# UVA-Computer-Vision-Lab/FrameINO

Measured on AMD Instinct MI355X. Metric: denoise-steps/sec (Wan2.2-5B FrameINO, 49f 704x1280, cond+uncond DiT forward + CFG + Euler), higher is better.
Workload: dtype bf16; 1 GPU; wan2.2-5b-49f-704x1280; layers=30, id_frames=1, hip_graph=False, parallelism=single, dead_rows_last_block=1760

## Files before the change

frameino_amd/_lib.py:

```python
import ctypes
import os
import re

_HERE = os.path.dirname(os.path.abspath(__file__))
LIB_PATH = os.environ.get("FINO_LIB_PATH") or os.path.join(_HERE, "lib", "libframeino_hip.so")
HEADER_PATH = os.path.join(os.path.dirname(_HERE), "include", "frameino_hip.h")

c_void_p, c_int, c_i64, c_float = ctypes.c_void_p, ctypes.c_int, ctypes.c_int64, ctypes.c_float

SIGNATURES = {
    "fino_version": [],
    "fino_last_error": [],
    "fino_tune_set": [c_int, c_int],
    "fino_tune_get": [c_int],
    "fino_adaln_modulate": [c_void_p, c_void_p, c_i64, c_int, c_i64, c_i64, c_void_p, c_void_p, c_i64, c_void_p,
                            c_float, c_int, c_void_p],
    "fino_layernorm": [c_void_p, c_void_p, c_i64, c_int, c_i64, c_i64, c_void_p, c_void_p, c_float, c_int, c_void_p],
    "fino_gated_residual": [c_void_p, c_void_p, c_void_p, c_i64, c_int, c_i64, c_i64, c_i64, c_void_p, c_i64,
                            c_void_p, c_int, c_void_p],
    "fino_gated_residual_staged": [c_void_p, c_void_p, c_void_p, c_i64, c_int, c_i64, c_i64, c_i64, c_void_p, c_i64,
                                   c_void_p, c_int, c_void_p],
    "fino_layernorm_zero": [c_void_p, c_void_p, c_i64, c_int, c_i64, c_i64, c_void_p, c_void_p, c_void_p, c_void_p,
                            c_i64, c_void_p, c_float, c_int, c_void_p],
    "fino_rmsnorm_rope": [c_void_p, c_i64, c_int, c_i64, c_void_p, c_float, c_void_p, c_void_p, c_int, c_int,
                          c_void_p],
    "fino_rmsnorm_rope_scaled": [c_void_p, c_i64, c_int, c_i64, c_void_p, c_float, c_void_p, c_void_p, c_int, c_float,
                                 c_int, c_void_p],
    "fino_qkv_rmsnorm_rope": [c_void_p, c_i64, c_int, c_i64, c_void_p, c_float, c_void_p, c_float, c_void_p, c_void_p, c_int,
                              c_float, c_void_p, c_void_p, c_void_p, c_int, c_void_p],
    "fino_rmsnorm_rope_scatter": [c_void_p, c_i64, c_int, c_i64, c_void_p, c_float, c_void_p, c_void_p, c_int, c_float,
                                  c_void_p, c_void_p, c_void_p, c_int, c_void_p],
    "fino_diag_mfma_peak": [c_int, c_int, c_int, c_void_p, ctypes.POINTER(ctypes.c_double), c_void_p],
    "fino_headnorm_rope": [c_void_p, c_int, c_i64, c_int, c_int, c_i64, c_i64, c_void_p, c_void_p, c_float,
                           c_void_p, c_void_p, c_i64, c_int, c_void_p],
    "fino_headnorm_rope_scaled": [c_void_p, c_int, c_i64, c_int, c_int, c_i64, c_i64, c_void_p, c_void_p, c_float,
                                  c_void_p, c_void_p, c_i64, c_float, c_int, c_void_p],
    "fino_attn_fwd": [c_void_p] * 4 + [c_int, c_int, c_i64, c_i64, c_int] + [c_i64] * 12 + [c_float, c_int, c_void_p],
    "fino_attn_fwd_ws": [c_void_p] * 4 + [c_int, c_int, c_i64, c_i64, c_int] + [c_i64] * 12 +
                        [c_float, c_int, c_void_p, c_i64, c_void_p],
    "fino_attn_workspace_bytes": [c_int, c_int, c_i64, c_i64, c_int],
    "fino_attn_tail_supported": [c_int, c_int, c_i64, c_i64, c_int],
    "fino_attn_fwd_tail": [c_void_p] * 4 + [c_int, c_int, c_i64, c_i64, c_int] + [c_i64] * 12 + [c_float, c_int, c_void_p, c_void_p,
                                                                                            c_void_p],
    "fino_attn_probs_supported": [c_int, c_int, c_i64, c_i64, c_int],
    "fino_attn_probs": [c_void_p] * 3 + [c_int, c_int, c_i64, c_i64, c_int] + [c_i64] * 6 + [c_int, c_i64, c_i64, c_float, c_int,
                                                                                         c_void_p, c_void_p, c_void_p, c_i64,
                                                                                         c_void_p, c_void_p],
    "fino_row_rrms": [c_void_p, c_i64, c_int, c_i64, c_float, c_void_p, c_int, c_void_p],
    "fino_attn_fp8_kv_bytes": [c_int, c_int, c_i64, c_int],
    "fino_attn_fwd_fp8": [c_void_p] * 4 + [c_int, c_int, c_i64, c_i64, c_int] + [c_i64] * 8 + [c_float, c_int, c_int, c_void_p,
                                                                                           c_i64, c_void_p],
    "fino_attn_partial_bytes": [c_int, c_int, c_i64, c_int],
    "fino_attn_partial": [c_void_p] * 3 + [c_int, c_int, c_i64, c_i64, c_int] + [c_i64] * 9 + [c_float, c_int, c_void_p,
                                                                                               c_i64, c_void_p],
    "fino_attn_merge": [c_void_p, c_int, c_int, c_i64, c_int, c_i64, c_i64, c_i64, c_void_p, c_void_p, c_void_p, c_int,
                        c_void_p],
    "fino_mxfp8_scale_bytes": [c_i64, c_i64],
    "fino_quantize_mxfp8": [c_void_p, c_void_p, c_void_p, c_i64, c_i64, c_i64, c_int, c_void_p],
    "fino_gemm_mxfp8": [c_void_p] * 6 + [c_i64] * 4 + [c_int, c_void_p, c_i64, c_void_p, c_i64, c_void_p, c_int, c_void_p],
    "fino_gemm_mxfp8_q": [c_void_p] * 7 + [c_i64] * 3 + [c_int, c_int, c_void_p],
    "fino_mxfp6_bytes": [c_i64, c_i64],
    "fino_mxfp6_scale_bytes": [c_i64, c_i64],
    "fino_quantize_mxfp6": [c_void_p, c_void_p, c_void_p, c_i64, c_i64, c_i64, c_int, c_void_p],
    "fino_gemm_mxfp6": [c_void_p] * 6 + [c_i64] * 4 + [c_int, c_void_p, c_i64, c_void_p, c_i64, c_void_p, c_int, c_void_p],
    "fino_traj_paint": [c_void_p, c_void_p, c_void_p, c_int, c_int, c_int, c_int, c_void_p],
    "fino_traj_blur_quantize": [c_void_p, c_void_p, c_void_p, c_void_p, c_int, c_int, c_int, c_int, c_void_p],
    "fino_groupnorm_workspace_bytes": [c_int],
    "fino_groupnorm_cl": [c_void_p, c_void_p] + [c_int] * 6 + [c_void_p, c_void_p, c_float, c_void_p, c_void_p] +
                         [c_int] * 4 + [c_void_p, c_i64, c_int, c_void_p],
    "fino_avg_pool_time2": [c_void_p, c_void_p] + [c_int] * 5 + [c_void_p],
    "fino_resize_area_pad_u8": [c_void_p, c_void_p] + [c_int] * 9 + [c_void_p],
    "fino_u8_hwc_to_chw_unit": [c_void_p, c_void_p, c_int, c_int, c_void_p],
    "fino_gemm": [c_void_p] * 4 + [c_i64] * 6 + [c_int, c_void_p, c_i64, c_void_p, c_i64, c_void_p, c_int, c_void_p],
    "fino_gemm_split_n": [c_void_p] * 4 + [c_i64] * 6 + [c_int, c_void_p, c_i64, c_void_p, c_i64, c_void_p, c_int, c_void_p,
                          c_i64, c_i64, c_int, c_void_p],
    "fino_ln_mxfp8": [c_int, c_void_p, c_void_p, c_void_p, c_i64, c_int, c_i64, c_void_p, c_void_p, c_void_p, c_void_p, c_i64,
                      c_void_p, c_float, c_int, c_void_p],
    "fino_gemm_blocked_a": [c_void_p, c_void_p, c_void_p, c_void_p, c_i64, c_i64, c_i64, c_i64, c_i64, c_int, c_i64, c_i64, c_i64,
                            c_i64, c_void_p, c_i64, c_void_p, c_i64, c_void_p, c_int, c_int, c_void_p],
    "fino_gemm_plan": [c_i64, c_i64, ctypes.POINTER(c_i64), ctypes.POINTER(c_int)],
    "fino_skinny_linear": [c_void_p, c_void_p, c_void_p, c_void_p, c_int, c_i64, c_i64, c_int, c_int, c_void_p],
    "fino_patchify": [c_void_p, c_void_p] + [c_int] * 7 + [c_i64, c_int, c_void_p],
    "fino_unpatchify": [c_void_p, c_void_p] + [c_int] * 7 + [c_i64, c_int, c_void_p],
    "fino_wan_model_input": [c_void_p] * 5 + [c_int] * 6 + [c_void_p],
    "fino_cfg_euler_step": [c_void_p, c_void_p, c_void_p] + [c_int] * 5 + [c_float, c_void_p, c_int, c_int, c_void_p],
    "fino_cfg_unipc_step": [c_void_p] * 6 + [c_int] * 5 + [c_void_p, c_int, c_void_p],
    "fino_cfg_vpred_step": [c_void_p, c_void_p, c_i64, c_i64, c_void_p, c_int, c_int, c_void_p],
    "fino_cfg_dpm_step": [c_void_p, c_void_p, c_void_p, c_void_p, c_i64, c_i64, c_void_p, c_int, c_int, c_void_p],
    "fino_conv3d": [c_void_p] * 4 + [c_int] * 19 + [c_void_p, c_void_p, c_int, c_void_p],
    "fino_rmsnorm_silu_cl": [c_void_p, c_void_p, c_i64, c_int, c_int, c_void_p, c_int, c_int, c_void_p],
    "fino_split_bf16": [c_void_p, c_void_p, c_i64, c_int, c_i64, c_i64, c_int, ctypes.c_uint, c_void_p],
    "fino_rmsnorm_silu_cl_f32": [c_void_p, c_void_p, c_i64, c_int, c_int, c_void_p, c_int, c_int, ctypes.c_uint, c_void_p],
    "fino_conv3d_split": [c_void_p] * 4 + [c_int] * 20 + [c_void_p, c_void_p, c_void_p],
    "fino_vae_blend_tiles": [c_void_p, c_void_p] + [c_int] * 9 + [c_void_p],
    "fino_softmax_rows": [c_void_p, c_i64, c_int, c_i64, c_float, c_int, c_void_p],
    "fino_dup_up3d_add": [c_void_p] * 3 + [c_int] * 10 + [c_void_p],
    "fino_avg_down3d_add": [c_void_p] * 3 + [c_int] * 10 + [c_void_p],
    "fino_vae_unpatchify_clamp": [c_void_p, c_void_p] + [c_int] * 7 + [c_void_p],
    "fino_vae_patchify": [c_void_p, c_void_p] + [c_int] * 7 + [c_void_p],
    "fino_lora_merge": [c_void_p, c_i64, c_void_p, c_i64, c_i64, c_i64, c_int, ctypes.POINTER(c_void_p),
                        ctypes.POINTER(c_i64), ctypes.POINTER(c_void_p), ctypes.POINTER(c_i64), ctypes.POINTER(c_int),
                        ctypes.POINTER(c_float), c_int, c_void_p],
    "fino_step_cache_probe": [c_void_p, c_int, c_i64, c_void_p, c_void_p, c_int, c_void_p],
    "fino_step_cache_residual": [c_void_p, c_i64, c_void_p, c_i64, c_void_p, c_i64, c_i64, c_i64, c_int, c_int, c_void_p],
}


class StepCacheSegment(ctypes.Structure):
    _fields_ = [("h0", c_void_p), ("h1", c_void_p), ("p", c_void_p), ("r", c_void_p), ("h1_copy", c_void_p),
                ("rows", c_i64), ("ld_h0", c_i64), ("ld_h1", c_i64), ("ld_p", c_i64), ("ld_r", c_i64), ("ld_h1_copy", c_i64)]
_RESTYPES = {"fino_last_error": ctypes.c_char_p, "fino_attn_workspace_bytes": c_i64, "fino_mxfp8_scale_bytes": c_i64,
             "fino_groupnorm_workspace_bytes": c_i64,
             "fino_attn_partial_bytes": c_i64, "fino_attn_fp8_kv_bytes": c_i64, "fino_mxfp6_bytes": c_i64,
             "fino_mxfp6_scale_bytes": c_i64}


ABI_VERSION = 103


def declared_symbols(header_path=HEADER_PATH):
    text = open(header_path).read()
    text = re.sub(r"/\*.*?\*/", "", text, flags=re.S)
    return sorted(set(re.findall(r"\b(fino_[a-z0-9_]+)\s*\(", text)))


def load(path=LIB_PATH):
    if not os.path.exists(path):
        raise RuntimeError(
            f"frameino_amd: HIP library not found at {path}. Build it with `python -c 'import __graft_entry__ as g; "
            f"g.build()'` (or `make -C frameino_amd/csrc`). There is no CPU fallback for the product path.")
    lib = ctypes.CDLL(path)
    lib.fino_version.restype = c_int
    if lib.fino_version() < 0 and os.environ.get("FINO_ALLOW_EXPERIMENT") != "1":
        raise RuntimeError(
            f"frameino_amd: {path} is a timing-EXPERIMENT build (compiled with -DFINO_EXPERIMENT: its kernels may skip "
            f"work and return wrong results; fino_version() = {lib.fino_version()}).  It is refused as the product library; "
            f"set FINO_ALLOW_EXPERIMENT=1 for the tools/ scripts that time it.")
    if abs(lib.fino_version()) != ABI_VERSION:
        raise RuntimeError(
            f"frameino_amd: {path} reports fino_version() = {lib.fino_version()}, this package binds ABI version "
            f"{ABI_VERSION} (include/frameino_hip.h: FINO_VERSION).  Rebuild it (`make -C frameino_amd/csrc`).")
    for name, argtypes in SIGNATURES.items():
        fn = getattr(lib, name)
        fn.argtypes = argtypes
        fn.restype = _RESTYPES.get(name, c_int)
    return lib


_lib = None


def lib():
    global _lib
    if _lib is None:
        _lib = load()
    return _lib


def check(rc, what=""):
    if rc != 0:
        raise RuntimeError(f"{what} failed ({rc}): {lib().fino_last_error().decode()}")
```

frameino_amd/csrc/fino_attention_probs.hip:

```cpp
#include <stdlib.h>

#include "fino_attention_common.h"
using namespace fino_attn_ns;

namespace {

struct ProbsParams {
    const uint16_t* q;
    const uint16_t* k;
    uint16_t* p;
    int batch, heads, lq, lk;
    int64_t q_bs, q_rs, q_hs, k_bs, k_rs, k_hs, p_bs, p_rs;
    int kp;
    const float* q_rrms;
    const uint16_t* q_weight;
    int64_t q_rrms_bs;
    float scale_log2;
    int lk_b[4];
    float log2_mult[4];
};

template <typename T, int NKB>
__global__ __launch_bounds__(256) void attn_probs_kernel(const ProbsParams p) {
    typedef typename T::vec8 vec8;
    __shared__ __attribute__((aligned(16))) char smem[4 * 8192];
    const int tid = threadIdx.x;
    const int lane = tid & 63;
    const int wave = tid >> 6;
    const int r = lane & 31;
    const int h = lane >> 5;
    const int hb = blockIdx.y;
    const int bi = hb / p.heads;
    const int head = hb - bi * p.heads;

    const int lkc = p.lk_b[bi < 4 ? bi : 3];
    const float lm = p.log2_mult[bi < 4 ? bi : 3];
    const int nkb = (lkc + 31) >> 5;
    const uint16_t* kp_ = p.k + bi * p.k_bs + head * p.k_hs;
    for (int i = 0; i < nkb * 2; ++i) {
        const int c = tid + 256 * i;
        const int row = c >> 4, ch = c & 15;
        uint4 u = make_uint4(0, 0, 0, 0);
        if (row < p.lk) u = *reinterpret_cast<const uint4*>(kp_ + (int64_t)row * p.k_rs + ch * 8);
        *reinterpret_cast<uint4*>(smem + row * 256 + ((ch ^ (row & 15)) << 4)) = u;
    }
    const int qrow = blockIdx.x * 128 + wave * 32 + r;
    const int qrc = qrow < p.lq ? qrow : p.lq - 1;
    const uint16_t* qp = p.q + bi * p.q_bs + head * p.q_hs + (int64_t)qrc * p.q_rs + 8 * h;
    vec8 qf[8];
    if (p.q_rrms) {
        const float rs = p.q_rrms[bi * p.q_rrms_bs + qrc];
        const uint16_t* wp = p.q_weight + head * 128 + 8 * h;
#pragma unroll
        for (int ks = 0; ks < 8; ++ks) {
            float f[8], ww[8];
            unpack8<T>(*reinterpret_cast<const uint4*>(qp + 16 * ks), f);
            unpack8<T>(*reinterpret_cast<const uint4*>(wp + 16 * ks), ww);
#pragma unroll
            for (int j = 0; j < 8; ++j) f[j] = round_to<T>(round_to<T>(f[j] * rs) * ww[j]);
            qf[ks] = __builtin_bit_cast(vec8, pack8<T>(f));
        }
    } else {
#pragma unroll
        for (int ks = 0; ks < 8; ++ks) qf[ks] = __builtin_bit_cast(vec8, *reinterpret_cast<const uint4*>(qp + 16 * ks));
    }
    __syncthreads();

    f32x16_t acc[NKB];
#pragma unroll
    for (int kb = 0; kb < NKB; ++kb)
#pragma unroll
        for (int j = 0; j < 16; ++j) acc[kb][j] = 0.f;
#pragma unroll
    for (int kb = 0; kb < NKB; ++kb) {
        if (kb < nkb) {
#pragma unroll
            for (int ks = 0; ks < 8; ++ks) {
                const int row = kb * 32 + r;
                const uint4 a = *reinterpret_cast<const uint4*>(smem + row * 256 + (((2 * ks + h) ^ (row & 15)) << 4));
                acc[kb] = T::mfma32(__builtin_bit_cast(vec8, a), qf[ks], acc[kb]);
            }
        }
    }

    const float c2 = p.scale_log2;
    float m = -INFINITY;
#pragma unroll
    for (int kb = 0; kb < NKB; ++kb) {
#pragma unroll
        for (int j = 0; j < 16; ++j) {
            const int key = kb * 32 + (j & 3) + 8 * (j >> 2) + 4 * h;
            float x = acc[kb][j] * c2;
            x = key == lkc - 1 ? x + lm : x;
            x = key >= lkc ? -INFINITY : x;
            acc[kb][j] = x;
            m = fmaxf(m, x);
        }
    }
    {
        const auto sw = __builtin_amdgcn_permlane32_swap(__float_as_uint(m), __float_as_uint(m), false, false);
        m = fmaxf(__uint_as_float(sw[0]), __uint_as_float(sw[1]));
    }
    float l = 0.f;
#pragma unroll
    for (int kb = 0; kb < NKB; ++kb) {
#pragma unroll
        for (int j = 0; j < 16; ++j) {
            const float e = __builtin_amdgcn_exp2f(acc[kb][j] - m);
            acc[kb][j] = e;
            l += e;
        }
    }
    {
        const auto sw = __builtin_amdgcn_permlane32_swap(__float_as_uint(l), __float_as_uint(l), false, false);
        l = __uint_as_float(sw[0]) + __uint_as_float(sw[1]);
    }
    const float inv = 1.0f / l;
    __syncthreads();
    char* stage = smem + wave * 8192;
#pragma unroll
    for (int kb = 0; kb < NKB; ++kb) {
#pragma unroll
        for (int g4 = 0; g4 < 4; ++g4) {
            const int key0 = kb * 32 + 8 * g4 + 4 * h;
            if (key0 < p.kp) {
                const uint32_t w0 = (uint32_t)T::from_f32(acc[kb][4 * g4 + 0] * inv) | ((uint32_t)T::from_f32(acc[kb][4 * g4 + 1] * inv) << 16);
                const uint32_t w1 = (uint32_t)T::from_f32(acc[kb][4 * g4 + 2] * inv) | ((uint32_t)T::from_f32(acc[kb][4 * g4 + 3] * inv) << 16);
                *reinterpret_cast<uint2*>(stage + r * 256 + ((((key0 >> 3)) ^ (r & 15)) << 4) + ((key0 & 4) << 1)) = make_uint2(w0, w1);
            }
        }
    }
    __syncthreads();
    const int pieces = p.kp >> 3;
    const int total = 32 * pieces;
    const int row_base = blockIdx.x * 128 + wave * 32;
    uint16_t* pbase = p.p + bi * p.p_bs + head * p.kp;
    for (int i = lane; i < total; i += 64) {
        const int rr = i / pieces, pc = i - rr * pieces;
        const uint4 u = *reinterpret_cast<const uint4*>(stage + rr * 256 + ((pc ^ (rr & 15)) << 4));
        if (row_base + rr < p.lq) *reinterpret_cast<uint4*>(pbase + (int64_t)(row_base + rr) * p.p_rs + pc * 8) = u;
    }
}

}

extern "C" int fino_attn_probs_supported(int batch, int heads, int64_t lq, int64_t lk, int head_dim) {
    return head_dim == 128 && batch >= 1 && batch <= 4 && heads > 0 && lq > 0 && lk >= 1 && lk <= 128 &&
           (int64_t)batch * heads <= 65535;
}

extern "C" int fino_attn_probs(const void* q, const void* k, void* p, int batch, int heads, int64_t lq, int64_t lk,
                               int head_dim, int64_t q_bs, int64_t q_rs, int64_t q_hs, int64_t k_bs, int64_t k_rs, int64_t k_hs,
                               int kp, int64_t p_bs, int64_t p_rs, float scale, int dtype, const int* lk_b,
                               const float* tail_mult, const float* q_rrms, int64_t q_rrms_bs, const void* q_weight,
                               void* stream) {
    FINO_CHECK((q_rrms == nullptr) == (q_weight == nullptr) && fino_aligned16(q_weight), FINO_ERR_ARG,
               "fino_attn_probs: q_rrms and q_weight come together (q_weight 16-byte aligned)");
    FINO_CHECK(dtype == FINO_BF16 || dtype == FINO_F16, FINO_ERR_ARG, "fino_attn_probs: dtype %d", dtype);
    FINO_CHECK(q && k && p && lk_b && tail_mult, FINO_ERR_ARG, "fino_attn_probs: null pointer");
    FINO_CHECK(fino_attn_probs_supported(batch, heads, lq, lk, head_dim), FINO_ERR_UNSUPPORTED,
               "fino_attn_probs: needs head_dim 128, batch <= 4, lk <= 128 (got head_dim %d, batch %d, lk %lld)", head_dim, batch,
               (long long)lk);
    FINO_CHECK(fino_aligned16(q) && fino_aligned16(k) && fino_aligned16(p) && q_rs % 8 == 0 && k_rs % 8 == 0 && q_hs % 8 == 0 &&
                   k_hs % 8 == 0 && q_bs % 8 == 0 && k_bs % 8 == 0 && p_bs % 8 == 0 && p_rs % 8 == 0,
               FINO_ERR_ARG, "fino_attn_probs: pointers and strides must be 16-byte aligned");
    FINO_CHECK(kp > 0 && kp % 8 == 0 && kp <= 128 && p_rs >= (int64_t)heads * kp, FINO_ERR_ARG,
               "fino_attn_probs: kp %d (a multiple of 8, <= 128), row stride %lld", kp, (long long)p_rs);
    FINO_CHECK(scale > 0.f || scale == FINO_ATTN_SCALE_FOLDED, FINO_ERR_ARG, "fino_attn_probs: scale");
    if (lq == 0) return FINO_OK;
    ProbsParams pp;
    pp.q = (const uint16_t*)q; pp.k = (const uint16_t*)k; pp.p = (uint16_t*)p;
    pp.batch = batch; pp.heads = heads; pp.lq = (int)lq; pp.lk = (int)lk;
    pp.q_bs = q_bs; pp.q_rs = q_rs; pp.q_hs = q_hs; pp.k_bs = k_bs; pp.k_rs = k_rs; pp.k_hs = k_hs; pp.p_bs = p_bs; pp.p_rs = p_rs;
    pp.kp = kp;
    pp.q_rrms = q_rrms; pp.q_weight = (const uint16_t*)q_weight; pp.q_rrms_bs = q_rrms_bs;
    pp.scale_log2 = scale == FINO_ATTN_SCALE_FOLDED ? 1.0f : scale * 1.4426950408889634f;
    for (int b = 0; b < 4; ++b) {
        const int bb = b < batch ? b : batch - 1;
        FINO_CHECK(lk_b[bb] >= 1 && lk_b[bb] <= lk && lk_b[bb] <= kp && tail_mult[bb] >= 1.0f, FINO_ERR_ARG,
                   "fino_attn_probs: lk_b[%d] = %d (of %lld, kp %d), tail_mult %g", bb, lk_b[bb], (long long)lk, kp,
                   (double)tail_mult[bb]);
        pp.lk_b[b] = lk_b[bb];
        pp.log2_mult[b] = log2f(tail_mult[bb]);
    }
    hipStream_t st = (hipStream_t)stream;
    const dim3 grid((unsigned)((lq + 127) / 128), (unsigned)(batch * heads));
    int max_lk = 0;
    for (int b = 0; b < batch; ++b) max_lk = lk_b[b] > max_lk ? lk_b[b] : max_lk;
    const int need = max_lk > kp ? max_lk : kp;
    const int nkb = need <= 64 ? 2 : (need <= 96 ? 3 : 4);
#define PROBS_LAUNCH(T_)                                                                                      \
    {                                                                                                         \
        if (nkb == 2) attn_probs_kernel<T_, 2><<<grid, 256, 0, st>>>(pp);                                     \
        else if (nkb == 3) attn_probs_kernel<T_, 3><<<grid, 256, 0, st>>>(pp);                                \
        else attn_probs_kernel<T_, 4><<<grid, 256, 0, st>>>(pp);                                              \
    }
    if (dtype == FINO_BF16) PROBS_LAUNCH(BF16) else PROBS_LAUNCH(F16)
#undef PROBS_LAUNCH
    FINO_LAUNCH_CHECK();
    return FINO_OK;
}
```

frameino_amd/csrc/fino_gemm.hip:

```cpp
#include <stdlib.h>

#include <atomic>
#include <type_traits>

#include "fino_gemm_common.h"

using namespace fino_gemm_ns;

#ifdef FINO_GEMM_STAMP
extern "C" int fino_gemm_debug_read(unsigned long long* out) {
    return (int)hipMemcpyFromSymbol(out, HIP_SYMBOL(fino_gemm_dbg), sizeof(unsigned long long) * 64);
}
#endif

namespace {

template <typename T, int EPI, bool GENERIC, bool CONV>
__global__ __launch_bounds__(kThreads, 2) void gemm_kernel(const GemmParams p) {
    extern __shared__ __attribute__((aligned(16))) char smem[];
    typedef typename T::vec8 vec8;
    const int tid = threadIdx.x;
    const int lane = tid & 63;
    const int wave = tid >> 6;
    const int wm = wave >> 2;
// ... 210 lines not shown
            acc0 += t1 - t0; acc1 += t2 - t1; acc2 += t3 - t2; acc3 += t4 - t3;
#endif
        }
#ifdef FINO_GEMM_STAMP
        if (blockIdx.x == 17 && lane == 0) {
            fino_gemm_dbg[wave * 8 + 0] = acc0; fino_gemm_dbg[wave * 8 + 1] = acc1;
            fino_gemm_dbg[wave * 8 + 2] = acc2; fino_gemm_dbg[wave * 8 + 3] = acc3;
            fino_gemm_dbg[wave * 8 + 4] = (unsigned long long)nk;
        }
#endif
        __syncthreads();
    }
#undef LD_W
#undef LD_A
#undef K_STEP
#undef LOAD_FRAGS
#undef MFMA_BLOCK

    gemm_epilogue<T, EPI>(acc, p, smem, m0, n0, tid, lane, wm, wn);
}

__device__ __forceinline__ int ablk_koff(const GemmParams& p, int kt) {
    const int b = (kt * p.a_inv) >> 16;
    const int j = (b * p.a_ginv) >> 16;
    return (b - j * p.a_groups) * (int)(p.a_grp_elems * 2) + j * (int)(p.a_blk_elems * 2) + (kt - b * p.a_tpb) * (BK * 2);
}

template <typename T, bool CONV, int MI, bool ABLK = false>
__device__ __forceinline__ void pp_mainloop(const GemmParams& p, char* smem, const int64_t m0, const int64_t n0,
                                            const int kb, const int nk, f32x4_t (&acc)[MI][4], const int tid,
                                            const int lane, const int wave, const int wm, const int wn) {
    typedef typename T::vec8 vec8;
    static_assert(MI >= 2 && MI <= 8, "tile height 64 .. 256");
    static_assert(!CONV || MI == 8, "the implicit-GEMM gather is built for 256-row tiles");
    enum : int { NA0 = (MI + 1) / 2, NA1 = MI - (MI + 1) / 2 };

    const int r8 = lane >> 3;
    const int sk = ((lane & 7) ^ ((4 * (wn & 1) + (lane >> 4)) & 7)) * 8;
    const __amdgpu_buffer_rsrc_t w_rsrc = __builtin_amdgcn_make_buffer_rsrc(
        (void*)p.w, 0, (int)(((p.n - 1) * p.ldw + p.k) * 2), 0x00020000);
    const int aq0 = wm == 0 ? 0 : NA0;
    uint32_t a_off[4], w_off[8];
    uint32_t pos[CONV ? 4 : 1];
    int ck = 0, tap_t = 0, tap_h = 0, tap_w = 0, t_first = 0, t_in_first = 0;
    int cseg = 0, seg = 0, a_koff = 0;
    const uint16_t* a_base_ptr = p.a;
    int64_t a_bytes = ((p.m - 1) * p.lda + p.k) * 2;
    if constexpr (ABLK)
        a_bytes = ((p.a_groups - 1) * p.a_grp_elems + (p.k / (BK * p.a_tpb) / p.a_groups - 1) * p.a_blk_elems +
                   (p.m - 1) * p.lda + BK * p.a_tpb) * 2;
    if constexpr (CONV) {
        const int hw = p.ho * p.wo;
        t_first = (int)(m0 / hw);
        t_in_first = t_first * p.st - p.pt;
        t_in_first = t_in_first < 0 ? 0 : t_in_first;
        const int64_t frame = (int64_t)p.hi * p.wi * p.lda;
        a_base_ptr = p.a + (int64_t)t_in_first * frame;
        a_bytes = (int64_t)(p.ti - t_in_first) * frame * 2;
        a_bytes = a_bytes > 0x7fffffffll ? 0x7fffffffll : a_bytes;
#pragma unroll
        for (int q = 0; q < NA0; ++q) {
            int64_t gm = m0 + (aq0 + q) * 32 + wn * 8 + r8;
            gm = gm < p.m ? gm : p.m - 1;
            const int t = (int)(gm / hw);
            const int rem = (int)(gm - (int64_t)t * hw);
            const int h = rem / p.wo;
            pos[q] = ((uint32_t)(t - t_first) << 24) | ((uint32_t)h << 12) | (uint32_t)(rem - h * p.wo);
        }
    }
    const __amdgpu_buffer_rsrc_t a_rsrc = __builtin_amdgcn_make_buffer_rsrc((void*)a_base_ptr, 0, (int)a_bytes, 0x00020000);
    auto conv_offsets = [&]() {
        const int hlim = p.up ? 2 * p.hi : p.hi, wlim = p.up ? 2 * p.wi : p.wi;
#pragma unroll
        for (int q = 0; q < NA0; ++q) {
            const int ti = (t_first + (int)(pos[CONV ? q : 0] >> 24)) * p.st + tap_t - p.pt;
            int hi = (int)((pos[CONV ? q : 0] >> 12) & 0xfffu) * p.sh + tap_h - p.ph;
            int wi = (int)(pos[CONV ? q : 0] & 0xfffu) * p.sw + tap_w - p.pw;
            const bool ok = (unsigned)ti < (unsigned)p.ti && (unsigned)hi < (unsigned)hlim && (unsigned)wi < (unsigned)wlim;
            if (p.up) { hi >>= 1; wi >>= 1; }
            const uint32_t off = (uint32_t)(((((ti - t_in_first) * p.hi + hi) * p.wi + wi) * (int)p.lda + sk) * 2);
            a_off[q] = ok ? off : 0x80000000u;
        }
    };
    auto conv_next = [&]() {
        if (p.a_cc > 0 && ++cseg == p.a_cc) { cseg = 0; ++seg; }
        if (++ck == p.cin_chunks) {
            ck = 0; cseg = 0; seg = 0;
            if (++tap_w == p.kw) {
                tap_w = 0;
                if (++tap_h == p.kh) { tap_h = 0; ++tap_t; }
            }
            conv_offsets();
        }
        if (p.a_cc > 0) {
            const int plane = p.a_nplanes == 3 ? (seg >= 3) + (seg >= 5) : (seg >= 2);
            a_koff = (plane * p.a_cc + cseg) * (BK * 2);
        } else {
            a_koff = ck * (BK * 2);
        }
    };
    if constexpr (CONV) {
        conv_offsets();
    } else {
#pragma unroll
        for (int q = 0; q < NA0; ++q) {
            int64_t gm = m0 + (aq0 + q) * 32 + wn * 8 + r8;
            gm = gm < p.m ? gm : p.m - 1;
            a_off[q] = (uint32_t)((gm * p.lda + sk) * 2);
        }
    }
    const int w_piece_bytes = (int)(32 * p.ldw * 2);
    const int w_pieces = CONV ? (int)((p.n - n0 + 31) / 32) : 8;
#pragma unroll
    for (int q = 0; q < 8; ++q) {
        int64_t gn = n0 + q * 32 + wn * 8 + r8;
        gn = gn < p.n ? gn : p.n - 1;
        w_off[q] = (uint32_t)((gn * p.ldw + sk) * 2);
    }
#ifndef GP_DMA_AUX
#define GP_DMA_AUX 0
#endif
#define PP_DMA_A(STAGE_, KT_, QI_)                                                                                \
    if ((QI_) < NA1 || wm == 0)                                                                                   \
        __builtin_amdgcn_raw_ptr_buffer_load_lds(                                                                 \
            a_rsrc, (FINO_LDS void*)(smem + (STAGE_) * kStageBytes + ((aq0 + (QI_)) * 32 + wn * 8) * 128), 16,    \
            a_off[QI_], CONV ? a_koff : (ABLK ? ablk_koff(p, kb + (KT_)) : (kb + (KT_)) * (BK * 2)), 0, GP_DMA_AUX);
#define PP_DMA_W(STAGE_, KT_, Q_)                                                                                 \
    if (!CONV || (Q_) < w_pieces)                                                                                 \
        __builtin_amdgcn_raw_ptr_buffer_load_lds(                                                                 \
            w_rsrc, (FINO_LDS void*)(smem + (STAGE_) * kStageBytes + kTileBytes + ((Q_) * 32 + wn * 8) * 128), 16, \
            w_off[CONV ? 0 : (Q_)], (kb + (KT_)) * (BK * 2) + (CONV ? (Q_) * w_piece_bytes : 0), 0, GP_DMA_AUX);

    const int frow = lane & 15;
    const int pch0 = (lane >> 4) ^ (frow >> 1);
    const int a_base = (wm * (16 * MI) + frow) * 128;
    const int w_base = kTileBytes + (wn * 64 + frow) * 128;

#pragma unroll
    for (int i = 0; i < MI; ++i)
#pragma unroll
        for (int j = 0; j < 4; ++j) acc[i][j] = f32x4_t{0.f, 0.f, 0.f, 0.f};

#pragma unroll
    for (int q = 0; q < 4; ++q) {
        if (q < NA0) { PP_DMA_A(0, 0, q) }
        if (wm == 0) { PP_DMA_W(0, 0, q) } else { PP_DMA_W(0, 0, 4 + q) }
    }
    if constexpr (CONV) conv_next();
    if (nk > 1) {
#pragma unroll
        for (int q = 0; q < 4; ++q) {
            if (q < NA0) { PP_DMA_A(1, 1, q) }
            if (wm == 0) { PP_DMA_W(1, 1, q) } else { PP_DMA_W(1, 1, 4 + q) }
        }
        if constexpr (CONV) conv_next();
    }
    asm volatile("s_waitcnt vmcnt(0)" ::: "memory");
    __builtin_amdgcn_s_barrier();
    if (wm == 1) __builtin_amdgcn_s_barrier();

    u32x4_t af[2][MI], wf[2][4];
#ifdef FINO_GEMM_STAMP
    unsigned long long t0, t1, t2, t3, t4, acc0 = 0, acc1 = 0, acc2 = 0, acc3 = 0;
#define PSTAMP(V_) { __builtin_amdgcn_sched_barrier(0); STAMP(V_) __builtin_amdgcn_sched_barrier(0); }
#else
#define PSTAMP(V_)
#endif
    for (int t = 0; t < nk; ++t) {
        const int cur = t & 1;
        const char* sb = smem + cur * kStageBytes;
        PSTAMP(t0)
#pragma unroll
        for (int kk = 0; kk < 2; ++kk) {
            const int pch = (pch0 ^ (kk << 2)) << 4;
#pragma unroll
            for (int j = 0; j < 4; ++j) wf[kk][j] = *reinterpret_cast<const u32x4_t*>(sb + w_base + j * 2048 + pch);
#pragma unroll
            for (int i = 0; i < MI; ++i) af[kk][i] = *reinterpret_cast<const u32x4_t*>(sb + a_base + i * 2048 + pch);
        }
        if (t >= 1 && t + 1 < nk) {
#pragma unroll
            for (int q = 0; q < NA0; ++q) PP_DMA_A(cur ^ 1, t + 1, q)
            if (wm == 0) {
#pragma unroll
                for (int q = 0; q < 8; ++q) { PP_DMA_W(cur ^ 1, t + 1, q) }
            }
            if constexpr (CONV) conv_next();
        }
        __builtin_amdgcn_sched_barrier(0);
        asm volatile("s_waitcnt lgkmcnt(0)" ::: "memory");
        PSTAMP(t1)
        __builtin_amdgcn_s_barrier();
        __builtin_amdgcn_sched_barrier(0);
        PSTAMP(t2)
#ifndef GP_ORDER
#define GP_ORDER 3
#endif
#pragma unroll
        for (int kk = 0; kk < 2; ++kk) {
#if GP_ORDER == 0
#pragma unroll
            for (int i = 0; i < MI; ++i) {
#pragma unroll
                for (int j = 0; j < 4; ++j)
                    acc[i][j] = T::mfma16(__builtin_bit_cast(vec8, wf[kk][j]), __builtin_bit_cast(vec8, af[kk][i]),
                                          acc[i][j]);
            }
#elif GP_ORDER == 1
#pragma unroll
            for (int j = 0; j < 4; ++j) {
#pragma unroll
                for (int i = 0; i < MI; ++i)
                    acc[i][j] = T::mfma16(__builtin_bit_cast(vec8, wf[kk][j]), __builtin_bit_cast(vec8, af[kk][i]),
                                          acc[i][j]);
            }
#elif GP_ORDER == 2
#pragma unroll
            for (int j = 0; j < 4; ++j) {
#pragma unroll
                for (int ii = 0; ii < MI; ++ii) {
                    const int i = ((j + 4 * kk) & 1) ? MI - 1 - ii : ii;
                    acc[i][j] = T::mfma16(__builtin_bit_cast(vec8, wf[kk][j]), __builtin_bit_cast(vec8, af[kk][i]),
                                          acc[i][j]);
                }
            }
#else
#pragma unroll
            for (int i = 0; i < MI; ++i) {
#pragma unroll
                for (int jj = 0; jj < 4; ++jj) {
                    const int j = ((i + MI * kk) & 1) ? 3 - jj : jj;
                    acc[i][j] = T::mfma16(__builtin_bit_cast(vec8, wf[kk][j]), __builtin_bit_cast(vec8, af[kk][i]),
                                          acc[i][j]);
                }
            }
#endif
        }
        __builtin_amdgcn_sched_barrier(0);
        asm volatile("s_waitcnt vmcnt(0)" ::: "memory");
        PSTAMP(t3)
        __builtin_amdgcn_s_barrier();
        __builtin_amdgcn_sched_barrier(0);
#ifdef FINO_GEMM_STAMP
        STAMP(t4)
        acc0 += t1 - t0; acc1 += t2 - t1; acc2 += t3 - t2; acc3 += t4 - t3;
#endif
    }
#ifdef FINO_GEMM_STAMP
    if (blockIdx.x == 17 && lane == 0) {
        fino_gemm_dbg[wave * 8 + 0] = acc0; fino_gemm_dbg[wave * 8 + 1] = acc1;
        fino_gemm_dbg[wave * 8 + 2] = acc2; fino_gemm_dbg[wave * 8 + 3] = acc3;
        fino_gemm_dbg[wave * 8 + 4] = (unsigned long long)nk;
    }
#endif
    if (wm == 0) __builtin_amdgcn_s_barrier();
    asm volatile("s_waitcnt vmcnt(0)" ::: "memory");
#undef PP_DMA_A
#undef PP_DMA_W
}

template <typename T, int EPI, bool CONV = false, int MI = 8, bool ABLK = false>
__global__ __launch_bounds__(kThreads, 2) void gemm_pp_kernel(const GemmParams p) {
    extern __shared__ __attribute__((aligned(16))) char smem[];
    const int tid = threadIdx.x;
    const int lane = tid & 63;
    const int wave = __builtin_amdgcn_readfirstlane(tid >> 6);
    const int wm = wave >> 2;
    const int wn = wave & 3;
    int tm, tn;
    tile_coords(p, tm, tn);
    const int64_t m0 = (int64_t)tm * (32 * MI), n0 = (int64_t)tn * BN;
    int nk = (int)(p.k / BK);
#ifndef GP_RAGGED
#define GP_RAGGED 1
#endif
    if constexpr (GP_RAGGED && MI == 8 && !CONV && EPI != FINO_EPI_F32 && EPI != FINO_EPI_F32_RESIDUAL) {
        const int64_t rows = p.m - m0;
        if (rows <= 64) {
            f32x4_t acc2[2][4];
            pp_mainloop<T, false, 2, ABLK>(p, smem, m0, n0, 0, nk, acc2, tid, lane, wave, wm, wn);
            gemm_epilogue<T, EPI, false, 2>(acc2, p, smem, m0, n0, tid, lane, wm, wn);
            return;
        }
        if (rows <= 128) {
            f32x4_t acc4[4][4];
            pp_mainloop<T, false, 4, ABLK>(p, smem, m0, n0, 0, nk, acc4, tid, lane, wave, wm, wn);
            gemm_epilogue<T, EPI, false, 4>(acc4, p, smem, m0, n0, tid, lane, wm, wn);
            return;
        }
    }
    f32x4_t acc[MI][4];
#ifdef FINO_GEMM_STAMP
    unsigned long long ts0, ts1;
    STAMP(ts0)
#endif
    pp_mainloop<T, CONV, MI, ABLK>(p, smem, m0, n0, 0, nk, acc, tid, lane, wave, wm, wn);
#ifdef FINO_GEMM_STAMP
    STAMP(ts1)
    if (blockIdx.x == 17 && lane == 0) fino_gemm_dbg[wave * 8 + 5] = ts1 - ts0;
#endif
    gemm_epilogue<T, EPI, false, MI>(acc, p, smem, m0, n0, tid, lane, wm, wn);
}

template <typename T, int EPI, bool GENERIC, bool CONV = false>
int launch_gemm_t(const GemmParams& p, hipStream_t st) {
    static FinoPerDeviceOnce once;
    if (int rc = fino_max_smem_once(once, reinterpret_cast<const void*>(&gemm_kernel<T, EPI, GENERIC, CONV>), kSmemBytes, "fino_gemm")) return rc;
    gemm_kernel<T, EPI, GENERIC, CONV><<<dim3((unsigned)(p.tiles_m * p.tiles_n)), kThreads, kSmemBytes, st>>>(p);
    FINO_LAUNCH_CHECK();
    return FINO_OK;
}

template <typename T, int EPI, bool CONV = false, int MI = 8, bool ABLK = false>
int launch_gemm_pp(const GemmParams& p, hipStream_t st) {
    static FinoPerDeviceOnce once;
    if (int rc = fino_max_smem_once(once, reinterpret_cast<const void*>(&gemm_pp_kernel<T, EPI, CONV, MI, ABLK>), kSmemBytes, "fino_gemm")) return rc;
    gemm_pp_kernel<T, EPI, CONV, MI, ABLK><<<dim3((unsigned)(p.tiles_m * p.tiles_n)), kThreads, kSmemBytes, st>>>(p);
    FINO_LAUNCH_CHECK();
    return FINO_OK;
}

inline int gemm_device_cus() {
    static std::atomic<int> cus[kFinoMaxDevices];
    const int dev = fino_current_device();
    int c = cus[dev].load(std::memory_order_relaxed);
    if (c == 0) {
        int n = 0;
        c = (hipDeviceGetAttribute(&n, hipDeviceAttributeMultiprocessorCount, dev) == hipSuccess && n > 0) ? n : 256;
        cus[dev].store(c, std::memory_order_relaxed);
    }
    return c;
}

struct TilePlan { int64_t rows1; int mi2; };
inline double plan_launch_cost(int64_t rows, int mi, int tiles_n, int cus) {
    if (rows <= 0) return 0.0;
    const double bm = 32.0 * mi;
    const int64_t tiles = ((rows + 32 * mi - 1) / (32 * mi)) * tiles_n;
    const double mfma_raw = 0.85 * bm / 256.0, mfma = mfma_raw > 0.80 ? mfma_raw : 0.80, deliver = (bm + 256.0) / 512.0;
    const int64_t full = tiles / cus, rem = tiles % cus;
    double c = (double)full * (mfma > deliver ? mfma : deliver);
    if (rem) {
        const double d = deliver * (double)rem / cus;
        c += mfma > d ? mfma : d;
    }
    return c + 0.07;
}
inline TilePlan plan_tiles_search(int64_t m, int tiles_n, int cus);
inline TilePlan plan_tiles(int64_t m, int tiles_n, int cus, int tile_m = 0) {
    const int forced = tile_m ? tile_m : fino_tune_get(FINO_TUNE_GEMM_TILE_M);
    if (forced >= 2 && forced <= 7) return TilePlan{0, forced};
    if (forced == 8 || m <= 0) return TilePlan{m, 8};
    static std::atomic<uint64_t> memo[64];
    const bool memoable = m < (1ll << 24) && tiles_n > 0 && tiles_n < 512 && cus > 0 && cus < 512;
    const uint64_t key = ((uint64_t)m << 18) | ((uint64_t)tiles_n << 9) | (uint64_t)cus;
    std::atomic<uint64_t>& slot = memo[(key * 0x9E3779B97F4A7C15ull) >> 58];
    if (memoable) {
        const uint64_t e = slot.load(std::memory_order_relaxed);
        if ((e & 1) && (e >> 22) == key) {
            const uint64_t r = (e >> 6) & 0xffff;
            return TilePlan{r == 0xffff ? m : (int64_t)r * 256, (int)((e >> 3) & 7) + 1};
        }
    }
    const TilePlan tp = plan_tiles_search(m, tiles_n, cus);
    if (memoable && (tp.rows1 == m || (tp.rows1 % 256 == 0 && tp.rows1 / 256 < 0xffff)) && tp.mi2 >= 2 && tp.mi2 <= 8)
        slot.store((key << 22) | ((tp.rows1 == m ? 0xffffull : (uint64_t)(tp.rows1 / 256)) << 6) |
                       ((uint64_t)(tp.mi2 - 1) << 3) | 1ull, std::memory_order_relaxed);
    return tp;
}
inline TilePlan plan_tiles_search(int64_t m, int tiles_n, int cus) {
    TilePlan best{m, 8};
    double best_c = plan_launch_cost(m, 8, tiles_n, cus);
    const double base_c = best_c;
    const int64_t rows256 = (m + 255) / 256;
    for (int64_t r1 = 0; r1 < rows256; ++r1) {
        const int64_t rows1 = r1 * 256;
        const double c1 = plan_launch_cost(rows1, 8, tiles_n, cus);
        for (int mi = 2; mi <= 8; ++mi) {
            if (rows1 > 0 && mi == 8) continue;
            const double c = c1 + plan_launch_cost(m - rows1, mi, tiles_n, cus);
            if (c < best_c - 1e-9) { best_c = c; best = TilePlan{rows1, mi}; }
        }
    }
    if (best_c > (best.rows1 > 0 ? 0.97 : 0.985) * base_c) return TilePlan{m, 8};
    return best;
}

inline bool use_pingpong() {
    static int v = -1;
    if (v < 0) {
        const char* e = getenv("FINO_GEMM_PP");
        v = (e && e[0] == '0') ? 0 : 1;
    }
    return v == 1;
}

template <typename T, int EPI>
int launch_gemm_pp_mi(const GemmParams& p, int mi, hipStream_t st) {
    if (p.a_tpb > 0) {
        if constexpr (EPI == FINO_EPI_GATED_RESIDUAL) {
            switch (mi) {
                case 2: return launch_gemm_pp<T, EPI, false, 2, true>(p, st);
                case 3: return launch_gemm_pp<T, EPI, false, 3, true>(p, st);
                case 4: return launch_gemm_pp<T, EPI, false, 4, true>(p, st);
                case 5: return launch_gemm_pp<T, EPI, false, 5, true>(p, st);
                case 6: return launch_gemm_pp<T, EPI, false, 6, true>(p, st);
                case 7: return launch_gemm_pp<T, EPI, false, 7, true>(p, st);
                default: return launch_gemm_pp<T, EPI, false, 8, true>(p, st);
            }
        } else {
            fino_set_error("fino_gemm_blocked_a: epilogue must be FINO_EPI_GATED_RESIDUAL");
            return FINO_ERR_UNSUPPORTED;
        }
    }
    switch (mi) {
        case 2: return launch_gemm_pp<T, EPI, false, 2>(p, st);
        case 3: return launch_gemm_pp<T, EPI, false, 3>(p, st);
        case 4: return launch_gemm_pp<T, EPI, false, 4>(p, st);
        case 5: return launch_gemm_pp<T, EPI, false, 5>(p, st);
        case 6: return launch_gemm_pp<T, EPI, false, 6>(p, st);
        case 7: return launch_gemm_pp<T, EPI, false, 7>(p, st);
        default: return launch_gemm_pp<T, EPI, false, 8>(p, st);
    }
}

template <typename T>
int launch_gemm_rows(GemmParams p, int64_t r0, int64_t rows, int mi, int epi, hipStream_t st) {
    p.a += r0 * p.lda;
    p.c += r0 * p.ldc;
    if (p.c2) p.c2 += r0 * p.ldc2;
    if (p.r) p.r += r0 * p.ldr;
    if (p.sel) p.sel += r0;
    p.m = rows;
    p.tiles_m = (int)((rows + 32 * mi - 1) / (32 * mi));
    switch (epi) {
        case FINO_EPI_NONE: return launch_gemm_pp_mi<T, FINO_EPI_NONE>(p, mi, st);
        case FINO_EPI_GELU_TANH: return launch_gemm_pp_mi<T, FINO_EPI_GELU_TANH>(p, mi, st);
        case FINO_EPI_RESIDUAL: return launch_gemm_pp_mi<T, FINO_EPI_RESIDUAL>(p, mi, st);
        case FINO_EPI_GATED_RESIDUAL_STAGED: return launch_gemm_pp_mi<T, FINO_EPI_GATED_RESIDUAL_STAGED>(p, mi, st);
        default: return launch_gemm_pp_mi<T, FINO_EPI_GATED_RESIDUAL>(p, mi, st);
    }
}

template <typename T, bool GENERIC>
int launch_gemm_e(const GemmParams& p, int epi, int tile_m, hipStream_t st) {
    const bool fits32 = ((p.m - 1) * p.lda + p.k) * 2 < (1ll << 31) && ((p.n - 1) * p.ldw + p.k) * 2 < (1ll << 31);
    if (epi == FINO_EPI_F32 || epi == FINO_EPI_F32_RESIDUAL) {
        if (GENERIC || !fits32) {
            fino_set_error("fino_gemm: the fp32-output epilogues need K %% 64 == 0, 16-byte aligned operands and operands < 2 GiB");
            return FINO_ERR_UNSUPPORTED;
        }
        return epi == FINO_EPI_F32 ? launch_gemm_pp<T, FINO_EPI_F32, false, 8>(p, st)
                                   : launch_gemm_pp<T, FINO_EPI_F32_RESIDUAL, false, 8>(p, st);
    }
    if (!GENERIC && use_pingpong() && fits32) {
        const TilePlan tp = plan_tiles(p.m, p.tiles_n, gemm_device_cus(), tile_m);
        if (tp.rows1 > 0)
            if (int rc = launch_gemm_rows<T>(p, 0, tp.rows1, 8, epi, st)) return rc;
        if (tp.rows1 < p.m) return launch_gemm_rows<T>(p, tp.rows1, p.m - tp.rows1, tp.mi2, epi, st);
        return FINO_OK;
    }
    switch (epi) {
        case FINO_EPI_NONE: return launch_gemm_t<T, FINO_EPI_NONE, GENERIC>(p, st);
        case FINO_EPI_GELU_TANH: return launch_gemm_t<T, FINO_EPI_GELU_TANH, GENERIC>(p, st);
        case FINO_EPI_RESIDUAL: return launch_gemm_t<T, FINO_EPI_RESIDUAL, GENERIC>(p, st);
        case FINO_EPI_GATED_RESIDUAL_STAGED: return launch_gemm_t<T, FINO_EPI_GATED_RESIDUAL_STAGED, GENERIC>(p, st);
        default: return launch_gemm_t<T, FINO_EPI_GATED_RESIDUAL, GENERIC>(p, st);
    }
}

template <int WT>
__global__ __launch_bounds__(256) void skinny_linear_kernel(const float* __restrict__ x, const void* __restrict__ w,
                                                            const void* __restrict__ b, float* __restrict__ y, int m,
                                                            int64_t n, int64_t k, int silu_input) {
    const int lane = threadIdx.x & 63;
    const int64_t col = (int64_t)blockIdx.x * 4 + (threadIdx.x >> 6);
    if (col >= n) return;
    float acc[16];
#pragma unroll
    for (int i = 0; i < 16; ++i) acc[i] = 0.f;
    for (int64_t kk = lane; kk < k; kk += 64) {
        float wv;
        if (WT == -1) wv = ((const float*)w)[col * k + kk];
        else if (WT == FINO_BF16) wv = BF16::to_f32(((const uint16_t*)w)[col * k + kk]);
        else wv = F16::to_f32(((const uint16_t*)w)[col * k + kk]);
#pragma unroll
        for (int i = 0; i < 16; ++i) {
            if (i < m) {
                float xv = x[(int64_t)i * k + kk];
                if (silu_input) xv = xv / (1.0f + __expf(-xv));
                acc[i] += xv * wv;
            }
        }
    }
    float bias = 0.f;
    if (b) {
        if (WT == -1) bias = ((const float*)b)[col];
        else if (WT == FINO_BF16) bias = BF16::to_f32(((const uint16_t*)b)[col]);
        else bias = F16::to_f32(((const uint16_t*)b)[col]);
    }
#pragma unroll
    for (int i = 0; i < 16; ++i) {
        if (i < m) {
            const float s = wave_sum(acc[i]);
            if (lane == 0) y[(int64_t)i * n + col] = s + bias;
        }
    }
}

}

extern "C" int fino_gemm_plan(int64_t m, int64_t n, int64_t* rows_256, int* tile_rows_rest) {
    if (m <= 0 || n <= 0) return FINO_ERR_ARG;
    const TilePlan tp = plan_tiles(m, (int)((n + BN - 1) / BN), gemm_device_cus());
    if (rows_256) *rows_256 = tp.rows1;
    if (tile_rows_rest) *tile_rows_rest = tp.rows1 < m ? 32 * tp.mi2 : 0;
    return FINO_OK;
}

extern "C" int fino_gemm(const void* a, const void* w, const void* bias, void* c, int64_t m, int64_t n, int64_t k,
                         int64_t lda, int64_t ldw, int64_t ldc, int epilogue, const void* r, int64_t ldr,
                         const float* gate, int64_t mod_stride, const int32_t* sel, int dtype, void* stream) {
    return fino_gemm_split_n(a, w, bias, c, m, n, k, lda, ldw, ldc, epilogue, r, ldr, gate, mod_stride, sel, dtype, nullptr,
                             0, 0, 0, stream);
}

extern "C" int fino_gemm_split_n(const void* a, const void* w, const void* bias, void* c, int64_t m, int64_t n, int64_t k,
                                 int64_t lda, int64_t ldw, int64_t ldc, int epilogue, const void* r, int64_t ldr,
                                 const float* gate, int64_t mod_stride, const int32_t* sel, int dtype, void* c2,
                                 int64_t ldc2, int64_t n_split, int tile_m, void* stream) {
    FINO_CHECK(dtype == FINO_BF16 || dtype == FINO_F16, FINO_ERR_ARG, "fino_gemm: dtype %d", dtype);
    FINO_CHECK(tile_m == 0 || (tile_m >= 2 && tile_m <= 8), FINO_ERR_ARG, "fino_gemm: tile_m=%d (0 = planned, 2 .. 8)", tile_m);
    if (c2 || n_split) {
        FINO_CHECK(c2 && n_split > 0 && n_split < n && n_split % BN == 0 && ldc2 % 8 == 0 && ldc2 >= n - n_split &&
                       fino_aligned16(c2) && k % BK == 0 && epilogue <= FINO_EPI_GELU_TANH,
                   FINO_ERR_ARG,
                   "fino_gemm_split_n: needs c2, 0 < n_split < N a multiple of %d, ldc2 >= N - n_split, K %% %d == 0, no "
                   "residual epilogue", BN, BK);
        FINO_CHECK(ldc >= n_split, FINO_ERR_ARG, "fino_gemm_split_n: ldc must cover the first n_split columns");
    }
    FINO_CHECK(a && w && c, FINO_ERR_ARG, "fino_gemm: null pointer");
    FINO_CHECK(m >= 0 && n > 0 && k > 0, FINO_ERR_ARG, "fino_gemm: bad shape M=%lld N=%lld K=%lld", (long long)m,
               (long long)n, (long long)k);
    FINO_CHECK(n % 8 == 0 && k % 8 == 0, FINO_ERR_ARG, "fino_gemm: N=%lld and K=%lld must be multiples of 8",
               (long long)n, (long long)k);
    FINO_CHECK(lda % 8 == 0 && ldw % 8 == 0 && ldc % 8 == 0 && lda >= k && ldw >= k && ldc >= (n_split > 0 ? n_split : n),
               FINO_ERR_ARG, "fino_gemm: leading dimensions must be multiples of 8 and cover the row");
    FINO_CHECK(fino_aligned16(a) && fino_aligned16(w) && fino_aligned16(c), FINO_ERR_ARG,
               "fino_gemm: A/W/C must be 16-byte aligned");
    FINO_CHECK(epilogue >= FINO_EPI_NONE && epilogue <= FINO_EPI_F32_RESIDUAL, FINO_ERR_ARG,
               "fino_gemm: epilogue %d", epilogue);
    if (epilogue == FINO_EPI_F32 || epilogue == FINO_EPI_F32_RESIDUAL)
        FINO_CHECK(!c2 && tile_m == 0 && fino_aligned16(bias), FINO_ERR_ARG,
                   "fino_gemm: the fp32-output epilogues take one output, the planned tiling and a 16-byte aligned fp32 bias");
    if (epilogue >= FINO_EPI_RESIDUAL && epilogue != FINO_EPI_F32)
        FINO_CHECK(r && ldr % 8 == 0 && ldr >= n && fino_aligned16(r), FINO_ERR_ARG, "fino_gemm: residual operand");
    if (epilogue == FINO_EPI_GATED_RESIDUAL || epilogue == FINO_EPI_GATED_RESIDUAL_STAGED)
        FINO_CHECK(gate && fino_aligned16(gate) && mod_stride % 4 == 0, FINO_ERR_ARG, "fino_gemm: gate operand");
    if (m == 0) return FINO_OK;
    GemmParams p = {};
    p.c2 = (uint16_t*)c2; p.ldc2 = ldc2; p.n_split = n_split;
    p.a = (const uint16_t*)a; p.w = (const uint16_t*)w; p.bias = (const uint16_t*)bias; p.c = (uint16_t*)c;
    p.r = (const uint16_t*)r; p.gate = gate; p.sel = sel;
    p.m = m; p.n = n; p.k = k; p.lda = lda; p.ldw = ldw; p.ldc = ldc; p.ldr = ldr; p.mod_stride = mod_stride;
    p.tiles_m = (int)((m + BM - 1) / BM);
    p.tiles_n = (int)((n + BN - 1) / BN);
    p.group_m = fino_tune_get(FINO_TUNE_GEMM_GROUP_M);
    hipStream_t st = (hipStream_t)stream;
    const bool generic = (k % BK) != 0;
    if (p.group_m <= 0) p.group_m = gemm_default_group_m(p.tiles_n, k);
    {
        const int rk = fino_tune_get(FINO_TUNE_GEMM_RASTER);
        if (rk == 1 || (rk == 3 && (k >= 8192 || n >= 8192)) || (rk != 2 && rk != 3 && k >= 8192)) p.group_m |= 0x100;
    }
    if (dtype == FINO_BF16)
        return generic ? launch_gemm_e<BF16, true>(p, epilogue, tile_m, st) : launch_gemm_e<BF16, false>(p, epilogue, tile_m, st);
    return generic ? launch_gemm_e<F16, true>(p, epilogue, tile_m, st) : launch_gemm_e<F16, false>(p, epilogue, tile_m, st);
}

extern "C" int fino_gemm_blocked_a(const void* a, const void* w, const void* bias, void* c, int64_t m, int64_t n, int64_t k,
                                   int64_t a_block_k, int64_t a_block_stride, int a_groups, int64_t a_group_stride,
                                   int64_t lda, int64_t ldw, int64_t ldc,
                                   const void* r, int64_t ldr, const float* gate, int64_t mod_stride, const int32_t* sel,
                                   int dtype, int tile_m, void* stream) {
    FINO_CHECK(dtype == FINO_BF16 || dtype == FINO_F16, FINO_ERR_ARG, "fino_gemm_blocked_a: dtype %d", dtype);
    FINO_CHECK(tile_m == 0 || (tile_m >= 2 && tile_m <= 8), FINO_ERR_ARG, "fino_gemm_blocked_a: tile_m=%d (0 = planned, 2 .. 8)",
               tile_m);
    FINO_CHECK(a && w && c && r && gate, FINO_ERR_ARG, "fino_gemm_blocked_a: null pointer");
    FINO_CHECK(m >= 0 && n > 0 && k > 0 && n % 8 == 0, FINO_ERR_ARG, "fino_gemm_blocked_a: bad shape");
    FINO_CHECK(a_block_k > 0 && a_block_k % BK == 0 && k % a_block_k == 0 && a_block_k / BK <= 256 && k / BK <= 4096,
               FINO_ERR_ARG, "fino_gemm_blocked_a: a_block_k=%lld must be a multiple of %d dividing K=%lld",
               (long long)a_block_k, BK, (long long)k);
    FINO_CHECK(lda % 8 == 0 && lda >= a_block_k && a_block_stride % 8 == 0 && ldw % 8 == 0 && ldw >= k && ldc % 8 == 0 &&
                   ldc >= n && ldr % 8 == 0 && ldr >= n && mod_stride % 4 == 0,
               FINO_ERR_ARG, "fino_gemm_blocked_a: leading dimensions");
    FINO_CHECK(fino_aligned16(a) && fino_aligned16(w) && fino_aligned16(c) && fino_aligned16(r) && fino_aligned16(gate),
               FINO_ERR_ARG, "fino_gemm_blocked_a: 16-byte alignment required");
    const int64_t nblk = k / a_block_k;
    FINO_CHECK(a_groups >= 1 && a_groups <= 16 && nblk % a_groups == 0 && a_group_stride % 8 == 0, FINO_ERR_ARG,
               "fino_gemm_blocked_a: a_groups=%d must divide the %lld K blocks", a_groups, (long long)nblk);
    const int64_t span = ((a_groups - 1) * a_group_stride + (nblk / a_groups - 1) * a_block_stride +
                          (m > 0 ? m - 1 : 0) * lda + a_block_k) * 2;
    FINO_CHECK(span < (1ll << 31) && ((n - 1) * ldw + k) * 2 < (1ll << 31), FINO_ERR_ARG,
               "fino_gemm_blocked_a: operands must span < 2 GiB");
    if (m == 0) return FINO_OK;
    GemmParams p = {};
    p.a = (const uint16_t*)a; p.w = (const uint16_t*)w; p.bias = (const uint16_t*)bias; p.c = (uint16_t*)c;
    p.r = (const uint16_t*)r; p.gate = gate; p.sel = sel;
    p.m = m; p.n = n; p.k = k; p.lda = lda; p.ldw = ldw; p.ldc = ldc; p.ldr = ldr; p.mod_stride = mod_stride;
    p.a_tpb = (int)(a_block_k / BK); p.a_inv = (65536 + p.a_tpb - 1) / p.a_tpb; p.a_blk_elems = a_block_stride;
    p.a_groups = a_groups; p.a_ginv = (65536 + a_groups - 1) / a_groups; p.a_grp_elems = a_group_stride;
    FINO_CHECK((k / BK - 1) * ((int64_t)p.a_inv * p.a_tpb - 65536) < 65536 &&
                   (nblk - 1) * ((int64_t)p.a_ginv * a_groups - 65536) < 65536,
               FINO_ERR_UNSUPPORTED,
               "fino_gemm_blocked_a: a_block_k=%lld / a_groups=%d with K=%lld is beyond the exact range of the kernel's "
               "reciprocal index arithmetic", (long long)a_block_k, a_groups, (long long)k);
    p.tiles_m = (int)((m + BM - 1) / BM);
    p.tiles_n = (int)((n + BN - 1) / BN);
    p.group_m = fino_tune_get(FINO_TUNE_GEMM_GROUP_M);
    if (p.group_m <= 0) p.group_m = gemm_default_group_m(p.tiles_n, k);
    hipStream_t st = (hipStream_t)stream;
    const TilePlan tp = plan_tiles(p.m, p.tiles_n, gemm_device_cus(), tile_m);
    auto rows = [&](int64_t r0, int64_t nr, int mi) {
        return dtype == FINO_BF16 ? launch_gemm_rows<BF16>(p, r0, nr, mi, FINO_EPI_GATED_RESIDUAL, st)
                                  : launch_gemm_rows<F16>(p, r0, nr, mi, FINO_EPI_GATED_RESIDUAL, st);
    };
    if (tp.rows1 > 0)
        if (int rc = rows(0, tp.rows1, 8)) return rc;
    if (tp.rows1 < p.m) return rows(tp.rows1, p.m - tp.rows1, tp.mi2);
    return FINO_OK;
}

static int conv3d_impl(const void* x, const void* w, const void* bias, void* y, int t_in, int h_in, int w_in,
                       int c_in_pad, int t_out, int h_out, int w_out, int c_out_pad, int kt, int kh, int kw, int st,
                       int sh, int sw, int pt, int ph, int pw, int upsample2x, int epilogue, const void* r,
                       const void* zero_page, int dtype, int planes, void* stream);

extern "C" int fino_conv3d(const void* x, const void* w, const void* bias, void* y, int t_in, int h_in, int w_in,
                           int c_in_pad, int t_out, int h_out, int w_out, int c_out_pad, int kt, int kh, int kw, int st,
                           int sh, int sw, int pt, int ph, int pw, int upsample2x, int epilogue, const void* r,
                           const void* zero_page, int dtype, void* stream) {
    return conv3d_impl(x, w, bias, y, t_in, h_in, w_in, c_in_pad, t_out, h_out, w_out, c_out_pad, kt, kh, kw, st, sh, sw, pt, ph,
                       pw, upsample2x, epilogue, r, zero_page, dtype, 0, stream);
}

extern "C" int fino_conv3d_split(const void* x_planes, const void* w_products, const float* bias, float* y, int t_in, int h_in,
                                 int w_in, int c_in_pad, int planes, int t_out, int h_out, int w_out, int c_out_pad, int kt,
                                 int kh, int kw, int st, int sh, int sw, int pt, int ph, int pw, int upsample2x, int epilogue,
                                 const float* r, const void* zero_page, void* stream) {
    FINO_CHECK(planes == 2 || planes == 3, FINO_ERR_ARG, "fino_conv3d_split: planes = %d (2: hi | lo, 3: hi | mid | lo)", planes);
    return conv3d_impl(x_planes, w_products, bias, y, t_in, h_in, w_in, c_in_pad, t_out, h_out, w_out, c_out_pad, kt, kh, kw, st,
                       sh, sw, pt, ph, pw, upsample2x, epilogue, r, zero_page, FINO_BF16, planes, stream);
}

static int conv3d_impl(const void* x, const void* w, const void* bias, void* y, int t_in, int h_in, int w_in,
                       int c_in_pad, int t_out, int h_out, int w_out, int c_out_pad, int kt, int kh, int kw, int st,
                       int sh, int sw, int pt, int ph, int pw, int upsample2x, int epilogue, const void* r,
                       const void* zero_page, int dtype, int planes, void* stream) {
    FINO_CHECK(dtype == FINO_BF16 || dtype == FINO_F16, FINO_ERR_ARG, "fino_conv3d: dtype %d", dtype);
    FINO_CHECK(x && w && y && zero_page, FINO_ERR_ARG, "fino_conv3d: null pointer");
    FINO_CHECK(c_in_pad > 0 && c_in_pad % BK == 0, FINO_ERR_ARG,
               "fino_conv3d: c_in_pad=%d must be a multiple of %d (pad channels with zeros)", c_in_pad, BK);
    FINO_CHECK(c_out_pad > 0 && c_out_pad % 8 == 0, FINO_ERR_ARG, "fino_conv3d: c_out_pad=%d %% 8 != 0", c_out_pad);
    FINO_CHECK(t_in > 0 && h_in > 0 && w_in > 0 && t_out > 0 && h_out > 0 && w_out > 0 && kt > 0 && kh > 0 && kw > 0 &&
                   st > 0 && sh > 0 && sw > 0 && pt >= 0 && ph >= 0 && pw >= 0,
               FINO_ERR_ARG, "fino_conv3d: bad geometry");
    FINO_CHECK(epilogue == FINO_EPI_NONE || (epilogue == FINO_EPI_RESIDUAL && r), FINO_ERR_ARG,
               "fino_conv3d: epilogue %d (NONE or RESIDUAL with r)", epilogue);
    FINO_CHECK(fino_aligned16(x) && fino_aligned16(w) && fino_aligned16(y) && fino_aligned16(r) &&
                   fino_aligned16(zero_page),
               FINO_ERR_ARG, "fino_conv3d: 16-byte alignment required");
    FINO_CHECK(planes == 0 || fino_aligned16(bias), FINO_ERR_ARG, "fino_conv3d_split: bias must be 16-byte aligned");
    const int products = planes == 0 ? 1 : (planes == 2 ? 3 : 6);
    const int64_t a_width = (int64_t)(planes == 0 ? 1 : planes) * c_in_pad;
    GemmParams p = {};
    p.a = (const uint16_t*)x; p.w = (const uint16_t*)w; p.bias = (const uint16_t*)bias; p.c = (uint16_t*)y;
    p.r = (const uint16_t*)r; p.gate = nullptr; p.sel = nullptr;
    p.m = (int64_t)t_out * h_out * w_out; p.n = c_out_pad; p.k = (int64_t)kt * kh * kw * c_in_pad * products;
    p.lda = a_width; p.ldw = p.k; p.ldc = c_out_pad; p.ldr = c_out_pad; p.mod_stride = 0;
    p.a_cc = planes == 0 ? 0 : c_in_pad / BK; p.a_nplanes = planes;
    p.tiles_m = (int)((p.m + BM - 1) / BM); p.tiles_n = (int)((p.n + BN - 1) / BN);
    p.group_m = fino_tune_get(FINO_TUNE_GEMM_GROUP_M);
    p.to = t_out; p.ho = h_out; p.wo = w_out; p.ti = t_in; p.hi = h_in; p.wi = w_in;
    p.kt = kt; p.kh = kh; p.kw = kw; p.st = st; p.sh = sh; p.sw = sw; p.pt = pt; p.ph = ph; p.pw = pw;
    p.up = upsample2x; p.cin_chunks = c_in_pad / BK * products; p.zero_page = (const uint16_t*)zero_page;
    hipStream_t s = (hipStream_t)stream;
    const int64_t hw_out = (int64_t)h_out * w_out;
    const int64_t t_span = (BM - 1 + hw_out - 1) / hw_out + 1;
    const int64_t in_span_bytes = (t_span * st + kt) * (int64_t)h_in * w_in * a_width * 2;
    const bool pp = use_pingpong() && fino_tune_get(FINO_TUNE_CONV_LOOP) != 1 && in_span_bytes < (1ll << 31) &&
                    h_out < 4096 && w_out < 4096 && t_span < 256 && c_out_pad % 32 == 0 && ((p.n - 1) * p.ldw + p.k) * 2 < (1ll << 31);
    if (planes > 0) {
        if (!pp) {
            fino_set_error("fino_conv3d_split: a 256-row tile's input span (%lld bytes) exceeds the 2 GiB the gather offsets cover, "
                           "or c_out_pad %% 32 != 0 -- run the layer in chunks of fewer frames", (long long)in_span_bytes);
            return FINO_ERR_UNSUPPORTED;
        }
        return epilogue == FINO_EPI_NONE ? launch_gemm_pp<BF16, FINO_EPI_F32, true>(p, s)
                                         : launch_gemm_pp<BF16, FINO_EPI_F32_RESIDUAL, true>(p, s);
    }
    if (pp) {
        if (dtype == FINO_BF16)
            return epilogue == FINO_EPI_NONE ? launch_gemm_pp<BF16, FINO_EPI_NONE, true>(p, s)
                                             : launch_gemm_pp<BF16, FINO_EPI_RESIDUAL, true>(p, s);
        return epilogue == FINO_EPI_NONE ? launch_gemm_pp<F16, FINO_EPI_NONE, true>(p, s)
                                         : launch_gemm_pp<F16, FINO_EPI_RESIDUAL, true>(p, s);
    }
    if (dtype == FINO_BF16)
        return epilogue == FINO_EPI_NONE ? launch_gemm_t<BF16, FINO_EPI_NONE, false, true>(p, s)
                                         : launch_gemm_t<BF16, FINO_EPI_RESIDUAL, false, true>(p, s);
    return epilogue == FINO_EPI_NONE ? launch_gemm_t<F16, FINO_EPI_NONE, false, true>(p, s)
                                     : launch_gemm_t<F16, FINO_EPI_RESIDUAL, false, true>(p, s);
}

extern "C" int fino_skinny_linear(const float* x, const void* w, const void* b, float* y, int m, int64_t n,
                                  int64_t k, int w_dtype, int silu_input, void* stream) {
    FINO_CHECK(x && w && y, FINO_ERR_ARG, "fino_skinny_linear: null pointer");
    FINO_CHECK(m >= 1 && m <= 16 && n > 0 && k > 0, FINO_ERR_ARG, "fino_skinny_linear: need 1 <= M <= 16 (M=%d)", m);
    FINO_CHECK(w_dtype == -1 || w_dtype == FINO_BF16 || w_dtype == FINO_F16, FINO_ERR_ARG,
               "fino_skinny_linear: w_dtype %d", w_dtype);
    const dim3 grid((unsigned)((n + 3) / 4));
    hipStream_t st = (hipStream_t)stream;
    if (w_dtype == -1) skinny_linear_kernel<-1><<<grid, 256, 0, st>>>(x, w, b, y, m, n, k, silu_input);
    else if (w_dtype == FINO_BF16) skinny_linear_kernel<FINO_BF16><<<grid, 256, 0, st>>>(x, w, b, y, m, n, k, silu_input);
    else skinny_linear_kernel<FINO_F16><<<grid, 256, 0, st>>>(x, w, b, y, m, n, k, silu_input);
    FINO_LAUNCH_CHECK();
    return FINO_OK;
}
```

frameino_amd/ops.py:

```python
import os

import torch

from . import _lib

BF16, F16 = 0, 1
EPI_NONE, EPI_GELU_TANH, EPI_RESIDUAL, EPI_GATED_RESIDUAL, EPI_GATED_RESIDUAL_STAGED = 0, 1, 2, 3, 4
EPI_F32, EPI_F32_RESIDUAL = 5, 6


class KernelTimer:

    active = None

    def __init__(self, names):
        self.names = set(names)
        self.events = {n: [] for n in self.names}
        self.flops = {}
        self.bytes = {}

    def __enter__(self):
        KernelTimer.active = self
        return self

    def __exit__(self, *exc):
        KernelTimer.active = None

    def summary(self):
        torch.cuda.synchronize()
        out = {}
        for n, evs in self.events.items():
            ms = [s.elapsed_time(e) for s, e in evs]
            if ms:
                out[n] = {"launches": len(ms), "avg_us": 1e3 * sum(ms) / len(ms), "total_ms": sum(ms)}
        return out


def _timed(name):
    kt = KernelTimer.active
    if kt is None or name not in kt.names:
        return None
    s, e = torch.cuda.Event(enable_timing=True), torch.cuda.Event(enable_timing=True)
    kt.events[name].append((s, e))
    s.record()
    return e


def _timed_gemm(epilogue, flops, nbytes=0.0):
    kt = KernelTimer.active
    if kt is None:
        return None
    name = "gemm" if epilogue is None else f"gemm_epi{int(epilogue)}"
    if name not in kt.names:
        name = "gemm"
        if name not in kt.names:
            return None
    ev = _timed(name)

    def done():
        ev.record()
        kt.flops[name] = kt.flops.get(name, 0.0) + flops
        kt.bytes[name] = kt.bytes.get(name, 0.0) + nbytes
    return done


def _dt(t):
    if t.dtype == torch.bfloat16:
        return BF16
    if t.dtype == torch.float16:
        return F16
    raise TypeError(f"frameino_amd: activations must be bf16 or fp16, got {t.dtype}")


F32 = 2


def _dt3(t):
    return F32 if t.dtype == torch.float32 else _dt(t)


def _stream():
    return torch.cuda.current_stream().cuda_stream


def _p(t):
    return 0 if t is None else t.data_ptr()


def _rows2d(t):
    if not t.is_cuda:
        raise RuntimeError("frameino_amd ops need CUDA(HIP) tensors; there is no CPU path")
    if t.stride(-1) != 1:
        raise ValueError("last dimension must be contiguous")
    t2 = t if t.dim() == 2 else t.reshape(-1, t.shape[-1]) if t.is_contiguous() else None
    if t2 is None:
        if t.dim() == 3 and t.shape[0] == 1:
            t2 = t[0]
        else:
            raise ValueError("need a 2-D row-strided view")
    return t2, t2.shape[0], t2.shape[1], t2.stride(0)


def _epi_operands(residual, gate):
    r2, ldr = (None, 0)
    if residual is not None:
        r2, _, _, ldr = _rows2d(residual)
    return r2, ldr, gate.stride(0) if (gate is not None and gate.dim() == 2) else 0


def _mx_pair(shape, scale_bytes, device, out):
    if out is not None:
        return out
    return (torch.empty(shape, dtype=torch.uint8, device=device), torch.zeros(scale_bytes, dtype=torch.uint8, device=device))


def adaln_modulate(x, shift, scale, sel=None, eps=1e-6, out=None):
    x2, rows, dim, ldx = _rows2d(x)
    out = torch.empty_like(x2) if out is None else out
    o2, _, _, ldy = _rows2d(out)
    assert shift.dtype == torch.float32 and scale.dtype == torch.float32
    ms = shift.stride(0) if shift.dim() == 2 else 0
    if scale.dim() == 2:
        assert scale.stride(0) == ms
    _lib.check(_lib.lib().fino_adaln_modulate(_p(x2), _p(o2), rows, dim, ldx, ldy, _p(shift), _p(scale), ms, _p(sel),
                                             eps, _dt(x), _stream()), "fino_adaln_modulate")
    return out.view(x.shape) if out.shape != x.shape and out.numel() == x.numel() else out


def layernorm(x, weight=None, bias=None, eps=1e-5, out=None):
    x2, rows, dim, ldx = _rows2d(x)
    out = torch.empty_like(x2) if out is None else out
    o2, _, _, ldy = _rows2d(out)
    for t in (weight, bias):
        assert t is None or t.dtype == torch.float32
    _lib.check(_lib.lib().fino_layernorm(_p(x2), _p(o2), rows, dim, ldx, ldy, _p(weight), _p(bias), eps, _dt(x),
                                        _stream()), "fino_layernorm")
    return out.view(x.shape) if out.shape != x.shape and out.numel() == x.numel() else out


def layernorm_zero(x, weight, bias, shift, scale, sel=None, eps=1e-5, out=None):
    x2, rows, dim, ldx = _rows2d(x)
    out = torch.empty_like(x2) if out is None else out
    o2, _, _, ldy = _rows2d(out)
    for t in (weight, bias, shift, scale):
        assert t is None or t.dtype == torch.float32
    ms = shift.stride(0) if shift.dim() == 2 else 0
    _lib.check(_lib.lib().fino_layernorm_zero(_p(x2), _p(o2), rows, dim, ldx, ldy, _p(weight), _p(bias), _p(shift),
                                             _p(scale), ms, _p(sel), eps, _dt(x), _stream()), "fino_layernorm_zero")
    return out.view(x.shape) if out.shape != x.shape and out.numel() == x.numel() else out


def gated_residual(x, y, gate=None, sel=None, out=None, staged=False):
    x2, rows, dim, ldx = _rows2d(x)
    y2, _, _, ldy = _rows2d(y)
    out = torch.empty_like(x2) if out is None else out
    o2, _, _, ldo = _rows2d(out)
    ms = gate.stride(0) if (gate is not None and gate.dim() == 2) else 0
    fn = _lib.lib().fino_gated_residual_staged if staged else _lib.lib().fino_gated_residual
    _lib.check(fn(_p(x2), _p(y2), _p(o2), rows, dim, ldx, ldy, ldo, _p(gate), ms, _p(sel), _dt(x), _stream()),
               "fino_gated_residual")
    return out.view(x.shape) if out.shape != x.shape and out.numel() == x.numel() else out


SCALE_FOLDED = -1.0
LOG2E = 1.4426950408889634


def rmsnorm_rope_(x, weight, eps, cos=None, sin=None, head_dim=0, out_scale=1.0):
    x2, rows, dim, ldx = _rows2d(x)
    if cos is not None:
        assert cos.dtype == torch.float32 and cos.is_contiguous() and cos.shape == (rows, head_dim // 2)
        assert sin.dtype == torch.float32 and sin.is_contiguous() and sin.shape == cos.shape
    _lib.check(_lib.lib().fino_rmsnorm_rope_scaled(_p(x2), rows, dim, ldx, _p(weight), eps, _p(cos), _p(sin), head_dim,
                                                  float(out_scale), _dt(x), _stream()), "fino_rmsnorm_rope")
    return x


def qkv_rmsnorm_rope_(qkv, dim, q_weight, q_eps, k_weight, k_eps, cos, sin, head_dim, q_out_scale=1.0, out=None,
                      head_off=None, head_ld=None):
    x2, rows, width, ldx = _rows2d(qkv)
    assert width == 3 * dim
    assert cos.dtype == torch.float32 and cos.is_contiguous() and cos.shape == (rows, head_dim // 2) and sin.shape == cos.shape
    if out is not None:
        assert head_off.dtype == torch.int64 and head_off.numel() == 3 * (dim // head_dim) and head_off.is_contiguous()
        assert head_ld.dtype == torch.int64 and head_ld.numel() == dim // head_dim and out.is_contiguous()
    _lib.check(_lib.lib().fino_qkv_rmsnorm_rope(_p(x2), rows, dim, ldx, _p(q_weight), q_eps, _p(k_weight), k_eps, _p(cos),
                                                _p(sin), head_dim, float(q_out_scale), _p(out), _p(head_off), _p(head_ld),
                                                _dt(qkv), _stream()), "fino_qkv_rmsnorm_rope")
    return qkv if out is None else out


def rmsnorm_rope_scatter(x, weight, eps, cos, sin, head_dim, out, head_off, head_ld, out_scale=1.0):
    x2, rows, dim, ldx = _rows2d(x)
    assert head_off.dtype == torch.int64 and head_ld.dtype == torch.int64 and head_off.is_cuda and head_ld.is_cuda
    assert head_off.numel() == dim // head_dim == head_ld.numel() and out.is_contiguous() and out.dtype == x.dtype
    if cos is not None:
        assert cos.dtype == torch.float32 and cos.is_contiguous() and cos.shape == (rows, head_dim // 2)
        assert sin.dtype == torch.float32 and sin.is_contiguous() and sin.shape == cos.shape
    _lib.check(_lib.lib().fino_rmsnorm_rope_scatter(_p(x2), rows, dim, ldx, _p(weight), eps, _p(cos), _p(sin), head_dim,
                                                    float(out_scale), _p(out), _p(head_off), _p(head_ld), _dt(x),
                                                    _stream()), "fino_rmsnorm_rope_scatter")
    return out


def headnorm_rope_(x, heads, head_dim, weight, bias, eps, cos=None, sin=None, rope_row0=0, out_scale=1.0):
    assert x.dim() == 3 and x.stride(2) == 1
    b, rows, _ = x.shape
    _lib.check(_lib.lib().fino_headnorm_rope_scaled(_p(x), b, rows, heads, head_dim, x.stride(1), x.stride(0), _p(weight),
                                                   _p(bias), eps, _p(cos), _p(sin), rope_row0, float(out_scale), _dt(x),
                                                   _stream()), "fino_headnorm_rope")
    return x


SPLIT_ATTENTION_TAIL = os.environ.get("FINO_ATTN_SPLIT", "1") != "0"
_attn_ws = {}


def _attention_workspace(b, heads, lq, lk, dh, device):
    need = _lib.lib().fino_attn_workspace_bytes(b, heads, lq, lk, dh)
    if need <= 0:
        return None, 0
    key = (device.index, torch.cuda.current_stream().cuda_stream)
    ws = _attn_ws.get(key)
    if ws is None or ws.numel() * 4 < need:
        ws = _attn_ws[key] = torch.empty(need // 4, dtype=torch.float32, device=device)
    return ws, need


def attention(q, k, v, heads, out=None, scale=None):
    assert q.dim() == 3 and k.dim() == 3 and v.dim() == 3
    b, lq, hd = q.shape
    lk = k.shape[1]
    dh = hd // heads
    for t in (q, k, v):
        assert t.stride(2) == 1 and t.is_cuda
    if out is None:
        out = torch.empty((b, lq, hd), dtype=q.dtype, device=q.device)
    scale = dh ** -0.5 if scale is None else scale
    ev = _timed("attn_self" if lk > 1024 else "attn_cross")
    ws, ws_bytes = _attention_workspace(b, heads, lq, lk, dh, q.device) if SPLIT_ATTENTION_TAIL else (None, 0)
    _lib.check(_lib.lib().fino_attn_fwd_ws(_p(q), _p(k), _p(v), _p(out), b, heads, lq, lk, dh,
                                          q.stride(0), q.stride(1), dh, k.stride(0), k.stride(1), dh,
                                          v.stride(0), v.stride(1), dh, out.stride(0), out.stride(1), dh,
                                          float(scale), _dt(q), _p(ws), ws_bytes, _stream()), "fino_attn_fwd_ws")
    if ev is not None:
        ev.record()
        kt_ = KernelTimer.active
        nm = "attn_self" if lk > 1024 else "attn_cross"
        kt_.flops[nm] = kt_.flops.get(nm, 0.0) + 4.0 * b * lq * lk * hd
        kt_.bytes[nm] = kt_.bytes.get(nm, 0.0) + 2.0 * b * hd * (2 * lq + 2 * lk)
    return out


def attention_tail_supported(b, heads, lq, lk, dh):
    return bool(_lib.lib().fino_attn_tail_supported(int(b), int(heads), int(lq), int(lk), int(dh)))


def attention_tail(q, k, v, heads, lk_b, tail_mult, out=None, scale=None):
    import ctypes
    assert q.dim() == 3 and k.dim() == 3 and v.dim() == 3
    b, lq, hd = q.shape
    lk = k.shape[1]
    dh = hd // heads
    for t in (q, k, v):
        assert t.stride(2) == 1 and t.is_cuda
    assert len(lk_b) == b and len(tail_mult) == b
    if out is None:
        out = torch.empty((b, lq, hd), dtype=q.dtype, device=q.device)
    scale = dh ** -0.5 if scale is None else scale
    lk_arr = (ctypes.c_int * b)(*[int(x) for x in lk_b])
    mult_arr = (ctypes.c_float * b)(*[float(x) for x in tail_mult])
    ev = _timed("attn_cross")
    _lib.check(_lib.lib().fino_attn_fwd_tail(_p(q), _p(k), _p(v), _p(out), b, heads, lq, lk, dh,
                                            q.stride(0), q.stride(1), dh, k.stride(0), k.stride(1), dh,
                                            v.stride(0), v.stride(1), dh, out.stride(0), out.stride(1), dh,
                                            float(scale), _dt(q), ctypes.cast(lk_arr, ctypes.c_void_p),
                                            ctypes.cast(mult_arr, ctypes.c_void_p), _stream()), "fino_attn_fwd_tail")
    if ev is not None:
        ev.record()
        kt_ = KernelTimer.active
        kt_.flops["attn_cross"] = kt_.flops.get("attn_cross", 0.0) + 4.0 * lq * hd * sum(int(x) for x in lk_b)
    return out


def attention_probs_supported(b, heads, lq, lk, dh):
    return bool(_lib.lib().fino_attn_probs_supported(int(b), int(heads), int(lq), int(lk), int(dh)))


def row_rrms(x, eps, out=None):
    x2, rows, dim, ldx = _rows2d(x)
    if out is None:
        out = torch.empty(rows, dtype=torch.float32, device=x.device)
    assert out.dtype == torch.float32 and out.is_contiguous() and out.numel() >= rows
    _lib.check(_lib.lib().fino_row_rrms(_p(x2), rows, dim, ldx, float(eps), _p(out), _dt(x), _stream()), "fino_row_rrms")
    return out


def attention_probs(q, k, heads, lk_b, tail_mult, kp, out=None, scale=None, q_rrms=None, q_weight=None):
    import ctypes
    assert q.dim() == 3 and k.dim() == 3
    b, lq, hd = q.shape
    lk = k.shape[1]
    dh = hd // heads
    for t in (q, k):
        assert t.stride(2) == 1 and t.is_cuda
    if out is None:
        out = torch.empty((b, lq, heads * kp), dtype=q.dtype, device=q.device)
    assert out.shape == (b, lq, heads * kp) and out.stride(2) == 1
    scale = dh ** -0.5 if scale is None else scale
    lk_arr = (ctypes.c_int * b)(*[int(x) for x in lk_b])
    mult_arr = (ctypes.c_float * b)(*[float(x) for x in tail_mult])
    ev = _timed("attn_cross")
    _lib.check(_lib.lib().fino_attn_probs(_p(q), _p(k), _p(out), b, heads, lq, lk, dh, q.stride(0), q.stride(1), dh,
                                         k.stride(0), k.stride(1), dh, int(kp), out.stride(0), out.stride(1), float(scale),
                                         _dt(q), ctypes.cast(lk_arr, ctypes.c_void_p), ctypes.cast(mult_arr, ctypes.c_void_p),
                                         _p(q_rrms), q_rrms.stride(0) if q_rrms is not None else 0, _p(q_weight), _stream()),
               "fino_attn_probs")
    if ev is not None:
        ev.record()
        kt_ = KernelTimer.active
        kt_.flops["attn_cross"] = kt_.flops.get("attn_cross", 0.0) + 2.0 * lq * hd * sum(int(x) for x in lk_b)
    return out


_attn_fp8_ws = {}


FP8_P_EXP2, FP8_P_RAMP = 0, 1
FP8_P_MODES = {"exp2": FP8_P_EXP2, "ramp": FP8_P_RAMP}
_p_env = os.environ.get("FINO_FP8_P_MODE", "ramp")
if _p_env not in FP8_P_MODES:
    raise ValueError(f"FINO_FP8_P_MODE={_p_env!r}: expected one of {' | '.join(FP8_P_MODES)} (how the opt-in fp8 attention turns a "
                     f"softmax weight into its e4m3 byte; 'ramp' -- a piecewise-linear exp2, the default since round 4 -- adds "
                     f"~0.3e-2 to the 5.5e-2 rel-RMS of the fp8 operands, 'exp2' is the exact form)")
FP8_P_DEFAULT = FP8_P_MODES[_p_env]


def attention_fp8(q, k, v, heads, out=None, scale=None, p_mode=None):
    p_mode = FP8_P_DEFAULT if p_mode is None else FP8_P_MODES.get(p_mode, p_mode)
    assert q.dim() == 3 and k.dim() == 3 and v.dim() == 3
    b, lq, hd = q.shape
    lk = k.shape[1]
    dh = hd // heads
    for t in (q, k, v):
        assert t.stride(2) == 1 and t.is_cuda
    if out is None:
        out = torch.empty((b, lq, hd), dtype=q.dtype, device=q.device)
    scale = dh ** -0.5 if scale is None else scale
    need = _lib.lib().fino_attn_fp8_kv_bytes(b, heads, lk, dh)
    if need <= 0:
        raise RuntimeError(f"attention_fp8: head_dim {dh} is not supported (64 or 128)")
    key = (q.device.index, torch.cuda.current_stream().cuda_stream)
    ws = _attn_fp8_ws.get(key)
    if ws is None or ws.numel() < need:
        ws = _attn_fp8_ws[key] = torch.empty(need, dtype=torch.uint8, device=q.device)
    ev = _timed("attn_self" if lk > 1024 else "attn_cross")
    _lib.check(_lib.lib().fino_attn_fwd_fp8(_p(q), _p(k), _p(v), _p(out), b, heads, lq, lk, dh, q.stride(0), q.stride(1),
                                           k.stride(0), k.stride(1), v.stride(0), v.stride(1), out.stride(0), out.stride(1),
                                           float(scale), _dt(q), int(p_mode), _p(ws), need, _stream()), "fino_attn_fwd_fp8")
    if ev is not None:
        ev.record()
        kt_ = KernelTimer.active
        nm = "attn_self" if lk > 1024 else "attn_cross"
        kt_.flops[nm] = kt_.flops.get(nm, 0.0) + 4.0 * b * lq * lk * hd
    return out


def attention_partial_floats(batch, heads, lq, head_dim):
    return _lib.lib().fino_attn_partial_bytes(batch, heads, lq, head_dim) // 4


def attention_partial(q, k, v, heads, out=None, scale=None):
    assert q.dim() == 3 and k.dim() == 3 and v.dim() == 3
    b, lq, hd = q.shape
    lk = k.shape[1]
    dh = hd // heads
    for t in (q, k, v):
        assert t.stride(2) == 1 and t.is_cuda
    need = _lib.lib().fino_attn_partial_bytes(b, heads, lq, dh)
    if out is None or out.numel() * 4 < need:
        out = torch.empty(need // 4, dtype=torch.float32, device=q.device)
    scale = dh ** -0.5 if scale is None else scale
    _lib.check(_lib.lib().fino_attn_partial(_p(q), _p(k), _p(v), b, heads, lq, lk, dh, q.stride(0), q.stride(1), dh,
                                           k.stride(0), k.stride(1), dh, v.stride(0), v.stride(1), dh, float(scale),
                                           _dt(q), _p(out), need, _stream()), "fino_attn_partial")
    return out


def attention_merge(parts, batch, lq, heads, head_dim, dtype, out=None):
    assert 1 <= len(parts) <= 3
    if out is None:
        out = torch.empty((batch, lq, heads * head_dim), dtype=dtype, device=parts[0].device)
    ps = list(parts) + [None] * (3 - len(parts))
    _lib.check(_lib.lib().fino_attn_merge(_p(out), batch, heads, lq, head_dim, out.stride(0), out.stride(1), head_dim,
                                         _p(ps[0]), _p(ps[1]), _p(ps[2]), _dt(out), _stream()), "fino_attn_merge")
    return out


def gemm_plan(m, n):
    import ctypes
    r, t = ctypes.c_int64(), ctypes.c_int()
    _lib.check(_lib.lib().fino_gemm_plan(m, n, ctypes.byref(r), ctypes.byref(t)), "fino_gemm_plan")
    return r.value, t.value


def gemm(a, w, bias=None, epilogue=EPI_NONE, residual=None, gate=None, sel=None, out=None, out2=None, split=0, tile_m=0):
    a2, m, k, lda = _rows2d(a)
    assert w.dim() == 2 and w.stride(1) == 1 and w.shape[1] == k and w.dtype == a.dtype
    n = w.shape[0]
    if out is None:
        out = torch.empty((m, split or n), dtype=a.dtype, device=a.device)
    o2, _, _, ldc = _rows2d(out)
    if out2 is not None:
        assert 0 < split < n and residual is None
        c2, _, _, ldc2 = _rows2d(out2)
        done = _timed_gemm(None, 2.0 * m * n * k)
        _lib.check(_lib.lib().fino_gemm_split_n(_p(a2), _p(w), _p(bias), _p(o2), m, n, k, lda, w.stride(0), ldc, epilogue,
                                               0, 0, 0, 0, 0, _dt(a), _p(c2), ldc2, split, tile_m, _stream()),
                   "fino_gemm_split_n")
        if done is not None:
            done()
        return out, out2
    r2, ldr, ms = _epi_operands(residual, gate)
    if bias is not None:
        assert bias.dtype == a.dtype and bias.is_contiguous()
    done = _timed_gemm(epilogue, 2.0 * m * n * k, 2.0 * (m * k + n * k + m * n * (2 if residual is not None else 1)))
    if tile_m:
        _lib.check(_lib.lib().fino_gemm_split_n(_p(a2), _p(w), _p(bias), _p(o2), m, n, k, lda, w.stride(0), ldc, epilogue,
                                               _p(r2), ldr, _p(gate), ms, _p(sel), _dt(a), None, 0, 0, tile_m, _stream()),
                   "fino_gemm_split_n")
    else:
        _lib.check(_lib.lib().fino_gemm(_p(a2), _p(w), _p(bias), _p(o2), m, n, k, lda, w.stride(0), ldc, epilogue, _p(r2),
                                       ldr, _p(gate), ms, _p(sel), _dt(a), _stream()), "fino_gemm")
    if done is not None:
        done()
    return out


def gemm_blocked_a(a_blocks, rows, w, bias, residual, gate, sel, out, tile_m=0):
    if a_blocks.dim() == 3:
        a_blocks = a_blocks[None]
    assert a_blocks.dim() == 4 and a_blocks.stride(3) == 1 and w.dtype == a_blocks.dtype and w.stride(1) == 1
    groups, peers, _, bk = a_blocks.shape
    n, k = w.shape
    assert k == groups * peers * bk and residual.shape == (rows, n) and out.shape == (rows, n)
    r2, _, _, ldr = _rows2d(residual)
    o2, _, _, ldc = _rows2d(out)
    ms = gate.stride(0) if gate.dim() == 2 else 0
    done = _timed_gemm(None, 2.0 * rows * n * k)
    _lib.check(_lib.lib().fino_gemm_blocked_a(_p(a_blocks), _p(w), _p(bias), _p(o2), rows, n, k, bk, a_blocks.stride(1),
                                              groups, a_blocks.stride(0), a_blocks.stride(2), w.stride(0), ldc, _p(r2),
                                              ldr, _p(gate), ms, _p(sel), _dt(a_blocks), tile_m, _stream()),
               "fino_gemm_blocked_a")
    if done is not None:
        done()
    return out


def quantize_mxfp8(x, out=None):
    x2, rows, cols, ldx = _rows2d(x)
    nbytes = _lib.lib().fino_mxfp8_scale_bytes(rows, cols)
    if nbytes <= 0:
        raise ValueError(f"quantize_mxfp8: cols={cols} must be a positive multiple of 128")
    q, s = _mx_pair((rows, cols), nbytes, x.device, out)
    _lib.check(_lib.lib().fino_quantize_mxfp8(_p(x2), _p(q), _p(s), rows, cols, ldx, _dt(x), _stream()),
               "fino_quantize_mxfp8")
    return q, s


def ln_mxfp8(mode, x, weight=None, bias=None, shift=None, scale=None, sel=None, eps=1e-6, out=None):
    x2, rows, dim, ldx = _rows2d(x)
    nbytes = _lib.lib().fino_mxfp8_scale_bytes(rows, dim)
    if nbytes <= 0:
        raise ValueError(f"ln_mxfp8: dim={dim} must be a positive multiple of 128")
    q, s = _mx_pair((rows, dim), nbytes, x.device, out)
    for t in (weight, bias, shift, scale):
        assert t is None or t.dtype == torch.float32
    ms = shift.stride(0) if (shift is not None and shift.dim() == 2) else 0
    _lib.check(_lib.lib().fino_ln_mxfp8(mode, _p(x2), _p(q), _p(s), rows, dim, ldx, _p(weight), _p(bias), _p(shift),
                                       _p(scale), ms, _p(sel), eps, _dt(x), _stream()), "fino_ln_mxfp8")
    return q, s


def _mx_gemm(entry, aq, a_scales, wq, w_scales, bias, epilogue, residual, gate, sel, out, out_dtype, m, n, k):
    if out is None:
        out = torch.empty((m, n), dtype=out_dtype, device=aq.device)
    o2, _, _, ldc = _rows2d(out)
    r2, ldr, ms = _epi_operands(residual, gate)
    done = _timed_gemm(None, 2.0 * m * n * k)
    _lib.check(getattr(_lib.lib(), entry)(_p(aq), _p(a_scales), _p(wq), _p(w_scales), _p(bias), _p(o2), m, n, k, ldc,
                                          epilogue, _p(r2), ldr, _p(gate), ms, _p(sel), _dt(out), _stream()), entry)
    if done is not None:
        done()
    return out


def gemm_mxfp8(aq, a_scales, wq, w_scales, bias=None, epilogue=EPI_NONE, residual=None, gate=None, sel=None, out=None,
               out_dtype=torch.bfloat16):
    m, k = aq.shape
    n = wq.shape[0]
    assert wq.shape[1] == k and aq.dtype == torch.uint8 and wq.dtype == torch.uint8 and aq.is_contiguous() \
        and wq.is_contiguous()
    return _mx_gemm("fino_gemm_mxfp8", aq, a_scales, wq, w_scales, bias, epilogue, residual, gate, sel, out, out_dtype, m, n, k)


def gemm_mxfp8_q(aq, a_scales, wq, w_scales, bias, epilogue=EPI_NONE, out=None):
    m, k = aq.shape
    n = wq.shape[0]
    assert bias is not None and wq.shape[1] == k
    q, s = _mx_pair((m, n), _lib.lib().fino_mxfp8_scale_bytes(m, n), aq.device, out)
    done = _timed_gemm(None, 2.0 * m * n * k)
    _lib.check(_lib.lib().fino_gemm_mxfp8_q(_p(aq), _p(a_scales), _p(wq), _p(w_scales), _p(bias), _p(q), _p(s), m, n, k,
                                           epilogue, _dt(bias), _stream()), "fino_gemm_mxfp8_q")
    if done is not None:
        done()
    return q, s


def quantize_mxfp6(x, out=None):
    x2, rows, cols, ldx = _rows2d(x)
    nbytes = _lib.lib().fino_mxfp6_scale_bytes(rows, cols)
    if nbytes <= 0:
        raise ValueError(f"quantize_mxfp6: cols={cols} must be a positive multiple of 128")
    q, s = _mx_pair(_lib.lib().fino_mxfp6_bytes(rows, cols), nbytes, x.device, out)
    _lib.check(_lib.lib().fino_quantize_mxfp6(_p(x2), _p(q), _p(s), rows, cols, ldx, _dt(x), _stream()),
               "fino_quantize_mxfp6")
    q.mx_shape = (rows, cols)
    return q, s


def gemm_mxfp6(aq, a_scales, wq, w_scales, bias=None, epilogue=EPI_NONE, residual=None, gate=None, sel=None, out=None,
               out_dtype=torch.bfloat16, m=None, n=None, k=None):
    assert aq.dtype == torch.uint8 and wq.dtype == torch.uint8 and aq.is_contiguous() and wq.is_contiguous()
    sa_, sw_ = getattr(aq, "mx_shape", None), getattr(wq, "mx_shape", None)
    m = m if m is not None else (sa_[0] if sa_ else None)
    n = n if n is not None else (sw_[0] if sw_ else None)
    k = k if k is not None else (sa_[1] if sa_ else (sw_[1] if sw_ else None))
    if m is None or n is None or k is None:
        raise ValueError("gemm_mxfp6: operands without mx_shape need m / n / k")
    if sw_ and sw_[1] != k:
        raise ValueError(f"gemm_mxfp6: K of A ({k}) and of W ({sw_[1]}) differ")
    lib = _lib.lib()
    if aq.numel() != lib.fino_mxfp6_bytes(m, k) or wq.numel() != lib.fino_mxfp6_bytes(n, k):
        raise ValueError(f"gemm_mxfp6: operand sizes {aq.numel()} / {wq.numel()} do not match M={m} N={n} K={k}")
    return _mx_gemm("fino_gemm_mxfp6", aq, a_scales, wq, w_scales, bias, epilogue, residual, gate, sel, out, out_dtype, m, n, k)


def skinny_linear(x, w, b=None, silu_input=False):
    assert x.dtype == torch.float32 and x.dim() == 2 and x.is_contiguous() and w.is_contiguous()
    m, k = x.shape
    n = w.shape[0]
    wd = -1 if w.dtype == torch.float32 else _dt(w)
    if b is not None:
        assert b.dtype == w.dtype
    y = torch.empty((m, n), dtype=torch.float32, device=x.device)
    _lib.check(_lib.lib().fino_skinny_linear(_p(x), _p(w), _p(b), _p(y), m, n, k, wd, int(silu_input), _stream()),
               "fino_skinny_linear")
    return y


def patchify(x, patch, out=None):
    assert x.dim() == 4 and x.is_contiguous()
    c, f, h, w = x.shape
    pt, ph, pw = patch
    L = (f // pt) * (h // ph) * (w // pw)
    if out is None:
        out = torch.empty((L, c * pt * ph * pw), dtype=x.dtype, device=x.device)
    _lib.check(_lib.lib().fino_patchify(_p(x), _p(out), c, f, h, w, pt, ph, pw, out.stride(0), _dt(x), _stream()),
               "fino_patchify")
    return out


def unpatchify(y, cout, frames, height, width, patch, out=None):
    pt, ph, pw = patch
    if out is None:
        out = torch.empty((cout, frames, height, width), dtype=y.dtype, device=y.device)
    _lib.check(_lib.lib().fino_unpatchify(_p(y), _p(out), cout, frames, height, width, pt, ph, pw, y.stride(0), _dt(y),
                                         _stream()), "fino_unpatchify")
    return out


def wan_model_input(lat, cond, id_lat, traj, dtype, out=None):
    c, fg, h, w = lat.shape
    nid = 0 if id_lat is None else id_lat.shape[1]
    for t in (lat, cond, id_lat, traj):
        assert t is None or (t.dtype == torch.float32 and t.is_contiguous())
    assert traj.shape == (c, fg + nid, h, w) and cond.shape == (c, 1, h, w)
    if out is None:
        out = torch.empty((2 * c, fg + nid, h, w), dtype=dtype, device=lat.device)
    _lib.check(_lib.lib().fino_wan_model_input(_p(lat), _p(cond), _p(id_lat), _p(traj), _p(out), c, fg, nid, h, w,
                                              _dt(out), _stream()), "fino_wan_model_input")
    return out


def cfg_euler_step_(lat, cond_pred, uncond_pred, guidance, dt_dev, round_out=True):
    c, fg, h, w = lat.shape
    ft = cond_pred.shape[1]
    assert lat.dtype == torch.float32 and lat.is_contiguous() and cond_pred.is_contiguous()
    assert dt_dev.dtype == torch.float32 and dt_dev.is_cuda
    _lib.check(_lib.lib().fino_cfg_euler_step(_p(cond_pred), _p(uncond_pred), _p(lat), c, fg, ft, h, w, float(guidance),
                                             _p(dt_dev), int(round_out), _dt(cond_pred), _stream()),
               "fino_cfg_euler_step")
    return lat


def cfg_unipc_step_(x, last, m0, m1, cond_pred, uncond_pred, coef_dev):
    c, fg, h, w = x.shape
    ft = cond_pred.shape[1]
    for t in (x, last, m0, m1):
        assert t.dtype == torch.float32 and t.is_contiguous() and t.shape == x.shape
    assert coef_dev.dtype == torch.float32 and coef_dev.numel() >= 10 and cond_pred.is_contiguous()
    _lib.check(_lib.lib().fino_cfg_unipc_step(_p(cond_pred), _p(uncond_pred), _p(x), _p(last), _p(m0), _p(m1), c, fg,
                                             ft, h, w, _p(coef_dev), _dt(cond_pred), _stream()), "fino_cfg_unipc_step")
    return x


def cfg_vpred_step_(lat, pred, coef_dev, has_uncond=True):
    assert lat.is_contiguous() and pred.is_contiguous() and coef_dev.dtype == torch.float32 and lat.dtype == pred.dtype
    _lib.check(_lib.lib().fino_cfg_vpred_step(_p(pred), _p(lat), lat.numel(), pred[0].numel(), _p(coef_dev),
                                             int(has_uncond), _dt(lat), _stream()), "fino_cfg_vpred_step")
    return lat


def cfg_dpm_step_(lat, pred, x0_old, noise, coef_dev, has_uncond=True):
    assert lat.is_contiguous() and pred.is_contiguous() and noise.is_contiguous() and x0_old.is_contiguous()
    assert coef_dev.dtype == torch.float32 and coef_dev.numel() >= 9 and lat.dtype == pred.dtype == noise.dtype
    assert x0_old.dtype == torch.float32 and x0_old.numel() == lat.numel() == noise.numel()
    _lib.check(_lib.lib().fino_cfg_dpm_step(_p(pred), _p(lat), _p(x0_old), _p(noise), lat.numel(), pred[0].numel(),
                                           _p(coef_dev), int(has_uncond), _dt(lat), _stream()), "fino_cfg_dpm_step")
    return lat


_ZERO_PAGE = {}


def zero_page(device):
    z = _ZERO_PAGE.get(str(device))
    if z is None:
        z = _ZERO_PAGE[str(device)] = torch.zeros(256, dtype=torch.uint8, device=device)
    return z


def conv3d_cl(x, w2, bias, kernel, stride=(1, 1, 1), pad=(0, 0, 0), out_thw=None, upsample2x=False, residual=None,
              out=None):
    assert x.dim() == 4 and x.is_contiguous() and w2.is_contiguous()
    t, h, w, cin = x.shape
    kt, kh, kw = kernel
    cout = w2.shape[0]
    assert w2.shape[1] == kt * kh * kw * cin, (w2.shape, kernel, cin)
    if out_thw is None:
        up = 2 if upsample2x else 1
        out_thw = ((t + pad[0] - kt) // stride[0] + 1, (h * up + 2 * pad[1] - kh) // stride[1] + 1,
                   (w * up + 2 * pad[2] - kw) // stride[2] + 1)
    to, ho, wo = out_thw
    if out is None:
        out = torch.empty((to, ho, wo, cout), dtype=x.dtype, device=x.device)
    ev = _timed("conv3d")
    _lib.check(_lib.lib().fino_conv3d(_p(x), _p(w2), _p(bias), _p(out), t, h, w, cin, to, ho, wo, cout, kt, kh, kw,
                                     stride[0], stride[1], stride[2], pad[0], pad[1], pad[2], int(upsample2x),
                                     EPI_RESIDUAL if residual is not None else EPI_NONE, _p(residual),
                                     _p(zero_page(x.device)), _dt(x), _stream()), "fino_conv3d")
    if ev is not None:
        ev.record()
        kt_ = KernelTimer.active
        kt_.flops["conv3d"] = kt_.flops.get("conv3d", 0.0) + 2.0 * to * ho * wo * cout * w2.shape[1]
    return out


def rmsnorm_silu_cl(x, gamma, c_valid, silu=True, out=None):
    assert x.is_contiguous() and gamma.dtype == torch.float32
    cpad = x.shape[-1]
    rows = x.numel() // cpad
    out = torch.empty_like(x) if out is None else out
    _lib.check(_lib.lib().fino_rmsnorm_silu_cl(_p(x), _p(out), rows, c_valid, cpad, _p(gamma), int(silu), _dt(x),
                                              _stream()), "fino_rmsnorm_silu_cl")
    return out


def softmax_rows_(s, n, scale):
    assert s.dim() == 2 and s.stride(1) == 1
    _lib.check(_lib.lib().fino_softmax_rows(_p(s), s.shape[0], n, s.stride(0), float(scale), _dt3(s), _stream()),
               "fino_softmax_rows")
    return s


def dup_up3d_add(main, x, c_in, c_out, factor_t, factor_s):
    t, h, w, cin_pad = x.shape
    out = torch.empty_like(main)
    assert main.shape == (1 + (t - 1) * factor_t, h * factor_s, w * factor_s, main.shape[3])
    _lib.check(_lib.lib().fino_dup_up3d_add(_p(main), _p(x), _p(out), t, h, w, c_in, cin_pad, c_out, main.shape[3],
                                           factor_t, factor_s, _dt3(x), _stream()), "fino_dup_up3d_add")
    return out


def avg_down3d_add(main, x, c_in, c_out, factor_t, factor_s):
    t, h, w, cin_pad = x.shape
    out = torch.empty_like(main)
    _lib.check(_lib.lib().fino_avg_down3d_add(_p(main), _p(x), _p(out), t, h, w, c_in, cin_pad, c_out, main.shape[3],
                                             factor_t, factor_s, _dt3(x), _stream()), "fino_avg_down3d_add")
    return out


def vae_unpatchify_clamp(y, channels, patch):
    t, h, w, cpad = y.shape
    out = torch.empty((channels, t, h * patch, w * patch), dtype=torch.float32, device=y.device)
    _lib.check(_lib.lib().fino_vae_unpatchify_clamp(_p(y), _p(out), t, h, w, cpad, channels, patch, _dt3(y), _stream()),
               "fino_vae_unpatchify_clamp")
    return out


def vae_patchify(x, c_pad, patch, dtype):
    c, t, hp, wp = x.shape
    assert x.dtype == torch.float32 and x.is_contiguous()
    y = torch.empty((t, hp // patch, wp // patch, c_pad), dtype=dtype, device=x.device)
    _lib.check(_lib.lib().fino_vae_patchify(_p(x), _p(y), t, hp // patch, wp // patch, c_pad, c, patch, _dt3(y),
                                           _stream()), "fino_vae_patchify")
    return y


SPLIT_PRODUCTS = {2: ((0, 0), (0, 1), (1, 0)),
                  3: ((0, 0), (0, 1), (0, 2), (1, 0), (1, 1), (2, 0))}


def _pack_planes(planes):
    v = 0
    for i, q in enumerate(planes):
        v |= int(q) << (2 * i)
    return v


def split_bf16(x, layout, nplanes=3, out=None):
    assert x.dtype == torch.float32 and x.stride(-1) == 1
    x2 = x if x.dim() == 2 else x.reshape(-1, x.shape[-1])
    rows, cols = x2.shape
    prod = SPLIT_PRODUCTS[nplanes]
    planes = tuple(range(nplanes)) if layout == "planes" else tuple(p[0 if layout == "A" else 1] for p in prod)
    nseg = len(planes)
    if out is None:
        out = torch.empty(tuple(x.shape[:-1]) + (nseg * cols,), dtype=torch.bfloat16, device=x.device)
# ... 196 lines not shown
```

frameino_amd/transformer_wan.py:

```python
import contextlib
import math
import os
from types import SimpleNamespace

import torch
from torch import nn

from . import ops
from .attention_processor import Attention, MI355WanAttnProcessor
from .loading import FromPretrainedMixin
from .lora import LoraModelMixin
from .mx_linears import MXLinearsMixin
from .step_cache import FirstBlockCacheMixin


class _Config(dict):
    __getattr__ = dict.__getitem__


class _FP32LayerNormParams(nn.Module):

    def __init__(self, dim, eps, elementwise_affine):
        super().__init__()
        self.eps = eps
        if elementwise_affine:
            self.weight = nn.Parameter(torch.ones(dim))
            self.bias = nn.Parameter(torch.zeros(dim))
        else:
            self.register_parameter("weight", None)
            self.register_parameter("bias", None)


class _GELUProj(nn.Module):
    def __init__(self, dim_in, dim_out):
        super().__init__()
        self.proj = nn.Linear(dim_in, dim_out)


class FeedForward(nn.Module):

    def __init__(self, dim, inner_dim):
        super().__init__()
        self.net = nn.ModuleList([_GELUProj(dim, inner_dim), nn.Dropout(0.0), nn.Linear(inner_dim, dim)])


class _MLP2(nn.Module):
    def __init__(self, d_in, d_hidden, d_out=None):
        super().__init__()
        self.linear_1 = nn.Linear(d_in, d_hidden)
        self.linear_2 = nn.Linear(d_hidden, d_out or d_hidden)


class WanTimeTextImageEmbedding(nn.Module):

    def __init__(self, dim, time_freq_dim, time_proj_dim, text_embed_dim):
        super().__init__()
        self.time_embedder = _MLP2(time_freq_dim, dim)
        self.time_proj = nn.Linear(dim, time_proj_dim)
        self.text_embedder = _MLP2(text_embed_dim, dim)


def wan_rope_tables(head_dim, max_seq_len, ppf, pph, ppw, theta=10000.0):
    h_dim = w_dim = 2 * (head_dim // 6)
    t_dim = head_dim - h_dim - w_dim

    def axis(dim):
        freqs = 1.0 / (theta ** (torch.arange(0, dim, 2, dtype=torch.float64)[: dim // 2] / dim))
        ang = torch.outer(torch.arange(max_seq_len, dtype=torch.float64), freqs)
        return ang.cos().float(), ang.sin().float()

    (ct, st), (ch, sh), (cw, sw) = axis(t_dim), axis(h_dim), axis(w_dim)

    def build(t, h, w):
        a = t[:ppf].view(ppf, 1, 1, -1).expand(ppf, pph, ppw, -1)
        b = h[:pph].view(1, pph, 1, -1).expand(ppf, pph, ppw, -1)
        c = w[:ppw].view(1, 1, ppw, -1).expand(ppf, pph, ppw, -1)
        return torch.cat([a, b, c], dim=-1).reshape(ppf * pph * ppw, -1).contiguous()

    return build(ct, ch, cw), build(st, sh, sw)


class WanTransformerBlock(nn.Module):
    def __init__(self, dim, ffn_dim, num_heads, qk_norm="rms_norm_across_heads", cross_attn_norm=False, eps=1e-6):
        super().__init__()
        self.attn1 = Attention(dim, heads=num_heads, dim_head=dim // num_heads, qk_norm=qk_norm, eps=eps, bias=True,
                               out_bias=True, processor=MI355WanAttnProcessor())
        self.attn2 = Attention(dim, heads=num_heads, dim_head=dim // num_heads, qk_norm=qk_norm, eps=eps, bias=True,
                               out_bias=True, processor=MI355WanAttnProcessor())
        self.norm2 = _FP32LayerNormParams(dim, eps, True) if cross_attn_norm else None
        self.ffn = FeedForward(dim, ffn_dim)
        self.scale_shift_table = nn.Parameter(torch.randn(1, 6, dim) / dim ** 0.5)


class WanTransformer3DModel(nn.Module, FromPretrainedMixin, LoraModelMixin, FirstBlockCacheMixin, MXLinearsMixin):
    _loader_name = "load_wan_transformer"
    _keep_in_fp32_modules = ["time_embedder", "scale_shift_table", "norm1", "norm2", "norm3"]
    _lora_wan_layout = True

    def __init__(self, patch_size=(1, 2, 2), num_attention_heads=40, attention_head_dim=128, in_channels=16,
                 out_channels=16, text_dim=4096, freq_dim=256, ffn_dim=13824, num_layers=40, cross_attn_norm=True,
                 qk_norm="rms_norm_across_heads", eps=1e-6, image_dim=None, added_kv_proj_dim=None,
                 rope_max_seq_len=1024, pos_embed_seq_len=None):
        super().__init__()
        if image_dim is not None or added_kv_proj_dim is not None:
            raise NotImplementedError("Wan2.1 image-embedding branch is outside FrameINO's TI2V-5B path")
        self.config = _Config(patch_size=tuple(patch_size), num_attention_heads=num_attention_heads,
                              attention_head_dim=attention_head_dim, in_channels=in_channels,
                              out_channels=out_channels or in_channels, text_dim=text_dim, freq_dim=freq_dim,
                              ffn_dim=ffn_dim, num_layers=num_layers, cross_attn_norm=cross_attn_norm, qk_norm=qk_norm,
                              eps=eps, image_dim=image_dim, added_kv_proj_dim=added_kv_proj_dim,
                              rope_max_seq_len=rope_max_seq_len, pos_embed_seq_len=pos_embed_seq_len)
        inner = num_attention_heads * attention_head_dim
        self.inner_dim = inner
        self.patch_embedding = nn.Conv3d(in_channels, inner, kernel_size=patch_size, stride=patch_size)
        self.condition_embedder = WanTimeTextImageEmbedding(inner, freq_dim, inner * 6, text_dim)
        self.blocks = nn.ModuleList([WanTransformerBlock(inner, ffn_dim, num_attention_heads, qk_norm, cross_attn_norm,
                                                         eps) for _ in range(num_layers)])
        self.proj_out = nn.Linear(inner, self.config.out_channels * math.prod(patch_size))
        self.scale_shift_table = nn.Parameter(torch.randn(1, 2, inner) / inner ** 0.5)
        self._packed = None
        self._rope_cache = {}
        self._text_cache = {}
        self._ws = {}
        self._ctx_name = None
        self.ops = ops
        self.parallel = None
        self.dedup_shared_prefix = True
        self.fold_softmax_scale = False
        self.fp8_attention = False
        self.dedup_text_padding = os.environ.get("FINO_TEXT_FOLD", "1") != "0"
        self.reassociate_text_out = os.environ.get("FINO_TEXT_REASSOC", "1") != "0"
        self.skip_dead_rows = os.environ.get("FINO_SKIP_DEAD_ROWS", "1") != "0"

    @property
    def dtype(self):
        return self.proj_out.weight.dtype

    @property
    def device(self):
        return self.proj_out.weight.device

    @contextlib.contextmanager
    def cache_context(self, name):
        prev, self._ctx_name = self._ctx_name, name
        try:
            yield
        finally:
            self._ctx_name = prev

    @property
    def attn_processors(self):
        out = {}
        for i, blk in enumerate(self.blocks):
            out[f"blocks.{i}.attn1.processor"] = blk.attn1.processor
            out[f"blocks.{i}.attn2.processor"] = blk.attn2.processor
        return out

    def load_reference_state_dict(self, sd, dtype=None):
        own = self.state_dict()
        missing = [k for k in own if k not in sd]
        extra = [k for k in sd if k not in own]
        if missing or extra:
            raise KeyError(f"state-dict mismatch: missing {missing[:5]} unexpected {extra[:5]}")
        with torch.no_grad():
            for k, p in self.named_parameters():
                keep32 = any(s in k for s in self._keep_in_fp32_modules)
                t = sd[k].to(torch.float32 if keep32 else (dtype or sd[k].dtype))
                p.data = t.to(p.device).contiguous()
        self.reset_caches()
        return self

    def reset_caches(self):
        had_fp8 = self._mx_invalidate()
        self._reset_stateful_cache()
        self._packed = None
        self._text_cache.clear()
        self._rope_cache.clear()
        self._ws.clear()
        return had_fp8

    def _apply(self, fn, *args, **kwargs):
        out = super()._apply(fn, *args, **kwargs)
        if hasattr(self, "_text_cache"):
            self.reset_caches()
        return out

    def load_state_dict(self, *args, **kwargs):
        out = super().load_state_dict(*args, **kwargs)
        self.reset_caches()
        return out

    def _default_processors(self):
        return all(type(b.attn1.processor) is MI355WanAttnProcessor and type(b.attn2.processor) is MI355WanAttnProcessor
                   for b in self.blocks)

    def _pack(self):
        d = self.inner_dim
        pk = SimpleNamespace(layers=[])
        for blk in self.blocks:
            a1, a2 = blk.attn1, blk.attn2
            e = SimpleNamespace()
            e.wqkv = torch.cat([a1.to_q.weight, a1.to_k.weight, a1.to_v.weight]).detach().contiguous()
            e.bqkv = torch.cat([a1.to_q.bias, a1.to_k.bias, a1.to_v.bias]).detach().contiguous()
            e.wkv2 = torch.cat([a2.to_k.weight, a2.to_v.weight]).detach().contiguous()
            e.bkv2 = torch.cat([a2.to_k.bias, a2.to_v.bias]).detach().contiguous()
            pk.layers.append(e)
        pk.sst = torch.stack([b.scale_shift_table.detach().float()[0] for b in self.blocks])
        pk.w_patch = self.patch_embedding.weight.detach().reshape(d, -1).contiguous()
        self._packed = pk
        return pk

    def _mx_linear_weights(self, pk):
        for li, (blk, e) in enumerate(zip(self.blocks, pk.layers)):
            for key, w in (("qkv", e.wqkv), ("out", blk.attn1.to_out[0].weight), ("q2", blk.attn2.to_q.weight),
                           ("out2", blk.attn2.to_out[0].weight), ("ff1", blk.ffn.net[0].proj.weight),
                           ("ff2", blk.ffn.net[2].weight)):
                yield li, key, w

    def enable_fp8_attention(self, enabled=True, p_mode=None):
        self.fp8_attention = bool(enabled)
        self.fp8_p_mode = p_mode
        return self

    def _workspace(self, L, dtype, device):
        key = (L, dtype, str(device), self._ctx_name)
        ws = self._ws.get(key)
        if ws is None:
            d, f = self.inner_dim, self.config.ffn_dim
            mk = lambda *s: torch.empty(*s, dtype=dtype, device=device)
            ws = SimpleNamespace(x=mk(L, d), n=mk(L, d), qkv=mk(L, 3 * d), att=mk(L, d), q2=mk(L, d), ff=mk(L, f),
                                 a=mk(L, self.config.in_channels * math.prod(self.config.patch_size)),
                                 po=mk(L, self.config.out_channels * math.prod(self.config.patch_size)))
            self._ws = {k: v for k, v in self._ws.items() if k[:3] == key[:3]}
            self._ws[key] = ws
        return ws

    def _rope(self, ppf, pph, ppw, device):
        key = (ppf, pph, ppw, str(device))
        if key not in self._rope_cache:
            cos, sin = wan_rope_tables(self.config.attention_head_dim, self.config.rope_max_seq_len, ppf, pph, ppw)
            self._rope_cache[key] = (cos.to(device), sin.to(device))
        return self._rope_cache[key]

    def _time_rows(self, t_rows, act_dtype):
        ce = self.condition_embedder
        half = self.config.freq_dim // 2
        expo = torch.exp(-math.log(10000.0) * torch.arange(half, dtype=torch.float32, device=t_rows.device) / half)
        ang = t_rows.float()[:, None] * expo[None, :]
        sinus = torch.cat([torch.cos(ang), torch.sin(ang)], dim=-1)
        te = ce.time_embedder
        wd = te.linear_1.weight.dtype
        silu = torch.nn.functional.silu
        outs = []
        for i in range(0, sinus.shape[0], 16):
            s = sinus[i:i + 16].to(wd).float().contiguous()
            h = self.ops.skinny_linear(s, te.linear_1.weight, te.linear_1.bias).to(wd)
            h = silu(h).float().contiguous()
            e = self.ops.skinny_linear(h, te.linear_2.weight, te.linear_2.bias).to(wd)
            temb = e.to(act_dtype)
            a = silu(temb).float().contiguous()
            tp = self.ops.skinny_linear(a, ce.time_proj.weight, ce.time_proj.bias).to(ce.time_proj.weight.dtype)
            outs.append((temb, tp))
        temb = torch.cat([o[0] for o in outs])
        tproj = torch.cat([o[1] for o in outs]).unflatten(1, (6, -1))
        return temb, tproj

    def _qk_norm_rope(self, blk, qkv, d, cos, sin, dh, qfold):
        o, a = self.ops, blk.attn1
        if hasattr(o, "qkv_rmsnorm_rope_"):
            o.qkv_rmsnorm_rope_(qkv, d, a.norm_q.weight, a.norm_q.eps, a.norm_k.weight, a.norm_k.eps, cos, sin, dh,
                                q_out_scale=qfold.get("out_scale", 1.0))
        else:
            o.rmsnorm_rope_(qkv[:, :d], a.norm_q.weight, a.norm_q.eps, cos, sin, dh, **qfold)
            o.rmsnorm_rope_(qkv[:, d:2 * d], a.norm_k.weight, a.norm_k.eps, cos, sin, dh)

    def _text_tail(self, ehs, lq):
        o = self.ops
        b, lt, _ = ehs.shape
        if not (self.dedup_text_padding and hasattr(o, "attention_tail")):
            return None
        live = (ehs != 0).any(dim=-1)
        last = torch.where(live.any(dim=1), lt - 1 - live.flip(1).int().argmax(dim=1), torch.full((b,), -1, device=ehs.device))
        n_real = [int(x) + 1 for x in last.tolist()]
        if max(n_real) >= lt:
            return None
        keep = max(128, -(-(max(n_real) + 1) // 64) * 64)
        heads = self.config.num_attention_heads
        if keep > lt - 64 or not o.attention_tail_supported(b, heads, lq, keep, self.inner_dim // heads):
            return None
        return keep, [n + 1 for n in n_real], [float(lt - n) for n in n_real]

    def _text_out_weights(self, val, b, lq, pk):
        o, d = self.ops, self.inner_dim
        heads = self.config.num_attention_heads
        dh = d // heads
        lk_b = val.tail[0]
        kps = [-(-lk // 8) * 8 for lk in lk_b]
        dev, dt = val.txt.device, val.txt.dtype
        hidx = torch.arange(heads, device=dev)
        val.kp = kps
        val.pbuf = [torch.empty((lq, heads * kp), dtype=dt, device=dev) for kp in kps]
        val.rrms = torch.empty(b * lq, dtype=torch.float32, device=dev)
        val.w2 = []
        for li, blk in enumerate(self.blocks):
            kv = val.kv[li].view(b, val.lt, 2 * d)
            per_sample = []
            for i, kp in enumerate(kps):
                vblk = torch.zeros((heads, kp, heads, dh), dtype=dt, device=dev)
                vblk[hidx, :, hidx, :] = kv[i, :kp, d:].reshape(kp, heads, dh).permute(1, 0, 2)
                per_sample.append(o.gemm(blk.attn2.to_out[0].weight, vblk.view(heads * kp, d)))
            val.w2.append(per_sample)
        if dt == torch.float16:
            finite = torch.stack([torch.isfinite(w).all() for layer in val.w2 for w in layer]).all()
            if not bool(finite):
                val.w2, val.pbuf, val.rrms = None, None, None

    def _text_kv(self, encoder_hidden_states, pk, lq=0, may_fold=False):
        hit = self._text_cache.get(self._ctx_name)
        if hit is not None and hit[0] is encoder_hidden_states and hit[1] == encoder_hidden_states._version \
                and hit[3] == (bool(may_fold), int(lq) if may_fold else 0, self._mx_on, self.reassociate_text_out,
                               self.dedup_text_padding):
            return hit[2]
        ce = self.condition_embedder
        d = self.inner_dim
        tail = self._text_tail(encoder_hidden_states, lq) if may_fold else None
        kept = encoder_hidden_states if tail is None else encoder_hidden_states[:, :tail[0]].contiguous()
        ctx = kept.reshape(-1, kept.shape[-1])
        h = self.ops.gemm(ctx, ce.text_embedder.linear_1.weight, ce.text_embedder.linear_1.bias, self.ops.EPI_GELU_TANH)
        txt = self.ops.gemm(h, ce.text_embedder.linear_2.weight, ce.text_embedder.linear_2.bias)
        kvs = []
        for blk, e in zip(self.blocks, pk.layers):
            kv = self.ops.gemm(txt, e.wkv2, e.bkv2)
            self.ops.rmsnorm_rope_(kv[:, :d], blk.attn2.norm_k.weight, blk.attn2.norm_k.eps)
            kvs.append(kv)
        val = SimpleNamespace(txt=txt, kv=kvs, lt=kept.shape[1], tail=None if tail is None else (tail[1], tail[2]), w2=None)
        worth = tail is not None and self.config.num_attention_heads * (-(-max(tail[1]) // 8) * 8) <= 0.6 * d
        if worth and self.reassociate_text_out and not self._mx_on \
                and hasattr(self.ops, "attention_probs") \
                and self.ops.attention_probs_supported(1, self.config.num_attention_heads, lq, kept.shape[1],
                                                       d // self.config.num_attention_heads):
            self._text_out_weights(val, kept.shape[0], lq, pk)
        self._text_cache[self._ctx_name] = (encoder_hidden_states, encoder_hidden_states._version, val,
                                            (bool(may_fold), int(lq) if may_fold else 0, self._mx_on,
                                             self.reassociate_text_out, self.dedup_text_padding))
        return val

    @torch.no_grad()
    def forward(self, hidden_states, timestep, encoder_hidden_states, encoder_hidden_states_image=None,
                return_dict=True, attention_kwargs=None, timestep_rows=None, live_rows=None, _cache_contexts=None):
        gen = self.forward_steps(hidden_states, timestep, encoder_hidden_states, encoder_hidden_states_image,
                                 return_dict, attention_kwargs, timestep_rows, live_rows=live_rows,
                                 _cache_contexts=_cache_contexts)
        while True:
            try:
                next(gen)
            except StopIteration as done:
                return done.value

    def forward_steps(self, hidden_states, timestep, encoder_hidden_states, encoder_hidden_states_image=None,
                      return_dict=True, attention_kwargs=None, timestep_rows=None, shard=None, live_rows=None,
                      _cache_contexts=None):
        if encoder_hidden_states_image is not None:
            raise NotImplementedError("encoder_hidden_states_image: Wan2.1 branch, outside the TI2V-5B path")
        if attention_kwargs is not None:
            attention_kwargs = dict(attention_kwargs)
        self._lora_apply(attention_kwargs.pop("scale", None) if attention_kwargs is not None else None)
        b = hidden_states.shape[0]
        self._mx_requantise_if_pending()
        pk = self._packed or self._pack()
        default_procs = self._default_processors()
        o = self.ops
        cfg = self.config
        _, c, nf, hh, ww = hidden_states.shape
        pt, ph, pw = cfg.patch_size
        ppf, pph, ppw = nf // pt, hh // ph, ww // pw
        L = ppf * pph * ppw
        d, heads, dh = self.inner_dim, cfg.num_attention_heads, cfg.attention_head_dim
        dev, dt = hidden_states.device, hidden_states.dtype
        cos1, sin1 = self._rope(ppf, pph, ppw, dev)

        sh = shard if shard is not None else self.parallel
        sh = sh if (sh is not None and sh.active) else None
        if sh is not None:
            if b != 1:
                raise NotImplementedError("token-sharded execution runs one sample per call")
            lo, n, lpad = sh.rows(L)
            cos1, sin1 = cos1[lo:lo + n].contiguous(), sin1[lo:lo + n].contiguous()
        else:
            lo, n, lpad = 0, L, L
        if self.is_cache_enabled and sh is not None:
            raise NotImplementedError("first-block caching runs on one GPU: a token-sharded forward cannot take the cache")
        fbc = self._step_cache_segments(b, n, _cache_contexts)
        tk = {}
        if sh is not None and getattr(sh, "gemm_tile_m", 0):
            tk = {"tile_m": sh.tile_m_for(n) if hasattr(sh, "tile_m_for") else sh.gemm_tile_m}
        nr = b * n
        ws = self._workspace(b * lpad, dt, dev)
        if b == 1:
            cos, sin = cos1, sin1
        else:
            key = ("rope_b", ppf, pph, ppw, b, str(dev))
            if key not in self._rope_cache:
                self._rope_cache[key] = (cos1.repeat(b, 1).contiguous(), sin1.repeat(b, 1).contiguous())
            cos, sin = self._rope_cache[key]

        same_rows = False
        if timestep_rows is not None:
            t_rows, sel = timestep_rows
            same_rows = True
            if sel is not None and sh is not None:
                sel = sel[lo:lo + n].contiguous()
            if sel is not None and b > 1:
                sel = sel.repeat(b)
        elif timestep.ndim == 2:
            t_rows, inv = torch.unique(timestep.reshape(-1), return_inverse=True)
            sel = inv.to(torch.int32).contiguous()
            if sh is not None:
                sel = sel[lo:lo + n].contiguous()
            elif timestep.shape[0] == 1 and b > 1:
                sel = sel.repeat(b)
                same_rows = True
        else:
            t_rows = timestep.reshape(-1)
            sel = None if b == 1 else torch.arange(b, device=dev, dtype=torch.int32).repeat_interleave(n)
            if t_rows.numel() == 1 and b > 1:
                sel = None
                same_rows = True
        temb, tproj = self._time_rows(t_rows.to(dev), encoder_hidden_states.dtype)
        mod = (pk.sst[None] + tproj.float()[:, None]).contiguous()
        head = (self.scale_shift_table.float() + temb.float()[:, None]).contiguous()

        text = self._text_kv(encoder_hidden_states, pk, lq=n, may_fold=default_procs)
        lt = text.lt

        shared = (self.dedup_shared_prefix and b > 1 and sh is None and hidden_states.stride(0) == 0 and default_procs
                  and same_rows)
        if b == 1 or shared:
            a_rows = o.patchify(hidden_states[0], cfg.patch_size)[lo:lo + n]
        else:
            a_rows = torch.cat([o.patchify(hidden_states[i], cfg.patch_size) for i in range(b)])
        x = ws.x[:nr]
        o.gemm(a_rows, pk.w_patch, self.patch_embedding.bias, out=x[:n] if shared else x, **tk)
        if fbc is not None:
            if getattr(ws, "fbc_h0", None) is None:
                ws.fbc_h0, ws.fbc_h1 = torch.empty_like(ws.x), torch.empty_like(ws.x)
            h0, h1c = ws.fbc_h0[:nr], ws.fbc_h1[:nr]
            if shared:
                for bi in range(b):
                    h0[bi * n:(bi + 1) * n].copy_(x[:n])
            else:
                h0.copy_(x)
        nrm, att, q2, ff = ws.n[:nr], ws.att[:nr], ws.q2[:nr], ws.ff[:nr]
        fold = self.fold_softmax_scale and hasattr(o, "SCALE_FOLDED")
        qfold = {"out_scale": dh ** -0.5 * o.LOG2E} if fold else {}
        afold = {"scale": o.SCALE_FOLDED} if fold else {}
        attend = o.attention
        if self.fp8_attention and sh is None and hasattr(o, "attention_fp8"):
            def attend(q_, k_, v_, heads_, **kw_):
                return o.attention_fp8(q_, k_, v_, heads_, p_mode=getattr(self, "fp8_p_mode", None), **kw_)
        yield

        live = None
        if (live_rows is not None and self.skip_dead_rows and default_procs and sh is None and len(self.blocks) > 1
                and not self._fp8 and attend is o.attention):
            l0, l1 = int(live_rows[0]), int(live_rows[1])
            if 0 <= l0 < l1 <= n and (l1 - l0) < n:
                live = (l0, l1)
        segs = [(0, nr)]
        for li, (blk, e) in enumerate(zip(self.blocks, pk.layers)):
            m = mod[:, li]
            last_live = live is not None and li == len(self.blocks) - 1
            if last_live:
                segs = [(bi * n + live[0], bi * n + live[1]) for bi in range(b)]
            once = shared and li == 0
            xq1 = None
            if not once:
                if default_procs and sh is None:
                    xq1 = self._ln_q(li, "qkv", 0, x, shift=m[:, 0], scale=m[:, 1], sel=sel, eps=cfg.eps)
                if xq1 is None:
                    o.adaln_modulate(x, m[:, 0], m[:, 1], sel, cfg.eps, out=nrm)
            if not default_procs:
                if sh is not None:
                    raise NotImplementedError("token-sharded execution needs the built-in MI355WanAttnProcessor")
                rot = _CompactRope((cos1, sin1))
                a = blk.attn1(nrm.view(b, n, d), rotary_emb=rot, **(attention_kwargs or {}))
                o.gated_residual(x, a.reshape(nr, d), m[:, 2], sel, out=x)
            elif sh is None and shared and li == 0:
                n1, q1, sel1 = nrm[:n], ws.qkv[:n], (None if sel is None else sel[:n])
                o.adaln_modulate(x[:n], m[:, 0], m[:, 1], sel1, cfg.eps, out=n1)
                self._lin(li, "qkv", n1, e.wqkv, e.bqkv, out=q1)
                self._qk_norm_rope(blk, q1, d, cos1, sin1, dh, qfold)
                q3 = q1.view(1, n, 3 * d)
                attend(q3[:, :, :d], q3[:, :, d:2 * d], q3[:, :, 2 * d:], heads, out=att[:n].view(1, n, d), **afold)
                self._lin(li, "out", att[:n], blk.attn1.to_out[0].weight, blk.attn1.to_out[0].bias, o.EPI_GATED_RESIDUAL,
                          residual=x[:n], gate=m[:, 2], sel=sel1, out=x[:n])
                for bi in range(1, b):
                    x[bi * n:(bi + 1) * n].copy_(x[:n])
            elif sh is None:
                qkv = ws.qkv[:nr]
                self._lin(li, "qkv", nrm, e.wqkv, e.bqkv, xq=xq1, out=qkv)
                self._qk_norm_rope(blk, qkv, d, cos, sin, dh, qfold)
                q3 = qkv.view(b, n, 3 * d)
                if last_live:
                    attend(q3[:, live[0]:live[1], :d], q3[:, :, d:2 * d], q3[:, :, 2 * d:], heads,
                           out=att.view(b, n, d)[:, live[0]:live[1]], **afold)
                else:
                    attend(q3[:, :, :d], q3[:, :, d:2 * d], q3[:, :, 2 * d:], heads, out=att.view(b, n, d), **afold)
            elif sh.heads_exchange_ok(heads):
                ways = sh.ways
                hp = heads // ways
                dp = hp * dh
                qkv = ws.qkv[:n]
                self._lin(li, "qkv", nrm, e.wqkv, e.bqkv, out=qkv, **tk)
                lay = sh.heads_send_layout(heads, dh, lpad, dt, dev) if hasattr(o, "qkv_rmsnorm_rope_") else None
                if lay is not None:
                    o.qkv_rmsnorm_rope_(qkv, d, blk.attn1.norm_q.weight, blk.attn1.norm_q.eps, blk.attn1.norm_k.weight,
                                        blk.attn1.norm_k.eps, cos, sin, dh, q_out_scale=qfold.get("out_scale", 1.0),
                                        out=lay.flat, head_off=lay.off_qkv, head_ld=lay.ld)
                else:
                    o.rmsnorm_rope_(qkv[:, :d], blk.attn1.norm_q.weight, blk.attn1.norm_q.eps, cos, sin, dh, **qfold)
                    o.rmsnorm_rope_(qkv[:, d:2 * d], blk.attn1.norm_k.weight, blk.attn1.norm_k.eps, cos, sin, dh)
                    q4 = qkv.view(n, 3, ways, dp)
                inflight = []
                for gi, (h0, h1) in enumerate(sh.head_ranges(hp)):
                    dg = (h1 - h0) * dh
                    if lay is not None:
                        send = lay.views[gi]
                    else:
                        send = sh.a2a_buffer(f"qkv_send{gi}", (ways, lpad, 3, dg), dt, dev)
                        send[:, :n].copy_(q4[:, :, :, h0 * dh:h1 * dh].permute(2, 0, 1, 3))
                    inflight.append((gi, h0, h1, dg) + sh.all_to_all(f"qkv_recv{gi}", send, async_op=True))
                orl = (sh.heads_recv_layout(heads, dh, lpad, dt, dev)
                       if (not self._fp8 and hasattr(o, "gemm_blocked_a") and hasattr(sh, "heads_recv_layout")) else None)
                back = []
                for gi, h0, h1, dg, recv, work in inflight:
                    if work is not None:
                        work.wait()
                    r3 = recv.view(1, ways * lpad, 3 * dg)[:, :L]
                    oh = sh.a2a_buffer(f"o_send{gi}", (ways, lpad, dg), dt, dev)
                    o.attention(r3[:, :, :dg], r3[:, :, dg:2 * dg], r3[:, :, 2 * dg:], h1 - h0,
                                out=oh.view(1, ways * lpad, dg)[:, :L], **afold)
                    back.append((h0, h1) + sh.all_to_all(f"o_recv{gi}", oh, async_op=True))
                if orl is not None and all(orv.data_ptr() == orl[gi].data_ptr() for gi, (_, _, orv, _) in enumerate(back)):
                    for _, _, _, work in back:
                        if work is not None:
                            work.wait()
                    o.gemm_blocked_a(orl, n, blk.attn1.to_out[0].weight, blk.attn1.to_out[0].bias, x, m[:, 2], sel, out=x,
                                     **tk)
                    once = True
                else:
                    a3 = att.view(n, ways, dp)
                    for h0, h1, orv, work in back:
                        if work is not None:
                            work.wait()
                        a3[:, :, h0 * dh:h1 * dh].copy_(orv[:, :n].permute(1, 0, 2))
            elif (hasattr(sh, "kv_groups") and sh.kv_groups(heads) > 1 and hasattr(o, "rmsnorm_rope_scatter")
                  and hasattr(sh, "kv_group_layout")):
                kv_loc = sh.kv_local(lpad, 2 * d, dt, dev)
                lay = sh.kv_group_layout(heads, dh, lpad, dt, dev)
                if sh.fused_qkv_ok() and not self._fp8:
                    o.gemm(nrm, e.wqkv, e.bqkv, out=q2, out2=kv_loc[:n], split=d, **tk)
                else:
                    self._lin(li, "kv", nrm, e.wqkv[d:], e.bqkv[d:], out=kv_loc[:n], **tk)
                o.rmsnorm_rope_scatter(kv_loc[:n, :d], blk.attn1.norm_k.weight, blk.attn1.norm_k.eps, cos, sin, dh, lay.flat,
                                       lay.off_k, lay.ld)
                o.rmsnorm_rope_scatter(kv_loc[:n, d:], None, 0.0, None, None, dh, lay.flat, lay.off_v, lay.ld)
                flying = [sh._all_gather(f"kv_all_g{gi}", v_, True) for gi, v_ in enumerate(lay.views)]
                if not (sh.fused_qkv_ok() and not self._fp8):
                    self._lin(li, "q", nrm, e.wqkv[:d], e.bqkv[:d], out=q2, **tk)
                o.rmsnorm_rope_(q2, blk.attn1.norm_q.weight, blk.attn1.norm_q.eps, cos, sin, dh, **qfold)
                q3, a3 = q2.view(1, n, d), att.view(1, n, d)
                for (h0, h1), (kv_all, work) in zip(lay.ranges, flying):
                    if work is not None:
                        work.wait()
                    dg = (h1 - h0) * dh
                    kv3 = kv_all.view(1, -1, 2 * dg)[:, :L]
                    o.attention(q3[:, :, h0 * dh:h1 * dh], kv3[:, :, :dg], kv3[:, :, dg:], h1 - h0,
                                out=a3[:, :, h0 * dh:h1 * dh], **afold)
            else:
                kv_loc = sh.kv_local(lpad, 2 * d, dt, dev)
                if sh.fused_qkv_ok() and not self._fp8:
                    o.gemm(nrm, e.wqkv, e.bqkv, out=q2, out2=kv_loc[:n], split=d, **tk)
                    o.rmsnorm_rope_(kv_loc[:n, :d], blk.attn1.norm_k.weight, blk.attn1.norm_k.eps, cos, sin, dh)
                    kv_all, work = sh.all_gather_kv(kv_loc)
                else:
                    self._lin(li, "kv", nrm, e.wqkv[d:], e.bqkv[d:], out=kv_loc[:n], **tk)
                    o.rmsnorm_rope_(kv_loc[:n, :d], blk.attn1.norm_k.weight, blk.attn1.norm_k.eps, cos, sin, dh)
                    kv_all, work = sh.all_gather_kv(kv_loc)
                    self._lin(li, "q", nrm, e.wqkv[:d], e.bqkv[:d], out=q2, **tk)
                o.rmsnorm_rope_(q2, blk.attn1.norm_q.weight, blk.attn1.norm_q.eps, cos, sin, dh, **qfold)
                if sh.local_first():
                    qv = q2.view(1, n, d)
                    pf = o.attention_partial_floats(1, heads, n, dh) if hasattr(o, "attention_partial_floats") else 0
                    parts = [o.attention_partial(qv, kv_loc[:n, :d][None], kv_loc[:n, d:][None], heads,
                                                 out=sh.partial_buf(0, pf, dev), **afold)]
                    if work is not None:
                        work.wait()
                    kv3 = kv_all.view(1, -1, 2 * d)
                    for pi, (k0, k1) in enumerate(((0, lo), (lo + lpad, L))):
                        if k1 > k0:
                            parts.append(o.attention_partial(qv, kv3[:, k0:k1, :d], kv3[:, k0:k1, d:], heads,
                                                             out=sh.partial_buf(1 + pi, pf, dev), **afold))
                    o.attention_merge(parts, 1, n, heads, dh, dt, out=att.view(1, n, d))
                else:
                    if work is not None:
                        work.wait()
                    kv3 = kv_all.view(1, -1, 2 * d)[:, :L]
                    o.attention(q2.view(1, n, d), kv3[:, :, :d], kv3[:, :, d:], heads, out=att.view(1, n, d), **afold)
            if default_procs and not once:
                for r0, r1 in segs:
                    self._lin(li, "out", att[r0:r1], blk.attn1.to_out[0].weight, blk.attn1.to_out[0].bias, o.EPI_GATED_RESIDUAL,
                              residual=x[r0:r1], gate=m[:, 2], sel=None if sel is None else sel[r0:r1], out=x[r0:r1], **tk)
            n2 = blk.norm2
            xq2 = self._ln_q(li, "q2", 1, x, weight=n2.weight, bias=n2.bias, eps=cfg.eps) if (n2 is not None and
                                                                                                default_procs) else None
            if xq2 is not None:
                pass
            elif n2 is not None:
                for r0, r1 in segs:
                    o.layernorm(x[r0:r1], n2.weight, n2.bias, cfg.eps, out=nrm[r0:r1])
            else:
                nrm.copy_(x)
            if default_procs:
                for r0, r1 in segs:
                    self._lin(li, "q2", nrm[r0:r1], blk.attn2.to_q.weight, blk.attn2.to_q.bias, xq=xq2, out=q2[r0:r1], **tk)
                kv = text.kv[li].view(b, lt, 2 * d)
                s0, s1 = (live if last_live else (0, n))
                if text.w2 is not None:
                    rr = text.rrms
                    for r0, r1 in segs:
                        o.row_rrms(q2[r0:r1], blk.attn2.norm_q.eps, out=rr[r0:r1])
                    for i in range(b):
                        r0, r1 = i * n + s0, i * n + s1
                        pr = o.attention_probs(q2[r0:r1].view(1, s1 - s0, d), kv[i:i + 1, :, :d], heads, text.tail[0][i:i + 1],
                                               text.tail[1][i:i + 1], text.kp[i], out=text.pbuf[i][:s1 - s0].view(1, s1 - s0, -1),
                                               q_rrms=rr[r0:r1].view(1, s1 - s0), q_weight=blk.attn2.norm_q.weight)
                        xi = x[r0:r1]
                        o.gemm(pr.view(s1 - s0, -1), text.w2[li][i], blk.attn2.to_out[0].bias, o.EPI_RESIDUAL, residual=xi, out=xi, **tk)
                else:
                    for r0, r1 in segs:
                        o.rmsnorm_rope_(q2[r0:r1], blk.attn2.norm_q.weight, blk.attn2.norm_q.eps)
                    qv, av = q2.view(b, n, d)[:, s0:s1], att.view(b, n, d)[:, s0:s1]
                    if text.tail is not None:
                        o.attention_tail(qv, kv[:, :, :d], kv[:, :, d:], heads, text.tail[0], text.tail[1], out=av)
                    else:
                        o.attention(qv, kv[:, :, :d], kv[:, :, d:], heads, out=av)
                    for r0, r1 in segs:
                        self._lin(li, "out2", att[r0:r1], blk.attn2.to_out[0].weight, blk.attn2.to_out[0].bias, o.EPI_RESIDUAL,
                                  residual=x[r0:r1], out=x[r0:r1], **tk)
            else:
                a = blk.attn2(nrm.view(b, n, d), encoder_hidden_states=text.txt.view(b, lt, d),
                              **(attention_kwargs or {}))
                o.gated_residual(x, a.reshape(nr, d), out=x)
            xq3 = (self._ln_q(li, "ff1", 0, x, shift=m[:, 3], scale=m[:, 4], sel=sel, eps=cfg.eps)
                   if (li, "ff2") in self._fp8 else None)
            if xq3 is None:
                for r0, r1 in segs:
                    o.adaln_modulate(x[r0:r1], m[:, 3], m[:, 4], None if sel is None else sel[r0:r1], cfg.eps, out=nrm[r0:r1])
            if self._ffn_mxfp8(li, nrm, xq3, blk.ffn.net[0].proj.bias, blk.ffn.net[2].bias, o.EPI_GATED_RESIDUAL, residual=x,
                               gate=m[:, 5], sel=sel, out=x) is None:
                for r0, r1 in segs:
                    self._lin(li, "ff1", nrm[r0:r1], blk.ffn.net[0].proj.weight, blk.ffn.net[0].proj.bias, o.EPI_GELU_TANH,
                              out=ff[r0:r1], **tk)
                    self._lin(li, "ff2", ff[r0:r1], blk.ffn.net[2].weight, blk.ffn.net[2].bias, o.EPI_GATED_RESIDUAL,
                              residual=x[r0:r1], gate=m[:, 5], sel=None if sel is None else sel[r0:r1], out=x[r0:r1], **tk)
            if fbc is not None and li == 0:
                computes = self._step_cache_probe(fbc, h0, x, h1c)
            yield
            if fbc is not None and not any(computes):
                break

        if fbc is not None:
            self._step_cache_finish(fbc, computes, x, h1c)
            if live is not None:
                segs = [(bi * n + live[0], bi * n + live[1]) for bi in range(b)]

        for r0, r1 in segs:
            o.adaln_modulate(x[r0:r1], head[:, 0], head[:, 1], None if sel is None else sel[r0:r1], cfg.eps, out=nrm[r0:r1])
        if sh is None:
            po = ws.po[:nr]
            if live is not None:
                po.zero_()
            for r0, r1 in segs:
                o.gemm(nrm[r0:r1], self.proj_out.weight, self.proj_out.bias, out=po[r0:r1])
        else:
            po_loc = sh.out_local(lpad, ws.po.shape[1], dt, dev)
            o.gemm(nrm, self.proj_out.weight, self.proj_out.bias, out=po_loc[:n], **tk)
            po = sh.all_gather_out(po_loc)[:L]
        if b == 1:
            out = o.unpatchify(po, cfg.out_channels, nf, hh, ww, cfg.patch_size)[None]
        else:
            po3 = po.view(b, L, -1)
            out = torch.stack([o.unpatchify(po3[i], cfg.out_channels, nf, hh, ww, cfg.patch_size) for i in range(b)])
        if not return_dict:
            return (out,)
        return SimpleNamespace(sample=out)


class _CompactRope(tuple):
    compact = True
```

include/frameino_hip.h:

```cpp
#ifndef FRAMEINO_HIP_H
#define FRAMEINO_HIP_H
#include <stdint.h>

#ifdef __cplusplus
extern "C" {
#endif

#define FINO_VERSION 103

enum { FINO_BF16 = 0, FINO_F16 = 1, FINO_F32 = 2 };
enum {
    FINO_OK = 0,
    FINO_ERR_ARG = -1,
    FINO_ERR_LAUNCH = -2,
    FINO_ERR_UNSUPPORTED = -3
};

int fino_version(void);
const char* fino_last_error(void);

enum { FINO_TUNE_GEMM_GROUP_M = 0, FINO_TUNE_GEMM_RASTER = 1, FINO_TUNE_CONV_LOOP = 2, FINO_TUNE_GEMM_TILE_M = 3,
       FINO_TUNE_ATTN_KERNEL = 4, FINO_TUNE_ATTN_FP8_KERNEL = 5, FINO_TUNE_ATTN_WALK_GRID = 6, FINO_TUNE_COUNT = 8 };
int fino_tune_set(int key, int value);
int fino_tune_get(int key);

int fino_adaln_modulate(const void* x, void* y, int64_t rows, int dim, int64_t ldx, int64_t ldy,
                        const float* shift, const float* scale, int64_t mod_stride, const int32_t* sel,
                        float eps, int dtype, void* stream);

int fino_layernorm(const void* x, void* y, int64_t rows, int dim, int64_t ldx, int64_t ldy, const float* w,
                   const float* b, float eps, int dtype, void* stream);

int fino_gated_residual(const void* x, const void* y, void* out, int64_t rows, int dim, int64_t ldx, int64_t ldy,
                        int64_t ldo, const float* gate, int64_t mod_stride, const int32_t* sel, int dtype,
                        void* stream);

int fino_gated_residual_staged(const void* x, const void* y, void* out, int64_t rows, int dim, int64_t ldx, int64_t ldy,
                               int64_t ldo, const float* gate, int64_t mod_stride, const int32_t* sel, int dtype,
                               void* stream);

int fino_layernorm_zero(const void* x, void* y, int64_t rows, int dim, int64_t ldx, int64_t ldy, const float* w,
                        const float* b, const float* shift, const float* scale, int64_t mod_stride, const int32_t* sel,
                        float eps, int dtype, void* stream);

int fino_ln_mxfp8(int mode, const void* x, void* q, void* scales, int64_t rows, int dim, int64_t ldx, const float* w,
                  const float* b, const float* shift, const float* scale, int64_t mod_stride, const int32_t* sel,
                  float eps, int dtype, void* stream);

int fino_rmsnorm_rope(void* x, int64_t rows, int dim, int64_t ldx, const void* weight, float eps,
                      const float* cos_t, const float* sin_t, int head_dim, int dtype, void* stream);
int fino_rmsnorm_rope_scaled(void* x, int64_t rows, int dim, int64_t ldx, const void* weight, float eps,
                             const float* cos_t, const float* sin_t, int head_dim, float out_scale, int dtype,
                             void* stream);

int fino_rmsnorm_rope_scatter(const void* x, int64_t rows, int dim, int64_t ldx, const void* weight, float eps,
                              const float* cos_t, const float* sin_t, int head_dim, float out_scale, void* out,
                              const int64_t* head_off, const int64_t* head_ld, int dtype, void* stream);

int fino_qkv_rmsnorm_rope(void* qkv, int64_t rows, int dim, int64_t ldx, const void* q_weight, float q_eps,
                          const void* k_weight, float k_eps, const float* cos_t, const float* sin_t, int head_dim,
                          float q_out_scale, void* out, const int64_t* head_off, const int64_t* head_ld, int dtype,
                          void* stream);

int fino_headnorm_rope(void* x, int batch, int64_t rows, int heads, int head_dim, int64_t ldx, int64_t batch_stride,
                       const void* w, const void* b, float eps, const float* cos_t, const float* sin_t,
                       int64_t rope_row0, int dtype, void* stream);
int fino_headnorm_rope_scaled(void* x, int batch, int64_t rows, int heads, int head_dim, int64_t ldx,
                              int64_t batch_stride, const void* w, const void* b, float eps, const float* cos_t,
                              const float* sin_t, int64_t rope_row0, float out_scale, int dtype, void* stream);

#define FINO_ATTN_SCALE_FOLDED (-1.0f)
int fino_attn_fwd(const void* q, const void* k, const void* v, void* o, int batch, int heads, int64_t lq,
                  int64_t lk, int head_dim, int64_t q_bs, int64_t q_rs, int64_t q_hs, int64_t k_bs, int64_t k_rs,
                  int64_t k_hs, int64_t v_bs, int64_t v_rs, int64_t v_hs, int64_t o_bs, int64_t o_rs,
                  int64_t o_hs, float scale, int dtype, void* stream);
enum { FINO_FP8_P_EXP2 = 0, FINO_FP8_P_RAMP = 1 };
int64_t fino_attn_fp8_kv_bytes(int batch, int heads, int64_t lk, int head_dim);
int fino_attn_fwd_fp8(const void* q, const void* k, const void* v, void* o, int batch, int heads, int64_t lq, int64_t lk,
                      int head_dim, int64_t q_bs, int64_t q_rs, int64_t k_bs, int64_t k_rs, int64_t v_bs, int64_t v_rs,
                      int64_t o_bs, int64_t o_rs, float scale, int dtype, int p_mode, void* kv_workspace,
                      int64_t kv_workspace_bytes, void* stream);

int fino_attn_tail_supported(int batch, int heads, int64_t lq, int64_t lk, int head_dim);
int fino_attn_fwd_tail(const void* q, const void* k, const void* v, void* o, int batch, int heads, int64_t lq, int64_t lk,
                       int head_dim, int64_t q_bs, int64_t q_rs, int64_t q_hs, int64_t k_bs, int64_t k_rs, int64_t k_hs,
                       int64_t v_bs, int64_t v_rs, int64_t v_hs, int64_t o_bs, int64_t o_rs, int64_t o_hs, float scale,
                       int dtype, const int* lk_b, const float* tail_mult, void* stream);

int fino_attn_probs_supported(int batch, int heads, int64_t lq, int64_t lk, int head_dim);
int fino_attn_probs(const void* q, const void* k, void* p, int batch, int heads, int64_t lq, int64_t lk, int head_dim,
                    int64_t q_bs, int64_t q_rs, int64_t q_hs, int64_t k_bs, int64_t k_rs, int64_t k_hs, int kp, int64_t p_bs,
                    int64_t p_rs, float scale, int dtype, const int* lk_b, const float* tail_mult, const float* q_rrms,
                    int64_t q_rrms_bs, const void* q_weight, void* stream);
int fino_row_rrms(const void* x, int64_t rows, int dim, int64_t ldx, float eps, float* rrms, int dtype, void* stream);

int64_t fino_attn_partial_bytes(int batch, int heads, int64_t lq, int head_dim);
int fino_attn_partial(const void* q, const void* k, const void* v, int batch, int heads, int64_t lq, int64_t lk,
                      int head_dim, int64_t q_bs, int64_t q_rs, int64_t q_hs, int64_t k_bs, int64_t k_rs, int64_t k_hs,
                      int64_t v_bs, int64_t v_rs, int64_t v_hs, float scale, int dtype, void* partial,
                      int64_t partial_bytes, void* stream);
int fino_attn_merge(void* o, int batch, int heads, int64_t lq, int head_dim, int64_t o_bs, int64_t o_rs, int64_t o_hs,
                    const void* part0, const void* part1, const void* part2, int dtype, void* stream);


int64_t fino_attn_workspace_bytes(int batch, int heads, int64_t lq, int64_t lk, int head_dim);
int fino_attn_fwd_ws(const void* q, const void* k, const void* v, void* o, int batch, int heads, int64_t lq,
                     int64_t lk, int head_dim, int64_t q_bs, int64_t q_rs, int64_t q_hs, int64_t k_bs, int64_t k_rs,
                     int64_t k_hs, int64_t v_bs, int64_t v_rs, int64_t v_hs, int64_t o_bs, int64_t o_rs, int64_t o_hs,
                     float scale, int dtype, void* workspace, int64_t workspace_bytes, void* stream);

enum { FINO_EPI_NONE = 0, FINO_EPI_GELU_TANH = 1, FINO_EPI_RESIDUAL = 2, FINO_EPI_GATED_RESIDUAL = 3,
       FINO_EPI_GATED_RESIDUAL_STAGED = 4, FINO_EPI_F32 = 5, FINO_EPI_F32_RESIDUAL = 6 };
int fino_gemm(const void* a, const void* w, const void* bias, void* c, int64_t m, int64_t n, int64_t k,
              int64_t lda, int64_t ldw, int64_t ldc, int epilogue, const void* r, int64_t ldr, const float* gate,
              int64_t mod_stride, const int32_t* sel, int dtype, void* stream);
int fino_gemm_split_n(const void* a, const void* w, const void* bias, void* c, int64_t m, int64_t n, int64_t k, int64_t lda,
                      int64_t ldw, int64_t ldc, int epilogue, const void* r, int64_t ldr, const float* gate,
                      int64_t mod_stride, const int32_t* sel, int dtype, void* c2, int64_t ldc2, int64_t n_split,
                      int tile_m, void* stream);
int fino_gemm_blocked_a(const void* a, const void* w, const void* bias, void* c, int64_t m, int64_t n, int64_t k,
                        int64_t a_block_k, int64_t a_block_stride, int a_groups, int64_t a_group_stride, int64_t lda,
                        int64_t ldw, int64_t ldc, const void* r, int64_t ldr, const float* gate, int64_t mod_stride,
                        const int32_t* sel, int dtype, int tile_m, void* stream);

int fino_gemm_plan(int64_t m, int64_t n, int64_t* rows_256, int* tile_rows_rest);
int fino_skinny_linear(const float* x, const void* w, const void* b, float* y, int m, int64_t n, int64_t k,
                       int w_dtype, int silu_input, void* stream);

int fino_patchify(const void* x, void* a, int channels, int frames, int height, int width, int pt, int ph, int pw,
                  int64_t lda, int dtype, void* stream);
int fino_unpatchify(const void* y, void* out, int cout, int frames, int height, int width, int pt, int ph, int pw,
                    int64_t ldy, int dtype, void* stream);

int fino_wan_model_input(const float* lat, const float* cond, const float* id_lat, const float* traj, void* out,
                         int channels, int gen_frames, int id_frames, int height, int width, int dtype, void* stream);
int fino_cfg_euler_step(const void* cond_pred, const void* uncond_pred, float* lat, int channels, int gen_frames,
                        int total_frames, int height, int width, float guidance, const float* dt_dev, int round_out,
                        int dtype, void* stream);

int fino_cfg_unipc_step(const void* cond_pred, const void* uncond_pred, float* x, float* last, float* m0, float* m1,
                        int channels, int gen_frames, int total_frames, int height, int width, const float* coef_dev,
                        int dtype, void* stream);

int fino_cfg_vpred_step(const void* pred, void* lat, int64_t n_lat, int64_t batch_stride, const float* coef_dev,
                        int has_uncond, int dtype, void* stream);

int fino_cfg_dpm_step(const void* pred, void* lat, float* x0_old, const void* noise, int64_t n_lat, int64_t batch_stride,
                      const float* coef_dev, int has_uncond, int dtype, void* stream);

int fino_conv3d(const void* x, const void* w, const void* bias, void* y, int t_in, int h_in, int w_in, int c_in_pad,
                int t_out, int h_out, int w_out, int c_out_pad, int kt, int kh, int kw, int st, int sh, int sw, int pt,
                int ph, int pw, int upsample2x, int epilogue, const void* r, const void* zero_page, int dtype,
                void* stream);
int fino_rmsnorm_silu_cl(const void* x, void* y, int64_t rows, int c_valid, int c_pad, const float* gamma, int silu,
                         int dtype, void* stream);
int fino_softmax_rows(void* s, int64_t rows, int n, int64_t ld, float scale, int dtype, void* stream);
int fino_dup_up3d_add(const void* main_in, const void* x, void* out, int t_in, int h_in, int w_in, int c_in,
                      int c_in_pad, int c_out, int c_out_pad, int factor_t, int factor_s, int dtype, void* stream);
int fino_avg_down3d_add(const void* main_in, const void* x, void* out, int t_in, int h_in, int w_in, int c_in,
                        int c_in_pad, int c_out, int c_out_pad, int factor_t, int factor_s, int dtype, void* stream);
int fino_vae_unpatchify_clamp(const void* y, float* out, int t, int h, int w, int c_pad, int channels, int patch,
                              int dtype, void* stream);
int fino_vae_patchify(const float* x, void* y, int t, int h, int w, int c_pad, int channels, int patch, int dtype,
                      void* stream);
int fino_split_bf16(const float* x, void* out, int64_t rows, int cols, int64_t ldx, int64_t ldo, int nseg,
                    unsigned planes_packed, void* stream);
int fino_rmsnorm_silu_cl_f32(const float* x, void* y, int64_t rows, int c_valid, int c_pad, const float* gamma, int silu,
                             int nseg, unsigned planes_packed, void* stream);
int fino_conv3d_split(const void* x_planes, const void* w_products, const float* bias, float* y, int t_in, int h_in, int w_in,
                      int c_in_pad, int planes, int t_out, int h_out, int w_out, int c_out_pad, int kt, int kh, int kw, int st,
                      int sh, int sw, int pt, int ph, int pw, int upsample2x, int epilogue, const float* r,
                      const void* zero_page, void* stream);

int64_t fino_mxfp8_scale_bytes(int64_t rows, int64_t cols);
int fino_quantize_mxfp8(const void* x, void* q, void* scales, int64_t rows, int64_t cols, int64_t ldx, int dtype,
                        void* stream);
int fino_gemm_mxfp8(const void* aq, const void* a_scales, const void* wq, const void* w_scales, const void* bias,
                    void* c, int64_t m, int64_t n, int64_t k, int64_t ldc, int epilogue, const void* r, int64_t ldr,
                    const float* gate, int64_t mod_stride, const int32_t* sel, int out_dtype, void* stream);
int fino_gemm_mxfp8_q(const void* aq, const void* a_scales, const void* wq, const void* w_scales, const void* bias,
                      void* cq, void* c_scales, int64_t m, int64_t n, int64_t k, int epilogue, int bias_dtype,
                      void* stream);

int64_t fino_mxfp6_bytes(int64_t rows, int64_t cols);
int64_t fino_mxfp6_scale_bytes(int64_t rows, int64_t cols);
int fino_quantize_mxfp6(const void* x, void* q, void* scales, int64_t rows, int64_t cols, int64_t ldx, int dtype,
                        void* stream);
int fino_gemm_mxfp6(const void* aq, const void* a_scales, const void* wq, const void* w_scales, const void* bias,
                    void* c, int64_t m, int64_t n, int64_t k, int64_t ldc, int epilogue, const void* r, int64_t ldr,
                    const float* gate, int64_t mod_stride, const int32_t* sel, int out_dtype, void* stream);

int fino_traj_paint(const int32_t* points, const int32_t* frame_offsets, float* canvas, int frames, int height, int width,
                    int radius, void* stream);
int fino_traj_blur_quantize(const float* canvas, float* scratch, float* out, const float* taps_dev, int taps, int planes,
                            int height, int width, void* stream);


int64_t fino_groupnorm_workspace_bytes(int c_pad);
int fino_groupnorm_cl(const void* x, void* y, int t, int h, int w, int channels, int c_pad, int groups,
                      const float* gamma, const float* beta, float eps, const void* mod_scale, const void* mod_shift,
                      int tz, int hz, int wz, int silu, void* workspace, int64_t workspace_bytes, int dtype,
                      void* stream);
int fino_avg_pool_time2(const void* x, void* y, int t_in, int h, int w, int c_pad, int dtype, void* stream);
int fino_vae_blend_tiles(const void* a, void* b, int t, int h_a, int w_a, int h_b, int w_b, int c_pad, int extent, int axis,
                         int dtype, void* stream);

int fino_resize_area_pad_u8(const void* src, void* dst, int src_h, int src_w, int region_h, int region_w, int out_h,
                            int out_w, int off_y, int off_x, int fill, void* stream);
int fino_u8_hwc_to_chw_unit(const void* src, float* dst, int height, int width, void* stream);

enum { FINO_LORA_MAX_ADAPTERS = 8, FINO_LORA_MAX_TOTAL_RANK = 1024 };
int fino_lora_merge(const void* w_base, int64_t ldw_base, void* w_out, int64_t ldw_out, int64_t n, int64_t k,
                    int n_adapters, const void* const* a, const int64_t* lda, const void* const* b, const int64_t* ldb,
                    const int* rank, const float* scale, int dtype, void* stream);

typedef struct {
    const void* h0;
    const void* h1;
    const void* p;
    void* r;
    void* h1_copy;
    int64_t rows, ld_h0, ld_h1, ld_p, ld_r, ld_h1_copy;
} FinoStepCacheSegment;
enum { FINO_STEP_CACHE_MAX_SEGMENTS = 4, FINO_STEP_CACHE_BLOCKS = 1024,
       FINO_STEP_CACHE_WORKSPACE_FLOATS = 2 * FINO_STEP_CACHE_MAX_SEGMENTS * FINO_STEP_CACHE_BLOCKS };
int fino_step_cache_probe(const FinoStepCacheSegment* segs, int nseg, int64_t dim, float* sums, float* workspace, int dtype,
                          void* stream);
int fino_step_cache_residual(const void* a, int64_t lda, const void* b, int64_t ldb, void* out, int64_t ldo, int64_t rows,
                             int64_t dim, int subtract, int dtype, void* stream);

int fino_diag_mfma_peak(int kind, int waves_per_simd, int iters, void* scratch, double* flops, void* stream);

#ifdef __cplusplus
}
#endif
#endif
```

Before: 3.766 denoise-steps/s.

## Batch text cross-attention tail into one multi-sample probs kernel and grouped GEMM

Replaces the per-sample loop over cond/uncond in the text cross-attention tail with a single multi-sample attention-probs kernel that processes all samples and heads in one launch. Each sample gets its own key length, padding and tail multiplier. The per-sample output projection GEMMs become one grouped GEMM launch with residual epilogue. When a single query pass suffices, the layernorm, q projection and rrms are also computed once over the shared rows rather than per segment. The goal is to cut kernel launch count and fill the GPU better on small per-sample problems, at the cost of new kernels with more complex indexing and per-sample parameter tables.

```diff
diff --git a/frameino_amd/_lib.py b/frameino_amd/_lib.py
--- a/frameino_amd/_lib.py
+++ b/frameino_amd/_lib.py
@@ -46,6 +46,9 @@
     "fino_attn_probs": [c_void_p] * 3 + [c_int, c_int, c_i64, c_i64, c_int] + [c_i64] * 6 + [c_int, c_i64, c_i64, c_float, c_int,
                                                                                          c_void_p, c_void_p, c_void_p, c_i64,
                                                                                          c_void_p, c_void_p],
+    "fino_attn_probs_multi": [c_void_p] * 3 + [c_int, c_int, c_i64, c_i64, c_int] + [c_i64] * 6 + [c_void_p, c_void_p, c_float, c_int,
+                                                                                               c_void_p, c_void_p, c_void_p, c_i64,
+                                                                                               c_void_p, c_int, c_void_p],
     "fino_row_rrms": [c_void_p, c_i64, c_int, c_i64, c_float, c_void_p, c_int, c_void_p],
     "fino_attn_fp8_kv_bytes": [c_int, c_int, c_i64, c_int],
     "fino_attn_fwd_fp8": [c_void_p] * 4 + [c_int, c_int, c_i64, c_i64, c_int] + [c_i64] * 8 + [c_float, c_int, c_int, c_void_p,
@@ -78,6 +81,7 @@
                       c_void_p, c_float, c_int, c_void_p],
     "fino_gemm_blocked_a": [c_void_p, c_void_p, c_void_p, c_void_p, c_i64, c_i64, c_i64, c_i64, c_i64, c_int, c_i64, c_i64, c_i64,
                             c_i64, c_void_p, c_i64, c_void_p, c_i64, c_void_p, c_int, c_int, c_void_p],
+    "fino_gemm_grouped": [c_int] + [c_void_p] * 5 + [c_i64] + [c_void_p] * 4 + [c_int, c_void_p, c_void_p, c_int, c_void_p],
     "fino_gemm_plan": [c_i64, c_i64, ctypes.POINTER(c_i64), ctypes.POINTER(c_int)],
     "fino_skinny_linear": [c_void_p, c_void_p, c_void_p, c_void_p, c_int, c_i64, c_i64, c_int, c_int, c_void_p],
     "fino_patchify": [c_void_p, c_void_p] + [c_int] * 7 + [c_i64, c_int, c_void_p],
diff --git a/frameino_amd/csrc/fino_attention_probs.hip b/frameino_amd/csrc/fino_attention_probs.hip
--- a/frameino_amd/csrc/fino_attention_probs.hip
+++ b/frameino_amd/csrc/fino_attention_probs.hip
@@ -140,6 +140,190 @@
         const uint4 u = *reinterpret_cast<const uint4*>(stage + rr * 256 + ((pc ^ (rr & 15)) << 4));
         if (row_base + rr < p.lq) *reinterpret_cast<uint4*>(pbase + (int64_t)(row_base + rr) * p.p_rs + pc * 8) = u;
     }
+}
+
+struct ProbsMultiParams {
+    const uint16_t* q[4];
+    const float* rrms[4];
+    const uint16_t* k[4];
+    uint16_t* p[4];
+    int64_t p_rs[4];
+    int lk_b[4], kp[4];
+    float log2_mult[4];
+    const uint16_t* q_weight;
+    int64_t q_rs, q_hs, k_rs, k_hs;
+    int heads, lq, lk, walk;
+    float scale_log2;
+};
+
+__device__ __forceinline__ void probs_wave_lds_fence() {
+    __builtin_amdgcn_fence(__ATOMIC_ACQ_REL, "wavefront");
+    __builtin_amdgcn_wave_barrier();
+}
+
+template <typename T, int NKB>
+__device__ __forceinline__ void probs_walk(const ProbsMultiParams& p, const char* kimg, char* stage, const uint16_t* qh,
+                                           const uint16_t* wh, const float* rrms, uint16_t* pbase, const int64_t p_rs, const int lkc, const float lm,
+                                           const int kp, const int nb, const int blk0, const int blk1, const int lane, const int wave) {
+    typedef typename T::vec8 vec8;
+    const int r = lane & 31;
+    const int h = lane >> 5;
+    const int lrow = lane >> 4, lch = lane & 15;
+    const int nkb = (lkc + 31) >> 5;
+    float ww[8];
+    if (rrms) unpack8<T>(*reinterpret_cast<const uint4*>(wh + lch * 8), ww);
+    uint4 u[8];
+    float rs[8];
+    auto load_block = [&](int blk) {
+#pragma unroll
+        for (int i = 0; i < 8; ++i) {
+            const int row = blk * 128 + wave * 32 + 4 * i + lrow;
+            const int rc = row < p.lq ? row : p.lq - 1;
+            u[i] = *reinterpret_cast<const uint4*>(qh + (int64_t)rc * p.q_rs + lch * 8);
+            rs[i] = rrms ? rrms[rc] : 0.f;
+        }
+    };
+    load_block(blk0);
+    for (int blk = blk0; blk < blk1; ++blk) {
+        const int row_base = blk * 128 + wave * 32;
+        if (row_base >= p.lq) break;
+#pragma unroll
+        for (int i = 0; i < 8; ++i) {
+            uint4 v = u[i];
+            if (rrms) {
+                float f[8];
+                unpack8<T>(v, f);
+#pragma unroll
+                for (int j = 0; j < 8; ++j) f[j] = round_to<T>(round_to<T>(f[j] * rs[i]) * ww[j]);
+                v = pack8<T>(f);
+            }
+            const int rl = 4 * i + lrow;
+            *reinterpret_cast<uint4*>(stage + rl * 256 + ((lch ^ (rl & 15)) << 4)) = v;
+        }
+        if (blk + 1 < blk1) load_block(blk + 1);
+        probs_wave_lds_fence();
+        vec8 qf[8];
+#pragma unroll
+        for (int ks = 0; ks < 8; ++ks)
+            qf[ks] = __builtin_bit_cast(vec8, *reinterpret_cast<const uint4*>(stage + r * 256 + (((2 * ks + h) ^ (r & 15)) << 4)));
+        probs_wave_lds_fence();
+
+        int koff = 0;
+        asm volatile("" : "+s"(koff));
+        const char* kblk = kimg + koff;
+        f32x16_t acc[NKB];
+#pragma unroll
+        for (int kb = 0; kb < NKB; ++kb) {
+            if (kb < nkb) {
+#pragma unroll
+                for (int ks = 0; ks < 8; ++ks) {
+                    const int row = kb * 32 + r;
+                    const uint4 a = *reinterpret_cast<const uint4*>(kblk + row * 256 + (((2 * ks + h) ^ (row & 15)) << 4));
+                    if (ks == 0) {
+                        f32x16_t z;
+#pragma unroll
+                        for (int j = 0; j < 16; ++j) z[j] = 0.f;
+                        acc[kb] = T::mfma32(__builtin_bit_cast(vec8, a), qf[ks], z);
+                    } else {
+                        acc[kb] = T::mfma32(__builtin_bit_cast(vec8, a), qf[ks], acc[kb]);
+                    }
+                }
+            }
+        }
+        int lkc_blk = lkc;
+        asm volatile("" : "+s"(lkc_blk));
+        const float c2 = p.scale_log2;
+        float m = -INFINITY;
+#pragma unroll
+        for (int kb = 0; kb < NKB; ++kb) {
+            if (kb >= nb) continue;
+            if (kb >= nkb) {
+#pragma unroll
+                for (int j = 0; j < 16; ++j) acc[kb][j] = -INFINITY;
+                continue;
+            }
+#pragma unroll
+            for (int j = 0; j < 16; ++j) {
+                const int key = kb * 32 + (j & 3) + 8 * (j >> 2) + 4 * h;
+                float x = acc[kb][j] * c2;
+                x = key == lkc_blk - 1 ? x + lm : x;
+                x = key >= lkc_blk ? -INFINITY : x;
+                acc[kb][j] = x;
+                m = fmaxf(m, x);
+            }
+        }
+        {
+            const auto sw = __builtin_amdgcn_permlane32_swap(__float_as_uint(m), __float_as_uint(m), false, false);
+            m = fmaxf(__uint_as_float(sw[0]), __uint_as_float(sw[1]));
+        }
+        float l = 0.f;
+#pragma unroll
+        for (int kb = 0; kb < NKB; ++kb) {
+            if (kb >= nb) continue;
+#pragma unroll
+            for (int j = 0; j < 16; ++j) {
+                const float e = __builtin_amdgcn_exp2f(acc[kb][j] - m);
+                acc[kb][j] = e;
+                l += e;
+            }
+        }
+        {
+            const auto sw = __builtin_amdgcn_permlane32_swap(__float_as_uint(l), __float_as_uint(l), false, false);
+            l = __uint_as_float(sw[0]) + __uint_as_float(sw[1]);
+        }
+        const float inv = 1.0f / l;
+#pragma unroll
+        for (int kb = 0; kb < NKB; ++kb) {
+#pragma unroll
+            for (int g4 = 0; g4 < 4; ++g4) {
+                const int key0 = kb * 32 + 8 * g4 + 4 * h;
+                if (kb < nb && key0 < kp) {
+                    const uint32_t w0 = (uint32_t)T::from_f32(acc[kb][4 * g4 + 0] * inv) | ((uint32_t)T::from_f32(acc[kb][4 * g4 + 1] * inv) << 16);
+                    const uint32_t w1 = (uint32_t)T::from_f32(acc[kb][4 * g4 + 2] * inv) | ((uint32_t)T::from_f32(acc[kb][4 * g4 + 3] * inv) << 16);
+                    *reinterpret_cast<uint2*>(stage + r * 256 + ((((key0 >> 3)) ^ (r & 15)) << 4) + ((key0 & 4) << 1)) = make_uint2(w0, w1);
+                }
+            }
+        }
+        probs_wave_lds_fence();
+        const int pieces = kp >> 3;
+        const int total = 32 * pieces;
+        for (int i = lane; i < total; i += 64) {
+            const int rr = i / pieces, pc = i - rr * pieces;
+            const uint4 v = *reinterpret_cast<const uint4*>(stage + rr * 256 + ((pc ^ (rr & 15)) << 4));
+            if (row_base + rr < p.lq) *reinterpret_cast<uint4*>(pbase + (int64_t)(row_base + rr) * p_rs + pc * 8) = v;
+        }
+        probs_wave_lds_fence();
+    }
+}
+
+template <typename T, int NKBMAX>
+__global__ __launch_bounds__(256, 2) void attn_probs_multi_kernel(const ProbsMultiParams p) {
+    extern __shared__ __attribute__((aligned(16))) char smem_multi[];
+    const int tid = threadIdx.x;
+    const int lane = tid & 63;
+    const int wave = __builtin_amdgcn_readfirstlane(tid >> 6);
+    const int s = blockIdx.y / p.heads;
+    const int head = blockIdx.y - s * p.heads;
+    const int lkc = p.lk_b[s];
+    const int nkb = (lkc + 31) >> 5;
+    const uint16_t* kp_ = p.k[s] + head * p.k_hs;
+    for (int i = 0; i < nkb * 2; ++i) {
+        const int c = tid + 256 * i;
+        const int row = c >> 4, ch = c & 15;
+        uint4 u = make_uint4(0, 0, 0, 0);
+        if (row < p.lk) u = *reinterpret_cast<const uint4*>(kp_ + (int64_t)row * p.k_rs + ch * 8);
+        *reinterpret_cast<uint4*>(smem_multi + row * 256 + ((ch ^ (row & 15)) << 4)) = u;
+    }
+    __syncthreads();
+    char* stage = smem_multi + NKBMAX * 8192 + wave * 8192;
+    const int nblk = (p.lq + 127) >> 7;
+    const int blk0 = blockIdx.x * p.walk;
+    const int blk1 = blk0 + p.walk < nblk ? blk0 + p.walk : nblk;
+    const uint16_t* qh = p.q[s] + head * p.q_hs;
+    uint16_t* pbase = p.p[s] + head * p.kp[s];
+    const int nb = (p.kp[s] + 31) >> 5;
+    probs_walk<T, NKBMAX>(p, smem_multi, stage, qh, p.q_weight + head * 128, p.rrms[s], pbase, p.p_rs[s], lkc, p.log2_mult[s],
+                          p.kp[s], nb, blk0, blk1, lane, wave);
 }
 
 }
@@ -200,3 +384,74 @@
     FINO_LAUNCH_CHECK();
     return FINO_OK;
 }
+
+template <typename T, int NKBMAX>
+static int launch_probs_multi(const ProbsMultiParams& pp, dim3 grid, hipStream_t st) {
+    static FinoPerDeviceOnce once;
+    const int smem = (NKBMAX + 4) * 8192;
+    if (int rc = fino_max_smem_once(once, reinterpret_cast<const void*>(&attn_probs_multi_kernel<T, NKBMAX>), smem, "fino_attn_probs_multi"))
+        return rc;
+    attn_probs_multi_kernel<T, NKBMAX><<<grid, 256, smem, st>>>(pp);
+    FINO_LAUNCH_CHECK();
+    return FINO_OK;
+}
+
+extern "C" int fino_attn_probs_multi(const void* q, const void* k, void* const* p, int batch, int heads, int64_t lq, int64_t lk,
+                                     int head_dim, int64_t q_bs, int64_t q_rs, int64_t q_hs, int64_t k_bs, int64_t k_rs,
+                                     int64_t k_hs, const int* kp, const int64_t* p_rs, float scale, int dtype, const int* lk_b,
+                                     const float* tail_mult, const float* q_rrms, int64_t q_rrms_bs, const void* q_weight,
+                                     int walk, void* stream) {
+    FINO_CHECK((q_rrms == nullptr) == (q_weight == nullptr) && fino_aligned16(q_weight), FINO_ERR_ARG,
+               "fino_attn_probs_multi: q_rrms and q_weight come together (q_weight 16-byte aligned)");
+    FINO_CHECK(dtype == FINO_BF16 || dtype == FINO_F16, FINO_ERR_ARG, "fino_attn_probs_multi: dtype %d", dtype);
+    FINO_CHECK(q && k && p && kp && p_rs && lk_b && tail_mult, FINO_ERR_ARG, "fino_attn_probs_multi: null pointer");
+    FINO_CHECK(fino_attn_probs_supported(batch, heads, lq, lk, head_dim), FINO_ERR_UNSUPPORTED,
+               "fino_attn_probs_multi: needs head_dim 128, batch <= 4, lk <= 128 (got head_dim %d, batch %d, lk %lld)", head_dim,
+               batch, (long long)lk);
+    FINO_CHECK(fino_aligned16(q) && fino_aligned16(k) && q_rs % 8 == 0 && k_rs % 8 == 0 && q_hs % 8 == 0 && k_hs % 8 == 0 &&
+                   q_bs % 8 == 0 && k_bs % 8 == 0 && q_bs >= 0 && q_rrms_bs >= 0,
+               FINO_ERR_ARG, "fino_attn_probs_multi: pointers and strides must be 16-byte aligned");
+    FINO_CHECK(scale > 0.f || scale == FINO_ATTN_SCALE_FOLDED, FINO_ERR_ARG, "fino_attn_probs_multi: scale");
+    FINO_CHECK(walk >= 0, FINO_ERR_ARG, "fino_attn_probs_multi: walk %d", walk);
+    if (lq == 0) return FINO_OK;
+    ProbsMultiParams pp = {};
+    int max_kp = 0;
+    for (int b = 0; b < batch; ++b) {
+        FINO_CHECK(p[b] && fino_aligned16(p[b]) && p_rs[b] % 8 == 0 && kp[b] > 0 && kp[b] % 8 == 0 && kp[b] <= 128 &&
+                       p_rs[b] >= (int64_t)heads * kp[b],
+                   FINO_ERR_ARG, "fino_attn_probs_multi: sample %d: kp %d (a multiple of 8, <= 128), row stride %lld, p 16-byte aligned",
+                   b, kp[b], (long long)p_rs[b]);
+        FINO_CHECK(lk_b[b] >= 1 && lk_b[b] <= lk && lk_b[b] <= kp[b] && tail_mult[b] >= 1.0f, FINO_ERR_ARG,
+                   "fino_attn_probs_multi: lk_b[%d] = %d (of %lld, kp %d), tail_mult %g", b, lk_b[b], (long long)lk, kp[b],
+                   (double)tail_mult[b]);
+        pp.q[b] = (const uint16_t*)q + b * q_bs;
+        pp.rrms[b] = q_rrms ? q_rrms + b * q_rrms_bs : nullptr;
+        pp.k[b] = (const uint16_t*)k + b * k_bs;
+        pp.p[b] = (uint16_t*)p[b];
+        pp.p_rs[b] = p_rs[b];
+        pp.lk_b[b] = lk_b[b];
+        pp.kp[b] = kp[b];
+        pp.log2_mult[b] = log2f(tail_mult[b]);
+        max_kp = kp[b] > max_kp ? kp[b] : max_kp;
+    }
+    pp.q_weight = (const uint16_t*)q_weight;
+    pp.q_rs = q_rs; pp.q_hs = q_hs; pp.k_rs = k_rs; pp.k_hs = k_hs;
+    pp.heads = heads; pp.lq = (int)lq; pp.lk = (int)lk;
+    pp.scale_log2 = scale == FINO_ATTN_SCALE_FOLDED ? 1.0f : scale * 1.4426950408889634f;
+    const int64_t nblk = (lq + 127) / 128;
+    if (walk == 0) walk = (int)((nblk * batch * heads + 1023) / 1024);
+    walk = walk < 1 ? 1 : walk;
+    pp.walk = (int)(walk < nblk ? walk : nblk);
+    const dim3 grid((unsigned)((nblk + pp.walk - 1) / pp.walk), (unsigned)(batch * heads));
+    hipStream_t st = (hipStream_t)stream;
+    const int nkb = (max_kp + 31) / 32;
+#define PROBS_MULTI(T_)                                                      \
+    switch (nkb) {                                                           \
+        case 1: return launch_probs_multi<T_, 1>(pp, grid, st);              \
+        case 2: return launch_probs_multi<T_, 2>(pp, grid, st);              \
+        case 3: return launch_probs_multi<T_, 3>(pp, grid, st);              \
+        default: return launch_probs_multi<T_, 4>(pp, grid, st);             \
+    }
+    if (dtype == FINO_BF16) PROBS_MULTI(BF16) else PROBS_MULTI(F16)
+#undef PROBS_MULTI
+}
diff --git a/frameino_amd/csrc/fino_gemm.hip b/frameino_amd/csrc/fino_gemm.hip
--- a/frameino_amd/csrc/fino_gemm.hip
+++ b/frameino_amd/csrc/fino_gemm.hip
@@ -536,6 +536,75 @@
     gemm_epilogue<T, EPI, false, MI>(acc, p, smem, m0, n0, tid, lane, wm, wn);
 }
 
+constexpr int kGroupMaxProblems = 4, kGroupMaxSegs = 2 * kGroupMaxProblems;
+struct GemmGroupSeg {
+    const uint16_t* a;
+    const uint16_t* w;
+    const uint16_t* bias;
+    const uint16_t* r;
+    uint16_t* c;
+    int64_t m, k, lda, ldw, ldc, ldr;
+    int tiles_m, mi, start, group_m;
+};
+struct GemmGroupParams {
+    int64_t n;
+    int tiles_n, nseg;
+    GemmGroupSeg seg[kGroupMaxSegs];
+};
+
+template <typename T, int EPI, int MI>
+__device__ __forceinline__ void gemm_group_tile(const GemmParams& p, char* smem, const int64_t m0, const int64_t n0, const int tid,
+                                                const int lane, const int wave, const int wm, const int wn) {
+    f32x4_t acc[MI][4];
+    pp_mainloop<T, false, MI>(p, smem, m0, n0, 0, (int)(p.k / BK), acc, tid, lane, wave, wm, wn);
+    gemm_epilogue<T, EPI, false, MI>(acc, p, smem, m0, n0, tid, lane, wm, wn);
+}
+
+template <typename T, int EPI>
+__global__ __launch_bounds__(kThreads, 2) void gemm_pp_grouped_kernel(const GemmGroupParams gp) {
+    extern __shared__ __attribute__((aligned(16))) char smem[];
+    const int tid = threadIdx.x;
+    const int lane = tid & 63;
+    const int wave = __builtin_amdgcn_readfirstlane(tid >> 6);
+    const int wm = wave >> 2;
+    const int wn = wave & 3;
+    int s = 0;
+#pragma unroll
+    for (int i = 1; i < kGroupMaxSegs; ++i)
+        if (i < gp.nseg && (int)blockIdx.x >= gp.seg[i].start) s = i;
+    const GemmGroupSeg& g = gp.seg[s];
+    GemmParams p = {};
+    p.a = g.a; p.w = g.w; p.bias = g.bias; p.r = g.r; p.c = g.c;
+    p.m = g.m; p.n = gp.n; p.k = g.k; p.lda = g.lda; p.ldw = g.ldw; p.ldc = g.ldc; p.ldr = g.ldr;
+    p.tiles_m = g.tiles_m; p.tiles_n = gp.tiles_n; p.group_m = g.group_m;
+    int tm, tn;
+    tile_raster(p, xcd_remap((int)blockIdx.x - g.start, p.tiles_m * p.tiles_n), tm, tn);
+    const int64_t m0 = (int64_t)tm * (32 * g.mi), n0 = (int64_t)tn * BN;
+    int mi = g.mi;
+    if (mi == 8) {
+        const int64_t rows = p.m - m0;
+        mi = rows <= 64 ? 2 : (rows <= 128 ? 4 : 8);
+    }
+    switch (mi) {
+        case 2: gemm_group_tile<T, EPI, 2>(p, smem, m0, n0, tid, lane, wave, wm, wn); break;
+        case 3: gemm_group_tile<T, EPI, 3>(p, smem, m0, n0, tid, lane, wave, wm, wn); break;
+        case 4: gemm_group_tile<T, EPI, 4>(p, smem, m0, n0, tid, lane, wave, wm, wn); break;
+        case 5: gemm_group_tile<T, EPI, 5>(p, smem, m0, n0, tid, lane, wave, wm, wn); break;
+        case 6: gemm_group_tile<T, EPI, 6>(p, smem, m0, n0, tid, lane, wave, wm, wn); break;
+        case 7: gemm_group_tile<T, EPI, 7>(p, smem, m0, n0, tid, lane, wave, wm, wn); break;
+        default: gemm_group_tile<T, EPI, 8>(p, smem, m0, n0, tid, lane, wave, wm, wn); break;
+    }
+}
+
+template <typename T, int EPI>
+int launch_gemm_grouped(const GemmGroupParams& gp, int total, hipStream_t st) {
+    static FinoPerDeviceOnce once;
+    if (int rc = fino_max_smem_once(once, reinterpret_cast<const void*>(&gemm_pp_grouped_kernel<T, EPI>), kSmemBytes, "fino_gemm_grouped")) return rc;
+    gemm_pp_grouped_kernel<T, EPI><<<dim3((unsigned)total), kThreads, kSmemBytes, st>>>(gp);
+    FINO_LAUNCH_CHECK();
+    return FINO_OK;
+}
+
 template <typename T, int EPI, bool GENERIC, bool CONV = false>
 int launch_gemm_t(const GemmParams& p, hipStream_t st) {
     static FinoPerDeviceOnce once;
@@ -750,6 +819,75 @@
     if (rows_256) *rows_256 = tp.rows1;
     if (tile_rows_rest) *tile_rows_rest = tp.rows1 < m ? 32 * tp.mi2 : 0;
     return FINO_OK;
+}
+
+extern "C" int fino_gemm_grouped(int count, const void* const* a, const void* const* w, const void* const* bias, void* const* c,
+                                 const int64_t* m, int64_t n, const int64_t* k, const int64_t* lda, const int64_t* ldw,
+                                 const int64_t* ldc, int epilogue, const void* const* r, const int64_t* ldr, int dtype,
+                                 void* stream) {
+    FINO_CHECK(dtype == FINO_BF16 || dtype == FINO_F16, FINO_ERR_ARG, "fino_gemm_grouped: dtype %d", dtype);
+    FINO_CHECK(count >= 1 && count <= kGroupMaxProblems, FINO_ERR_ARG, "fino_gemm_grouped: count %d (1 .. %d)", count,
+               kGroupMaxProblems);
+    FINO_CHECK(epilogue == FINO_EPI_NONE || epilogue == FINO_EPI_RESIDUAL, FINO_ERR_ARG,
+               "fino_gemm_grouped: epilogue %d (FINO_EPI_NONE or FINO_EPI_RESIDUAL)", epilogue);
+    FINO_CHECK(a && w && c && m && k && lda && ldw && ldc && (epilogue == FINO_EPI_NONE || (r && ldr)), FINO_ERR_ARG,
+               "fino_gemm_grouped: null argument array");
+    FINO_CHECK(n > 0 && n % 8 == 0, FINO_ERR_ARG, "fino_gemm_grouped: N=%lld must be a positive multiple of 8", (long long)n);
+    for (int i = 0; i < count; ++i) {
+        FINO_CHECK(a[i] && w[i] && c[i] && fino_aligned16(a[i]) && fino_aligned16(w[i]) && fino_aligned16(c[i]), FINO_ERR_ARG,
+                   "fino_gemm_grouped: problem %d: A/W/C must be non-null and 16-byte aligned", i);
+        FINO_CHECK(m[i] >= 0 && k[i] > 0 && k[i] % BK == 0, FINO_ERR_ARG,
+                   "fino_gemm_grouped: problem %d: bad shape M=%lld K=%lld (K must be a multiple of %d)", i, (long long)m[i],
+                   (long long)k[i], BK);
+        FINO_CHECK(lda[i] % 8 == 0 && ldw[i] % 8 == 0 && ldc[i] % 8 == 0 && lda[i] >= k[i] && ldw[i] >= k[i] && ldc[i] >= n,
+                   FINO_ERR_ARG, "fino_gemm_grouped: problem %d: leading dimensions must be multiples of 8 and cover the row", i);
+        if (epilogue == FINO_EPI_RESIDUAL)
+            FINO_CHECK(r[i] && ldr[i] % 8 == 0 && ldr[i] >= n && fino_aligned16(r[i]), FINO_ERR_ARG,
+                       "fino_gemm_grouped: problem %d: residual operand", i);
+        FINO_CHECK(((m[i] > 0 ? m[i] - 1 : 0) * lda[i] + k[i]) * 2 < (1ll << 31) && ((n - 1) * ldw[i] + k[i]) * 2 < (1ll << 31),
+                   FINO_ERR_UNSUPPORTED, "fino_gemm_grouped: problem %d: operands must span < 2 GiB", i);
+    }
+    int order[kGroupMaxProblems];
+    for (int i = 0; i < count; ++i) order[i] = i;
+    for (int i = 1; i < count; ++i)
+        for (int j = i; j > 0 && k[order[j]] > k[order[j - 1]]; --j) { const int t = order[j]; order[j] = order[j - 1]; order[j - 1] = t; }
+    GemmGroupParams gp = {};
+    gp.n = n;
+    gp.tiles_n = (int)((n + BN - 1) / BN);
+    int total = 0;
+    const int cus = gemm_device_cus();
+    for (int oi = 0; oi < count; ++oi) {
+        const int i = order[oi];
+        if (m[i] == 0) continue;
+        int gm = fino_tune_get(FINO_TUNE_GEMM_GROUP_M);
+        if (gm <= 0) gm = gemm_default_group_m(gp.tiles_n, k[i]);
+        const TilePlan tp = plan_tiles(m[i], gp.tiles_n, cus);
+        const int64_t r0s[2] = {0, tp.rows1}, rows[2] = {tp.rows1, m[i] - tp.rows1};
+        const int mis[2] = {8, tp.mi2};
+        for (int h = 0; h < 2; ++h) {
+            if (rows[h] <= 0) continue;
+            GemmGroupSeg& g = gp.seg[gp.nseg++];
+            g.a = (const uint16_t*)a[i] + r0s[h] * lda[i];
+            g.w = (const uint16_t*)w[i];
+            g.bias = bias ? (const uint16_t*)bias[i] : nullptr;
+            g.c = (uint16_t*)c[i] + r0s[h] * ldc[i];
+            g.r = epilogue == FINO_EPI_RESIDUAL ? (const uint16_t*)r[i] + r0s[h] * ldr[i] : nullptr;
+            g.m = rows[h]; g.k = k[i]; g.lda = lda[i]; g.ldw = ldw[i]; g.ldc = ldc[i];
+            g.ldr = epilogue == FINO_EPI_RESIDUAL ? ldr[i] : 0;
+            g.mi = mis[h];
+            g.tiles_m = (int)((rows[h] + 32 * g.mi - 1) / (32 * g.mi));
+            g.start = total;
+            g.group_m = gm;
+            total += g.tiles_m * gp.tiles_n;
+        }
+    }
+    if (total == 0) return FINO_OK;
+    hipStream_t st = (hipStream_t)stream;
+    if (dtype == FINO_BF16)
+        return epilogue == FINO_EPI_NONE ? launch_gemm_grouped<BF16, FINO_EPI_NONE>(gp, total, st)
+                                         : launch_gemm_grouped<BF16, FINO_EPI_RESIDUAL>(gp, total, st);
+    return epilogue == FINO_EPI_NONE ? launch_gemm_grouped<F16, FINO_EPI_NONE>(gp, total, st)
+                                     : launch_gemm_grouped<F16, FINO_EPI_RESIDUAL>(gp, total, st);
 }
 
 extern "C" int fino_gemm(const void* a, const void* w, const void* bias, void* c, int64_t m, int64_t n, int64_t k,
diff --git a/frameino_amd/ops.py b/frameino_amd/ops.py
--- a/frameino_amd/ops.py
+++ b/frameino_amd/ops.py
@@ -321,6 +321,39 @@
         kt_ = KernelTimer.active
         kt_.flops["attn_cross"] = kt_.flops.get("attn_cross", 0.0) + 2.0 * lq * hd * sum(int(x) for x in lk_b)
     return out
+
+
+def attention_probs_multi(q, k, heads, lk_b, tail_mult, kps, outs, scale=None, q_rrms=None, q_weight=None, walk=0):
+    import ctypes
+    assert q.dim() == 3 and k.dim() == 3
+    b, lk = k.shape[0], k.shape[1]
+    lq, hd = q.shape[1], q.shape[2]
+    dh = hd // heads
+    assert q.shape[0] in (1, b) and len(lk_b) == b and len(tail_mult) == b and len(kps) == b and len(outs) == b
+    for t in (q, k):
+        assert t.stride(2) == 1 and t.is_cuda
+    for o_, kp in zip(outs, kps):
+        assert o_.shape == (lq, heads * kp) and o_.stride(1) == 1 and o_.dtype == q.dtype and o_.is_cuda
+    shared = q.shape[0] == 1 and b > 1
+    if q_rrms is not None:
+        assert q_rrms.dtype == torch.float32 and q_rrms.shape == (q.shape[0], lq) and q_rrms.stride(1) == 1
+    scale = dh ** -0.5 if scale is None else scale
+    lk_arr = (ctypes.c_int * b)(*[int(x) for x in lk_b])
+    mult_arr = (ctypes.c_float * b)(*[float(x) for x in tail_mult])
+    kp_arr = (ctypes.c_int * b)(*[int(x) for x in kps])
+    p_arr = (ctypes.c_void_p * b)(*[o_.data_ptr() for o_ in outs])
+    prs_arr = (ctypes.c_int64 * b)(*[o_.stride(0) for o_ in outs])
+    ev = _timed("attn_cross")
+    _lib.check(_lib.lib().fino_attn_probs_multi(
+        _p(q), _p(k), ctypes.cast(p_arr, ctypes.c_void_p), b, heads, lq, lk, dh, 0 if shared else q.stride(0), q.stride(1), dh,
+        k.stride(0), k.stride(1), dh, ctypes.cast(kp_arr, ctypes.c_void_p), ctypes.cast(prs_arr, ctypes.c_void_p), float(scale),
+        _dt(q), ctypes.cast(lk_arr, ctypes.c_void_p), ctypes.cast(mult_arr, ctypes.c_void_p), _p(q_rrms),
+        0 if (q_rrms is None or shared) else q_rrms.stride(0), _p(q_weight), int(walk), _stream()), "fino_attn_probs_multi")
+    if ev is not None:
+        ev.record()
+        kt_ = KernelTimer.active
+        kt_.flops["attn_cross"] = kt_.flops.get("attn_cross", 0.0) + 2.0 * lq * hd * sum(int(x) for x in lk_b)
+    return outs
 
 
 _attn_fp8_ws = {}
@@ -435,6 +468,41 @@
     if done is not None:
         done()
     return out
+
+
+def gemm_grouped(problems, epilogue=EPI_NONE):
+    import ctypes
+    cnt = len(problems)
+    assert 1 <= cnt <= 4 and epilogue in (EPI_NONE, EPI_RESIDUAL)
+    n, dt = problems[0][1].shape[0], problems[0][0].dtype
+    pa, pw, pb, pc, pr, ms, ks, lda, ldw, ldc, ldr = ([] for _ in range(11))
+    flops = nbytes = 0.0
+    for a, w, bias, out, residual in problems:
+        a2, m, k, la = _rows2d(a)
+        assert w.dim() == 2 and w.stride(1) == 1 and w.shape == (n, k) and w.dtype == a.dtype == dt
+        o2, mo, no, lc = _rows2d(out)
+        assert (mo, no) == (m, n) and out.dtype == dt
+        if bias is not None:
+            assert bias.dtype == dt and bias.is_contiguous() and bias.numel() == n
+        if epilogue == EPI_RESIDUAL:
+            r2, mr, nr_, lr = _rows2d(residual)
+            assert (mr, nr_) == (m, n) and residual.dtype == dt
+        else:
+            assert residual is None
+            r2, lr = None, 0
+        for lst, v in ((pa, _p(a2)), (pw, _p(w)), (pb, _p(bias)), (pc, _p(o2)), (pr, _p(r2)), (ms, m), (ks, k), (lda, la),
+                       (ldw, w.stride(0)), (ldc, lc), (ldr, lr)):
+            lst.append(v)
+        flops += 2.0 * m * n * k
+        nbytes += 2.0 * (m * k + n * k + m * n * (2 if residual is not None else 1))
+    vp = lambda v: ctypes.cast((ctypes.c_void_p * cnt)(*v), ctypes.c_void_p)
+    ip = lambda v: ctypes.cast((ctypes.c_int64 * cnt)(*v), ctypes.c_void_p)
+    done = _timed_gemm(epilogue, flops, nbytes)
+    _lib.check(_lib.lib().fino_gemm_grouped(cnt, vp(pa), vp(pw), vp(pb), vp(pc), ip(ms), n, ip(ks), ip(lda), ip(ldw), ip(ldc),
+                                            epilogue, vp(pr), ip(ldr), _dt(problems[0][0]), _stream()), "fino_gemm_grouped")
+    if done is not None:
+        done()
+    return [p_[3] for p_ in problems]
 
 
 def gemm_blocked_a(a_blocks, rows, w, bias, residual, gate, sel, out, tile_m=0):
diff --git a/frameino_amd/transformer_wan.py b/frameino_amd/transformer_wan.py
--- a/frameino_amd/transformer_wan.py
+++ b/frameino_amd/transformer_wan.py
@@ -130,6 +130,8 @@
         self.fp8_attention = False
         self.dedup_text_padding = os.environ.get("FINO_TEXT_FOLD", "1") != "0"
         self.reassociate_text_out = os.environ.get("FINO_TEXT_REASSOC", "1") != "0"
+        self.text_tail_multi = os.environ.get("FINO_TEXT_TAIL", "1") != "0"
+        self.text_tail_grouped = os.environ.get("FINO_TEXT_TAIL", "1") not in ("0", "2")
         self.skip_dead_rows = os.environ.get("FINO_SKIP_DEAD_ROWS", "1") != "0"
 
     @property
@@ -612,31 +614,54 @@
                     self._lin(li, "out", att[r0:r1], blk.attn1.to_out[0].weight, blk.attn1.to_out[0].bias, o.EPI_GATED_RESIDUAL,
                               residual=x[r0:r1], gate=m[:, 2], sel=None if sel is None else sel[r0:r1], out=x[r0:r1], **tk)
             n2 = blk.norm2
+            tail1 = (default_procs and text.w2 is not None and self.text_tail_multi and b <= 4
+                     and hasattr(o, "attention_probs_multi"))
+            one_q = tail1 and once and not last_live and not self._fp8
+            qsegs = [(0, n)] if one_q else segs
             xq2 = self._ln_q(li, "q2", 1, x, weight=n2.weight, bias=n2.bias, eps=cfg.eps) if (n2 is not None and
                                                                                                 default_procs) else None
             if xq2 is not None:
                 pass
             elif n2 is not None:
-                for r0, r1 in segs:
+                for r0, r1 in qsegs:
                     o.layernorm(x[r0:r1], n2.weight, n2.bias, cfg.eps, out=nrm[r0:r1])
             else:
                 nrm.copy_(x)
             if default_procs:
-                for r0, r1 in segs:
+                for r0, r1 in qsegs:
                     self._lin(li, "q2", nrm[r0:r1], blk.attn2.to_q.weight, blk.attn2.to_q.bias, xq=xq2, out=q2[r0:r1], **tk)
                 kv = text.kv[li].view(b, lt, 2 * d)
                 s0, s1 = (live if last_live else (0, n))
                 if text.w2 is not None:
                     rr = text.rrms
-                    for r0, r1 in segs:
+                    for r0, r1 in qsegs:
                         o.row_rrms(q2[r0:r1], blk.attn2.norm_q.eps, out=rr[r0:r1])
-                    for i in range(b):
-                        r0, r1 = i * n + s0, i * n + s1
-                        pr = o.attention_probs(q2[r0:r1].view(1, s1 - s0, d), kv[i:i + 1, :, :d], heads, text.tail[0][i:i + 1],
-                                               text.tail[1][i:i + 1], text.kp[i], out=text.pbuf[i][:s1 - s0].view(1, s1 - s0, -1),
-                                               q_rrms=rr[r0:r1].view(1, s1 - s0), q_weight=blk.attn2.norm_q.weight)
-                        xi = x[r0:r1]
-                        o.gemm(pr.view(s1 - s0, -1), text.w2[li][i], blk.attn2.to_out[0].bias, o.EPI_RESIDUAL, residual=xi, out=xi, **tk)
+                    if tail1:
+                        if one_q:
+                            qv, rv = q2[:n].view(1, n, d), rr[:n].view(1, n)
+                        else:
+                            qv, rv = q2.view(b, n, d)[:, s0:s1], rr[:nr].view(b, n)[:, s0:s1]
+                        prs = [text.pbuf[i][:s1 - s0] for i in range(b)]
+                        o.attention_probs_multi(qv, kv[:, :, :d], heads, text.tail[0], text.tail[1], text.kp, prs, q_rrms=rv,
+                                                q_weight=blk.attn2.norm_q.weight)
+                    if (tail1 and self.text_tail_grouped and not tk and hasattr(o, "gemm_grouped")
+                            and all((heads * kp) % 64 == 0 for kp in text.kp)):
+                        xs = [x[i * n + s0:i * n + s1] for i in range(b)]
+                        o.gemm_grouped([(prs[i], text.w2[li][i], blk.attn2.to_out[0].bias, xs[i], xs[i]) for i in range(b)],
+                                       o.EPI_RESIDUAL)
+                    else:
+                        for i in range(b):
+                            r0, r1 = i * n + s0, i * n + s1
+                            if tail1:
+                                pr = prs[i]
+                            else:
+                                pr = o.attention_probs(q2[r0:r1].view(1, s1 - s0, d), kv[i:i + 1, :, :d], heads,
+                                                       text.tail[0][i:i + 1], text.tail[1][i:i + 1], text.kp[i],
+                                                       out=text.pbuf[i][:s1 - s0].view(1, s1 - s0, -1),
+                                                       q_rrms=rr[r0:r1].view(1, s1 - s0), q_weight=blk.attn2.norm_q.weight)
+                            xi = x[r0:r1]
+                            o.gemm(pr.view(s1 - s0, -1), text.w2[li][i], blk.attn2.to_out[0].bias, o.EPI_RESIDUAL, residual=xi,
+                                   out=xi, **tk)
                 else:
                     for r0, r1 in segs:
                         o.rmsnorm_rope_(q2[r0:r1], blk.attn2.norm_q.weight, blk.attn2.norm_q.eps)
diff --git a/include/frameino_hip.h b/include/frameino_hip.h
--- a/include/frameino_hip.h
+++ b/include/frameino_hip.h
@@ -93,6 +93,10 @@
                     int64_t p_rs, float scale, int dtype, const int* lk_b, const float* tail_mult, const float* q_rrms,
                     int64_t q_rrms_bs, const void* q_weight, void* stream);
 int fino_row_rrms(const void* x, int64_t rows, int dim, int64_t ldx, float eps, float* rrms, int dtype, void* stream);
+int fino_attn_probs_multi(const void* q, const void* k, void* const* p, int batch, int heads, int64_t lq, int64_t lk, int head_dim,
+                          int64_t q_bs, int64_t q_rs, int64_t q_hs, int64_t k_bs, int64_t k_rs, int64_t k_hs, const int* kp,
+                          const int64_t* p_rs, float scale, int dtype, const int* lk_b, const float* tail_mult,
+                          const float* q_rrms, int64_t q_rrms_bs, const void* q_weight, int walk, void* stream);
 
 int64_t fino_attn_partial_bytes(int batch, int heads, int64_t lq, int head_dim);
 int fino_attn_partial(const void* q, const void* k, const void* v, int batch, int heads, int64_t lq, int64_t lk,
@@ -124,6 +128,9 @@
                         const int32_t* sel, int dtype, int tile_m, void* stream);
 
 int fino_gemm_plan(int64_t m, int64_t n, int64_t* rows_256, int* tile_rows_rest);
+int fino_gemm_grouped(int count, const void* const* a, const void* const* w, const void* const* bias, void* const* c,
+                      const int64_t* m, int64_t n, const int64_t* k, const int64_t* lda, const int64_t* ldw, const int64_t* ldc,
+                      int epilogue, const void* const* r, const int64_t* ldr, int dtype, void* stream);
 int fino_skinny_linear(const float* x, const void* w, const void* b, float* y, int m, int64_t n, int64_t k,
                        int w_dtype, int silu_input, void* stream);
 
```

Result: no change. 3.785 denoise-steps/s (median of 6 runs) (+0.5%).
